# DaanVrancken/HubbardTN

Measured on AMD Instinct MI355X. Metric: DMRG sweep time (s) + GS energy/site, 1-band Hubbard L=64 chi=1024, lower is better.
Workload: dtype c128; 1 GPU; one-band Hubbard chain L=64 U/t=4, half filling, fZ2xSU(2)xU(1), two-site DMRG sweep (2L-3=125 bond updates) at chi=1024 (TensorKit dim units); model=one_band, L=64, chi=1024, krylovdim=30, parallelism=sector-parallel apply x1, backend=hip

## Files before the change

hubbardtn_amd/abi.py:

```python
from __future__ import annotations

import ctypes as C
import os

import numpy as np

HERE = os.path.dirname(os.path.abspath(__file__))
LIB_PATH = os.path.join(HERE, "csrc", "libhubbardtn_hip.so")

HTN_MAX_BUFS = 8
HTN_TILE = 32
OP_N, OP_T, OP_C = 0, 1, 2
SEG_GEMM, SEG_COPY = 0, 1

TILE_DT = np.dtype([("c_off", "<i8"), ("buf_c", "<i4"), ("ldc", "<i4"), ("m", "<i4"), ("n", "<i4"),
                    ("row0", "<i4"), ("col0", "<i4"), ("seg_begin", "<i4"), ("seg_count", "<i4"),
                    ("pad0", "<i4"), ("pad1", "<i4"), ("part", "<i4"), ("nparts", "<i4"), ("ws_slot", "<i4"),
                    ("ticket", "<i4")], align=False)
BUF_WS = 7
WS_TICKET_ELEMS = 4096
SEG_DT = np.dtype([("a_off", "<i8"), ("b_off", "<i8"), ("buf_a", "<i4"), ("buf_b", "<i4"),
                   ("lda", "<i4"), ("ldb", "<i4"), ("k", "<i4"), ("op_a", "<i4"), ("op_b", "<i4"),
                   ("type", "<i4"), ("alpha_re", "<f8"), ("alpha_im", "<f8")], align=False)
SVD_DT = np.dtype([("g_off", "<i8"), ("v_off", "<i8"), ("s_off", "<i8"), ("m", "<i4"), ("n", "<i4"),
                   ("flags", "<i4"), ("pad", "<i4")], align=False)
SVD_ACCUMULATE = 1
SVD_QRCP = 2
COPY_DT = np.dtype([("dst_off", "<i8"), ("src_off", "<i8"), ("idx_off", "<i8"), ("scl_off", "<i8"),
                    ("rows", "<i4"), ("cols", "<i4"), ("ldd", "<i4"), ("lds", "<i4"), ("op", "<i4"),
                    ("gather_dim", "<i4"), ("scale_dim", "<i4"), ("inv_norm", "<i4")], align=False)
assert TILE_DT.itemsize == 64 and SEG_DT.itemsize == 64 and SVD_DT.itemsize == 40 and COPY_DT.itemsize == 64

SYM_SU2_U1, SYM_U1_U1, SYM_SU2 = 0, 1, 2
MAX_SITE = 4
BACKEND_CPU, BACKEND_HIP = 0, 1
SITE_OP_DT = np.dtype([("k", "<i4"), ("dN", "<i4"), ("red", "<f8", (MAX_SITE * MAX_SITE,))], align=False)
MPO_ENTRY_DT = np.dtype([("wl", "<i4"), ("wr", "<i4"), ("op", "<i4"), ("pad", "<i4"), ("coef_re", "<f8"),
                         ("coef_im", "<f8")], align=False)
SUBBLOCK_DT = np.dtype([("lN", "<i4"), ("lj", "<i4"), ("s", "<i4"), ("rN", "<i4"), ("rj", "<i4"), ("ld", "<i4"),
                        ("off", "<i8")], align=False)
SECTOR_DT = np.dtype([("N", "<i4"), ("j", "<i4"), ("count", "<i4")], align=False)
ENV_BLOCK_DT = np.dtype([("aN", "<i4"), ("aj", "<i4"), ("w", "<i4"), ("bN", "<i4"), ("bj", "<i4"), ("rows", "<i4"),
                         ("cols", "<i4"), ("pad", "<i4"), ("off", "<i8")], align=False)
BOND_STATS_DT = np.dtype([("bond", "<i4"), ("direction", "<i4"), ("n_matvec", "<i4"), ("jacobi_sweeps", "<i4"),
                          ("chi_full", "<i4"), ("multiplets", "<i4"), ("n_tiles", "<i4"), ("n_segs", "<i4"),
                          ("theta_size", "<i8"), ("apply_flops", "<i8"), ("apply_bytes", "<i8"), ("svd_flops", "<i8"),
                          ("energy", "<f8"), ("residual", "<f8"), ("trunc_weight", "<f8"), ("t_plan", "<f8"),
                          ("t_lanczos", "<f8"), ("t_svd", "<f8"), ("t_env", "<f8"), ("t_total", "<f8"),
                          ("matvec_ms", "<f8")], align=False)
assert SITE_OP_DT.itemsize == 136 and MPO_ENTRY_DT.itemsize == 32 and SUBBLOCK_DT.itemsize == 32
assert SECTOR_DT.itemsize == 12 and ENV_BLOCK_DT.itemsize == 40 and BOND_STATS_DT.itemsize == 136


class Symmetry(C.Structure):
    _fields_ = [("kind", C.c_int32), ("n_site", C.c_int32), ("site_N", C.c_int32 * MAX_SITE),
                ("site_j", C.c_int32 * MAX_SITE)]


class SvdOpts(C.Structure):
    _fields_ = [("split_elems", C.c_int32), ("sweeps_hint", C.c_int32), ("rank_cut", C.c_double),
                ("sweeps_used", C.POINTER(C.c_int32))]


class SweepOpts(C.Structure):
    _fields_ = [("chi_full", C.c_int32), ("weighting", C.c_int32), ("cutoff", C.c_double), ("krylovdim", C.c_int32),
                ("maxrestart", C.c_int32), ("lanczos_tol", C.c_double), ("jacobi_tol", C.c_double),
                ("jacobi_max_sweeps", C.c_int32), ("svd_split_elems", C.c_int32), ("rank_cut", C.c_double),
                ("profile", C.c_int32), ("pad", C.c_int32)]


class IdmrgOpts(C.Structure):
    _fields_ = [("sweep", SweepOpts), ("cell_sites", C.c_int32), ("window_dN", C.c_int32), ("tol", C.c_double),
                ("min_steps", C.c_int32), ("maxiter", C.c_int32), ("sweeps_per_step", C.c_int32), ("warm_start", C.c_int32)]


class IdmrgStats(C.Structure):
    _fields_ = [("step", C.c_int32), ("sweeps", C.c_int32), ("converged", C.c_int32), ("finished", C.c_int32),
                ("needs_window", C.c_int32), ("chi_full", C.c_int32), ("energy", C.c_double),
                ("energy_per_site", C.c_double), ("delta", C.c_double)]


assert C.sizeof(SweepOpts) == 64 and C.sizeof(IdmrgOpts) == 96 and C.sizeof(IdmrgStats) == 48

EXPORTS = ["htn_last_error", "htn_abi_version", "htn_device_init", "htn_grouped_gemm_z",
           "htn_dots_scratch_elems", "htn_dots_z", "htn_axpys_z", "htn_scale_inv_sqrt_z",
           "htn_jacobi_svd_z", "htn_batched_copy_z", "htn_lanczos_scratch_elems", "htn_lanczos_z", "htn_lanczos_orth_z"]
ENGINE_EXPORTS = ["htn_ctx_create", "htn_ctx_destroy", "htn_ctx_backend", "htn_ctx_set_timing", "htn_comm_unique_id",
                  "htn_ctx_set_comm", "htn_ctx_set_exchange", "htn_mpo_create", "htn_mpo_destroy", "htn_mps_create",
                  "htn_mps_destroy", "htn_bond_update", "htn_dmrg2_sweep", "htn_mps_theta_size", "htn_heff2_apply",
                  "htn_mps_get_theta", "htn_mps_nsites", "htn_mps_bond", "htn_mps_spectrum", "htn_mps_site_size",
                  "htn_mps_get_site", "htn_mps_env_size", "htn_mps_get_env", "htn_mps_env_blocks", "htn_mps_env_bond",
                  "htn_plan_apply_dump", "htn_mps_cache_stats", "htn_balance_tiles",
                  "htn_idmrg_create", "htn_idmrg_destroy", "htn_idmrg_boundary", "htn_idmrg_step", "htn_idmrg_window",
                  "htn_mps_set_orthogonal", "htn_mps_orthogonal_count", "htn_mps_overlap"]


class GemmLaunch(C.Structure):
    _fields_ = [("bufs", C.c_void_p * HTN_MAX_BUFS), ("tiles", C.c_void_p), ("segs", C.c_void_p),
                ("n_tiles", C.c_int32), ("pad", C.c_int32)]


EXCHANGE_FN = C.CFUNCTYPE(C.c_int, C.c_void_p, C.c_int64, C.c_void_p)

_lib = None


class HtnError(RuntimeError):
    pass


def load_library(path: str | None = None):
    global _lib
    if _lib is not None and path is None:
        return _lib
    p = path or LIB_PATH
    import torch
    if not os.path.exists(p):
        raise HtnError(f"{p} not found: build it with `python -m hubbardtn_amd.build` "
                       "(hipcc --offload-arch=gfx950); there is no CPU fallback")
    lib = C.CDLL(p)
    vp, i32, i64, f64 = C.c_void_p, C.c_int32, C.c_int64, C.c_double
    lib.htn_last_error.restype = C.c_char_p
    lib.htn_abi_version.restype = C.c_int
    lib.htn_device_init.argtypes = [C.c_int, C.c_char_p, C.POINTER(C.c_int)]
    lib.htn_grouped_gemm_z.argtypes = [C.POINTER(vp), vp, i32, vp, vp]
    lib.htn_dots_scratch_elems.argtypes = [i32]
    lib.htn_dots_scratch_elems.restype = i64
    lib.htn_dots_z.argtypes = [vp, i64, i32, vp, i64, vp, vp, vp]
    lib.htn_axpys_z.argtypes = [vp, vp, i64, i32, vp, f64, i64, vp]
    lib.htn_scale_inv_sqrt_z.argtypes = [vp, vp, vp, i64, vp]
    lib.htn_jacobi_svd_z.argtypes = [vp, vp, vp, vp, vp, i32, i32, i32, f64, vp, C.POINTER(SvdOpts), vp]
    lib.htn_batched_copy_z.argtypes = [vp, vp, vp, vp, vp, i32, f64, vp]
    lib.htn_lanczos_scratch_elems.argtypes = [i32]
    lib.htn_lanczos_scratch_elems.restype = i64
    lib.htn_lanczos_z.argtypes = [C.POINTER(GemmLaunch), i32, i32, i32, vp, i64, i32, f64, i32, vp, i32,
                                  EXCHANGE_FN, vp, C.POINTER(f64), C.POINTER(i32), C.POINTER(f64), C.POINTER(f64), vp]
    lib.htn_lanczos_orth_z.argtypes = [C.POINTER(GemmLaunch), i32, i32, i32, vp, i64, i32, f64, i32, vp, i32,
                                       EXCHANGE_FN, vp, C.POINTER(f64), C.POINTER(i32), C.POINTER(f64), C.POINTER(f64),
                                       vp, i32, vp]
    declare_engine(lib)
    for name in EXPORTS + ENGINE_EXPORTS:
        getattr(lib, name)
    if lib.htn_abi_version() != ABI_VERSION:
        raise HtnError("ABI version mismatch")
    if path is None:
        _lib = lib
    return lib


ABI_VERSION = 2


def declare_engine(lib):
    vp, i32, i64, f64 = C.c_void_p, C.c_int32, C.c_int64, C.c_double
    lib.htn_last_error.restype = C.c_char_p
    lib.htn_abi_version.restype = C.c_int
    lib.htn_ctx_create.argtypes = [i32, i32, vp, C.POINTER(vp)]
    lib.htn_ctx_destroy.argtypes = [vp]
    lib.htn_ctx_destroy.restype = None
    lib.htn_ctx_backend.argtypes = [vp]
    lib.htn_ctx_set_timing.argtypes = [vp, i32]
    lib.htn_comm_unique_id.argtypes = [vp]
    lib.htn_ctx_set_comm.argtypes = [vp, i32, i32, vp]
    lib.htn_ctx_set_exchange.argtypes = [vp, i32, i32, EXCHANGE_FN, vp]
    lib.htn_mpo_create.argtypes = [vp, C.POINTER(Symmetry), i32, vp, i32, vp, vp, vp, vp, C.POINTER(vp)]
    lib.htn_mpo_destroy.argtypes = [vp]
    lib.htn_mpo_destroy.restype = None
    lib.htn_mps_create.argtypes = [vp, vp, i32, vp, vp, vp, vp, vp, vp, vp, vp, C.POINTER(vp)]
    lib.htn_mps_destroy.argtypes = [vp]
    lib.htn_mps_destroy.restype = None
    lib.htn_bond_update.argtypes = [vp, i32, i32, i32, i32, C.POINTER(SweepOpts), vp]
    lib.htn_dmrg2_sweep.argtypes = [vp, C.POINTER(SweepOpts), vp, C.POINTER(f64)]
    lib.htn_mps_theta_size.argtypes = [vp, i32]
    lib.htn_mps_theta_size.restype = i64
    lib.htn_heff2_apply.argtypes = [vp, i32, vp, vp]
    lib.htn_mps_get_theta.argtypes = [vp, i32, vp]
    lib.htn_mps_nsites.argtypes = [vp]
    lib.htn_mps_bond.argtypes = [vp, i32, vp]
    lib.htn_mps_spectrum.argtypes = [vp, i32, vp, vp]
    lib.htn_mps_spectrum.restype = i64
    lib.htn_mps_site_size.argtypes = [vp, i32, C.POINTER(i32)]
    lib.htn_mps_site_size.restype = i64
    lib.htn_mps_get_site.argtypes = [vp, i32, vp, vp]
    lib.htn_mps_env_size.argtypes = [vp, i32, i32]
    lib.htn_mps_env_size.restype = i64
    lib.htn_mps_get_env.argtypes = [vp, i32, i32, vp]
    lib.htn_mps_env_blocks.argtypes = [vp, i32, i32, vp]
    lib.htn_mps_env_bond.argtypes = [vp, i32, i32, vp]
    lib.htn_plan_apply_dump.argtypes = [vp, i32, i32, C.POINTER(i32), vp, C.POINTER(i32), vp, C.POINTER(i64),
                                        C.POINTER(i64)]
    lib.htn_mps_cache_stats.argtypes = [vp, C.POINTER(i64), C.POINTER(i64)]
    lib.htn_balance_tiles.argtypes = [vp, i32, i32, vp, i32, C.POINTER(i32)]
    lib.htn_idmrg_create.argtypes = [vp, vp, C.POINTER(IdmrgOpts), C.POINTER(vp)]
    lib.htn_idmrg_destroy.argtypes = [vp]
    lib.htn_idmrg_destroy.restype = None
    lib.htn_idmrg_boundary.argtypes = [vp, i32, vp]
    lib.htn_idmrg_step.argtypes = [vp, vp, vp, vp, vp, vp, vp, C.POINTER(IdmrgStats)]
    lib.htn_idmrg_window.argtypes = [vp, C.POINTER(vp)]
    lib.htn_mps_set_orthogonal.argtypes = [vp, C.POINTER(vp), i32]
    lib.htn_mps_orthogonal_count.argtypes = [vp, C.POINTER(i32)]
    lib.htn_mps_overlap.argtypes = [vp, vp, C.POINTER(f64)]
    for name in ENGINE_EXPORTS:
        getattr(lib, name)


def check(lib, rc: int, what: str):
    if rc != 0:
        raise HtnError(f"{what}: {lib.htn_last_error().decode()}")
```

hubbardtn_amd/csrc/htn_backend_hip.hip:

```cpp
#include <dlfcn.h>

#include <map>
#include <mutex>

#include "htn_common.h"
#include "htn_core.h"

namespace {

__global__ __launch_bounds__(256) void k_scale_z(double2* __restrict__ x, int64_t n, double f) {
    for (int64_t j = (int64_t)blockIdx.x * blockDim.x + threadIdx.x; j < n; j += (int64_t)gridDim.x * blockDim.x) {
        const double2 v = x[j];
        x[j] = make_double2(v.x * f, v.y * f);
    }
}

__global__ __launch_bounds__(256) void k_copy_words(uint32_t* __restrict__ dst, const uint32_t* __restrict__ src, size_t n) {
    for (size_t j = (size_t)blockIdx.x * blockDim.x + threadIdx.x; j < n; j += (size_t)gridDim.x * blockDim.x) dst[j] = src[j];
    __threadfence_system();
}

struct Rccl {
    void* lib = nullptr;
    int (*GetUniqueId)(void*) = nullptr;
// ... 161 lines not shown
        } else
            HIP_TRY(hipMemcpyAsync(land, src, bytes, hipMemcpyDeviceToHost, st));
        HIP_TRY(htn_stream_spin(st));
        memcpy(dst, land, bytes);
        stage_pos = 0;
        return 0;
    }
    int zero(void* p, size_t bytes) override {
        if (!bytes) return 0;
        HIP_TRY(hipMemsetAsync(p, 0, bytes, st));
        return 0;
    }
    int sync() override {
        HIP_TRY(htn_stream_spin(st));
        stage_pos = 0;
        return 0;
    }
    int grouped_gemm(const void* const* bufs, const htn_tile* tiles, int32_t n_tiles, const htn_seg* segs) override {
        return htn_grouped_gemm_z(bufs, tiles, n_tiles, segs, st);
    }
    int lanczos(const htn_gemm_launch* stages, int n_stages, int x_slot, int y_slot, void* V, int64_t n, int krylovdim,
                double tol, int max_restart, int zero_y, htn_exchange2_fn exchange, void* user, double* eig, int* n_matvec,
                double* residual, double* matvec_ms) override {
        if (ensure_lan_scratch(htn_lanczos_scratch_elems(krylovdim))) return 1;
        int32_t nmv = 0;
        const int rc = htn_lanczos_z(stages, n_stages, x_slot, y_slot, V, n, krylovdim, tol, max_restart, lan_scratch, zero_y,
                                     exchange, user, eig, &nmv, residual, matvec_ms, st);
        *n_matvec = nmv;
        return rc;
    }
    int ensure_lan_scratch(int64_t need) {
        if (need > lan_scratch_elems) {
            if (lan_scratch) HIP_TRY(hipFree(lan_scratch));
            HIP_TRY(hipMalloc(&lan_scratch, sizeof(double2) * need));
            if (htn_debug_poison()) HIP_TRY(hipMemsetAsync(lan_scratch, 0xFF, sizeof(double2) * need, st));
            lan_scratch_elems = need;
        }
        return 0;
    }
    int lanczos_orth(const htn_gemm_launch* stages, int n_stages, int x_slot, int y_slot, void* V, int64_t n, int krylovdim,
                     double tol, int max_restart, int zero_y, htn_exchange2_fn exchange, void* user, const void* Q, int n_frozen,
                     double* eig, int* n_matvec, double* residual, double* matvec_ms) override {
        if (ensure_lan_scratch(htn_lanczos_scratch_elems(krylovdim + n_frozen))) return 1;
        int32_t nmv = 0;
        const int rc = htn_lanczos_orth_z(stages, n_stages, x_slot, y_slot, V, n, krylovdim, tol, max_restart, lan_scratch, zero_y,
                                          exchange, user, eig, &nmv, residual, matvec_ms, Q, n_frozen, st);
        *n_matvec = nmv;
        return rc;
    }
    int orthonormalise_rows(void* Pv, int64_t n, int nvec, double drop_tol, int* kept) override {
        if (nvec > 32) return htn::set_error("orthonormalise_rows: more than 32 rows");
        if (ensure_lan_scratch(htn_dots_scratch_elems(32) + 64)) return 1;
        double2* P = (double2*)Pv;
        double2* part = (double2*)lan_scratch;
        double2* coef = part + htn_dots_scratch_elems(32);
        double2* nrm = coef + 32;
        int k = 0;
        for (int r = 0; r < nvec; ++r) {
            double2* dst = P + (int64_t)k * n;
            if (r != k) HIP_TRY(hipMemcpyAsync(dst, P + (int64_t)r * n, sizeof(double2) * n, hipMemcpyDeviceToDevice, st));
            if (htn_dots_z(dst, n, 1, dst, n, nrm, part, st)) return 1;
            for (int pass = 0; pass < 2 && k > 0; ++pass) {
                if (htn_dots_z(P, n, k, dst, n, coef, part, st)) return 1;
                if (htn_axpys_z(dst, P, n, k, coef, -1.0, n, st)) return 1;
            }
            if (htn_dots_z(dst, n, 1, dst, n, nrm + 1, part, st)) return 1;
            double h[4];
            if (download(h, nrm, sizeof(h))) return 1;
            const double n0 = h[0], n1 = h[2];
            if (!(n0 > 0.0) || !(n1 > drop_tol * drop_tol * n0)) continue;
            if (htn_scale_inv_sqrt_z(dst, dst, nrm + 1, n, st)) return 1;
            ++k;
        }
        *kept = k;
        return 0;
    }
    int jacobi_svd(void* G, void* Vj, double* S, const htn_svd_block* desc_dev, const htn_svd_block* desc_host, int n_blocks,
                   int max_m, int max_sweeps, double tol, int32_t* info_dev, const htn_svd_opts* opts) override {
        fork_open = true;
        const int rc = htn_jacobi_svd_z(G, Vj, S, desc_dev, desc_host, n_blocks, max_m, max_sweeps, tol, info_dev, opts, st);
        fork_open = false;
        return rc;
    }
    int batched_copy(void* dst, const void* src, const int32_t* idx, const double* scl, const htn_copy_item* items, int n_items,
                     double gscale) override {
        return htn_batched_copy_z(dst, src, idx, scl, items, n_items, gscale, st);
    }
    int scale(void* x, int64_t n, double f) override {
        if (n <= 0) return 0;
        const int grid = (int)std::min<int64_t>((n + 255) / 256, 2048);
        hipLaunchKernelGGL(k_scale_z, dim3(grid), dim3(256), 0, st, (double2*)x, n, f);
        HIP_TRY(hipGetLastError());
        return 0;
    }
    int set_comm(int rank, int world, const void* id) override {
        Rccl& r = rccl();
        if (!r.ok) return htn::set_error("htn_ctx_set_comm: librccl.so could not be loaded");
        if (comm) {
            r.CommDestroy(comm);
            comm = nullptr;
        }
        NcclId uid;
        memcpy(uid.internal, id, sizeof(uid.internal));
        const int rc = ((nccl_init_fn)r.CommInitRank)(&comm, world, uid, rank);
        if (rc != 0) return htn::set_error("ncclCommInitRank: %s", r.GetErrorString ? r.GetErrorString(rc) : "error");
        return 0;
    }
    bool has_comm() const override { return comm != nullptr; }
    int allreduce(void* y, int64_t n) override {
        if (!comm) return htn::set_error("allreduce: no communicator (htn_ctx_set_comm)");
        const int rc = rccl().AllReduce(y, y, (size_t)(2 * n), 8, 0, comm, st);
        if (rc != 0) return htn::set_error("ncclAllReduce: %s", rccl().GetErrorString ? rccl().GetErrorString(rc) : "error");
        return 0;
    }
};

}

char* htn_err_buf() { return htn::err_buf(); }

namespace htn {
Backend* make_backend(int backend, int device, void* stream) {
    if (backend != HTN_BACKEND_HIP) {
        set_error("libhubbardtn_hip.so has no CPU backend (backend %d requested): there is no CPU fallback", backend);
        return nullptr;
    }
    char name[256];
    int cus = 0;
    if (htn_device_init(device, name, &cus)) return nullptr;
    auto* b = new HipBackend();
    b->device = device;
    if (stream) b->st = (hipStream_t)stream;
    else {
        if (hipStreamCreateWithFlags(&b->st, hipStreamNonBlocking) != hipSuccess) {
            set_error("hipStreamCreate failed");
            delete b;
            return nullptr;
        }
        b->own_stream = true;
    }
    return b;
}
}

extern "C" int htn_comm_unique_id(void* id_host) {
    Rccl& r = rccl();
    if (!r.ok) return htn::set_error("htn_comm_unique_id: librccl.so could not be loaded");
    const int rc = r.GetUniqueId(id_host);
    if (rc != 0) return htn::set_error("ncclGetUniqueId: %s", r.GetErrorString ? r.GetErrorString(rc) : "error");
    return 0;
}
```

hubbardtn_amd/csrc/htn_common.h:

```cpp
#pragma once
#include <hip/hip_runtime.h>
#include <stdint.h>
#include <stdio.h>
#include <stdlib.h>
#include <string.h>

#include <map>
#include <memory>
#include <mutex>
#include <utility>

#include "hubbardtn_hip.h"

char* htn_err_buf();

static inline int htn_fail(const char* what, hipError_t e) {
    snprintf(htn_err_buf(), 512, "%s: %s", what, hipGetErrorString(e));
    return 1;
}
static inline int htn_fail_msg(const char* what) {
    snprintf(htn_err_buf(), 512, "%s", what);
    return 1;
}
#define fail htn_fail
// ... 43 lines not shown
__host__ __device__ __forceinline__ unsigned long long lan_check(unsigned long long w0, unsigned long long w1, unsigned long long w2,
                                                                 unsigned long long serial) {
    return serial ^ lan_rotl(w0, 13) ^ lan_rotl(w1, 29) ^ lan_rotl(w2, 47) ^ 0x9E3779B97F4A7C15ull;
}
#define HTN_DOT_BLOCKS 256
struct HtnGemmPublish {
    const double* norm_partial;
    const double2* c1;
    const double2* c2;
    LanRecord* rec_out;
    unsigned long long serial;
};
int htn_grouped_gemm_launch(const void* const* bufs_host, const htn_tile* tiles, int32_t n_tiles, const htn_seg* segs,
                            const HtnGemmPublish* pub, hipStream_t stream);

enum HtnBufKind {
    HTN_BUF_DEVICE,
    HTN_BUF_PINNED,
    HTN_BUF_MAPPED
};
struct HtnBuf {
    const HtnBufKind kind;
    const bool poison;
    void* p = nullptr;
    void* dev = nullptr;
    size_t cap = 0;
    explicit HtnBuf(HtnBufKind k, bool poison_new = true) : kind(k), poison(poison_new) {}
    HtnBuf(const HtnBuf&) = delete;
    ~HtnBuf() { (void)release(); }
    hipError_t release() {
        const hipError_t e = !p ? hipSuccess : (kind == HTN_BUF_DEVICE ? hipFree(p) : hipHostFree(p));
        p = dev = nullptr, cap = 0;
        return e;
    }
    int reserve(size_t bytes) {
        if (bytes <= cap) return 0;
        HIP_TRY(release());
        const size_t want = bytes * 2;
        if (kind == HTN_BUF_DEVICE) {
            HIP_TRY(hipMalloc(&p, want));
            dev = p;
            if (poison && htn_debug_poison()) HIP_TRY(hipMemset(p, 0xFF, want));
        } else if (kind == HTN_BUF_PINNED) {
            HIP_TRY(hipHostMalloc(&p, want, hipHostMallocDefault));
        } else {
            HIP_TRY(hipHostMalloc(&p, want, hipHostMallocMapped | hipHostMallocCoherent));
            HIP_TRY(hipHostGetDevicePointer(&dev, p, 0));
        }
        cap = want;
        return 0;
    }
};

template <class T>
class HtnStreamRegistry {
    std::mutex mu;
    std::map<std::pair<int, hipStream_t>, std::unique_ptr<T>> entries;

public:
    template <class Init>
    int get(hipStream_t st, T** out, Init init) {
        int dev = 0;
        HIP_TRY(hipGetDevice(&dev));
        std::lock_guard<std::mutex> lk(mu);
        auto it = entries.find({dev, st});
        if (it == entries.end()) {
            auto r = std::make_unique<T>();
            r->device = dev;
            if (init(*r)) return 1;
            it = entries.emplace(std::make_pair(dev, st), std::move(r)).first;
        }
        *out = it->second.get();
        return 0;
    }
    void release(hipStream_t st) {
        int dev = 0;
        if (hipGetDevice(&dev) != hipSuccess) return;
        std::lock_guard<std::mutex> lk(mu);
        entries.erase({dev, st});
    }
};
void htn_krylov_release_stream(hipStream_t st);
void htn_svd_release_stream(hipStream_t st);

template <int CTRL>
__device__ __forceinline__ double dpp_f64(double v) {
    const int lo = __builtin_amdgcn_update_dpp(0, __double2loint(v), CTRL, 0xF, 0xF, true);
    const int hi = __builtin_amdgcn_update_dpp(0, __double2hiint(v), CTRL, 0xF, 0xF, true);
    return __hiloint2double(hi, lo);
}

__device__ __forceinline__ double row_sum16(double v) {
    v += dpp_f64<0xB1>(v);
    v += dpp_f64<0x4E>(v);
    v += dpp_f64<0x141>(v);
    v += dpp_f64<0x140>(v);
    return v;
}

template <int L>
__device__ __forceinline__ double lane_bcast(double v) {
    const int lo = __builtin_amdgcn_readlane(__double2loint(v), L);
    const int hi = __builtin_amdgcn_readlane(__double2hiint(v), L);
    return __hiloint2double(hi, lo);
}

__device__ __forceinline__ double wave_sum(double v) {
    v = row_sum16(v);
    const double a = lane_bcast<0>(v) + lane_bcast<16>(v);
    const double b = lane_bcast<32>(v) + lane_bcast<48>(v);
    return a + b;
}

template <int CTRL>
__device__ __forceinline__ unsigned long long dpp_u64(unsigned long long v) {
    const unsigned lo = (unsigned)__builtin_amdgcn_update_dpp(0, (int)(unsigned)v, CTRL, 0xF, 0xF, true);
    const unsigned hi = (unsigned)__builtin_amdgcn_update_dpp(0, (int)(unsigned)(v >> 32), CTRL, 0xF, 0xF, true);
    return ((unsigned long long)hi << 32) | lo;
}
__device__ __forceinline__ unsigned long long umax64(unsigned long long a, unsigned long long b) { return a > b ? a : b; }
__device__ __forceinline__ unsigned long long row_max16_u64(unsigned long long v) {
    v = umax64(v, dpp_u64<0xB1>(v));
    v = umax64(v, dpp_u64<0x4E>(v));
    v = umax64(v, dpp_u64<0x141>(v));
    v = umax64(v, dpp_u64<0x140>(v));
    return v;
}
template <int L>
__device__ __forceinline__ unsigned long long lane_bcast_u64(unsigned long long v) {
    const unsigned lo = (unsigned)__builtin_amdgcn_readlane((int)(unsigned)v, L);
    const unsigned hi = (unsigned)__builtin_amdgcn_readlane((int)(unsigned)(v >> 32), L);
    return ((unsigned long long)hi << 32) | lo;
}
__device__ __forceinline__ unsigned long long wave_max_u64(unsigned long long v) {
    v = row_max16_u64(v);
    return umax64(umax64(lane_bcast_u64<0>(v), lane_bcast_u64<16>(v)),
                  umax64(lane_bcast_u64<32>(v), lane_bcast_u64<48>(v)));
}

__device__ __forceinline__ double fast_rcp(double a) {
    double x = __builtin_amdgcn_rcp(a);
    x = fma(fma(-a, x, 1.0), x, x);
    x = fma(fma(-a, x, 1.0), x, x);
    return x;
}
__device__ __forceinline__ double fast_rsq(double a) {
    double y = __builtin_amdgcn_rsq(a);
    const double h = 0.5 * a;
    y = y * fma(-h * y, y, 1.5);
    y = y * fma(-h * y, y, 1.5);
    return y;
}
```

hubbardtn_amd/csrc/htn_core.h:

```cpp
#pragma once
#include <stdint.h>
#include <string.h>

#include <array>
#include <complex>
#include <memory>
#include <string>
#include <unordered_map>
#include <utility>
#include <vector>

#include "hubbardtn_hip.h"

namespace htn {

typedef std::complex<double> cplx;

enum { BUF_X = 0, BUF_Y, BUF_L, BUF_R, BUF_Z, BUF_S1, BUF_S2, BUF_AUX };

struct Sec {
    int32_t N, j;
};
inline bool operator<(const Sec& a, const Sec& b) { return a.N < b.N || (a.N == b.N && a.j < b.j); }
inline bool operator==(const Sec& a, const Sec& b) { return a.N == b.N && a.j == b.j; }
// ... 184 lines not shown
    int64_t zsize = 0;
    int64_t nterms = 0;
};
void plan_apply(const Mpo& mpo, const ThetaLayout& tl, const EnvLayout& Ll, const EnvLayout& Rl, const MpoSite& W1,
                const MpoSite& W2, ApplyPlan& out);
void plan_theta(const char* mode, const SiteLayout& lay1, const SiteLayout& lay2, const ThetaLayout& tl, Tasks& out);
struct EnvPlan {
    Tasks t1, t2;
    int64_t zsize = 0;
};
void plan_left_env(const Mpo& mpo, const EnvLayout& Ll, const SiteLayout& lay, const MpoSite& W, const EnvLayout& Lnew,
                   EnvPlan& out);
void plan_right_env(const Mpo& mpo, const EnvLayout& Rl, const SiteLayout& lay, const MpoSite& W, const EnvLayout& Rnew,
                    EnvPlan& out);

struct OvlLayout {
    BondP rows, cols;
    std::vector<Sec> secs;
    std::vector<int64_t> off;
    std::vector<int32_t> m, n;
    std::unordered_map<uint64_t, int> index;
    int64_t size = 0;
    int find(Sec s) const {
        auto it = index.find(skey(s));
        return it == index.end() ? -1 : it->second;
    }
};
typedef std::shared_ptr<const OvlLayout> OvlLayoutP;
OvlLayoutP build_ovl_layout(BondP rows, BondP cols);
struct OvlPlan {
    Tasks t1, t2;
    int64_t zsize = 0;
};
void plan_ovl_left(const OvlLayout& Ol, const SiteLayout& bra, const SiteLayout& ket, const OvlLayout& Onew, OvlPlan& out);
void plan_ovl_right(const OvlLayout& Or, const SiteLayout& bra, const SiteLayout& ket, const OvlLayout& Onew, OvlPlan& out);
void plan_ovl_project(const OvlLayout& Ol, const OvlLayout& Or, const SiteLayout& k1, const SiteLayout& k2, const ThetaLayout& tl,
                      OvlPlan& out);

struct SvdPlan {
    std::vector<htn_svd_block> desc;
    std::vector<htn_copy_item> stage;
    std::vector<Sec> mids;
    std::vector<char> transposed, accumulate;
    int64_t g_size = 0, v_size = 0, s_size = 0;
    int32_t max_m = 0;
    int64_t flops = 0;
    bool any_accumulate = false;
};
int plan_svd(const ThetaLayout& tl, bool right, SvdPlan& out);

void truncate(const std::vector<double>& vals, const std::vector<int>& lens, const std::vector<int>& qdims, int chi_full,
              double cutoff, int weighting, std::vector<int>& counts, double& trunc_weight, double& kept_norm);

struct FinalizePlan {
    std::vector<htn_copy_item> iso_g, cen_g, iso_v;
    Tasks cen;
    bool has_cen = false;
    int64_t n_idx = 0;
};
void plan_finalize(const ThetaLayout& tl, const SvdPlan& sp, const std::vector<int>& keep, const SiteLayout& layA,
                   const SiteLayout& layB, bool right, int64_t offA, int64_t offB, FinalizePlan& out);

struct Backend {
    virtual ~Backend() {}
    virtual int kind() const = 0;
    virtual int activate() { return 0; }
    virtual void* alloc(size_t bytes) = 0;
    virtual void release(void* p) = 0;
    virtual int upload(void* dst, const void* src_host, size_t bytes) = 0;
    virtual int download(void* dst_host, const void* src, size_t bytes) = 0;
    virtual int zero(void* p, size_t bytes) = 0;
    virtual int sync() = 0;
    virtual int grouped_gemm(const void* const* bufs, const htn_tile* tiles, int32_t n_tiles, const htn_seg* segs) = 0;
    virtual int lanczos(const htn_gemm_launch* stages, int n_stages, int x_slot, int y_slot, void* V, int64_t n,
                        int krylovdim, double tol, int max_restart, int zero_y, htn_exchange2_fn exchange, void* user,
                        double* eig, int* n_matvec, double* residual, double* matvec_ms) = 0;
    virtual int lanczos_orth(const htn_gemm_launch* stages, int n_stages, int x_slot, int y_slot, void* V, int64_t n,
                             int krylovdim, double tol, int max_restart, int zero_y, htn_exchange2_fn exchange, void* user,
                             const void* Q, int n_frozen, double* eig, int* n_matvec, double* residual, double* matvec_ms);
    virtual int orthonormalise_rows(void* P, int64_t n, int nvec, double drop_tol, int* kept);
    virtual int jacobi_svd(void* G, void* Vj, double* S, const htn_svd_block* desc_dev, const htn_svd_block* desc_host,
                           int n_blocks, int max_m, int max_sweeps, double tol, int32_t* info_dev,
                           const htn_svd_opts* opts) = 0;
    virtual int batched_copy(void* dst, const void* src, const int32_t* idx, const double* scl,
                             const htn_copy_item* items_dev, int n_items, double gscale) = 0;
    virtual int scale(void* x, int64_t n, double f) = 0;
    virtual int set_comm(int rank, int world, const void* id) { return 1; }
    virtual bool has_comm() const { return false; }
    virtual int allreduce(void* y, int64_t n) { return 1; }
    bool timing = false;
};

int set_error(const char* fmt, ...);
char* err_buf();

}
```

hubbardtn_amd/csrc/htn_engine.cpp:

```cpp
#include <math.h>
#include <stdio.h>
#include <stdlib.h>

#include <algorithm>
#include <atomic>
#include <chrono>
#include <map>

#include "htn_core.h"

namespace htn {
Backend* make_backend(int backend, int device, void* stream);
}
using namespace htn;

namespace {
void tridiag_lowest_host(const std::vector<double>& alpha, const std::vector<double>& beta, double* eig, std::vector<double>& vec) {
    const int k = (int)alpha.size();
    auto count = [&](double x) {
        int cnt = 0;
        double d = 1.0;
        for (int i = 0; i < k; ++i) {
            d = (alpha[i] - x) - (i ? beta[i - 1] * beta[i - 1] / d : 0.0);
            if (d == 0.0) d = 1e-300;
// ... 191 lines not shown
    }
    DBuf(const DBuf&) = delete;
    DBuf& operator=(const DBuf&) = delete;
};
typedef std::shared_ptr<DBuf> DBufP;
struct DView {
    DBufP base;
    int64_t off = 0;
    cplx* ptr() const { return base ? (cplx*)base->p + off : nullptr; }
};

struct DevTasks {
    DBufP mem;
    const htn_tile* tiles = nullptr;
    const htn_seg* segs = nullptr;
    int32_t ntiles = 0, nsegs = 0;
    int32_t ws_slots = 0;
    int64_t flops = 0;
};

struct ApplyC {
    DevTasks dz, dy;
    bool has_z = false;
    int64_t zsize = 0, flops = 0;
    int32_t ntiles = 0, nsegs = 0;
};
struct EnvC {
    EnvLayoutP lay;
    DevTasks d1, d2;
    int64_t zsize = 0, flops = 0;
};
struct SvdC {
    SvdPlan sp;
    DBufP stage, desc;
    std::vector<htn_svd_block> own_desc;
    DBufP own_stage, own_desc_dev;
    int n_own = 0;
};
struct FinC {
    SiteLayoutP layA, layB;
    DBufP items;
    const htn_copy_item *ig = nullptr, *cg = nullptr, *iv = nullptr;
    int n_ig = 0, n_cg = 0, n_iv = 0;
    DevTasks cen;
    bool has_cen = false;
};

struct Spectrum {
    std::vector<Sec> secs;
    std::vector<std::vector<double>> vals;
};
struct OvlC {
    OvlLayoutP lay;
    DevTasks d1, d2;
    int64_t zsize = 0;
};
struct OrthState {
    htn_mps* phi = nullptr;
    std::vector<OvlLayoutP> Llay, Rlay;
    std::vector<DView> Lbuf, Rbuf;
};

}

struct htn_mps {
    std::atomic<int> refs{1};
    htn_ctx* ctx;
    htn_mpo* mpo_handle = nullptr;
    Backend* be;
    const Mpo* mpo;
    int L;
    std::vector<BondP> bonds;
    std::vector<SiteLayoutP> site_lay;
    std::vector<DView> site_buf;
    std::vector<EnvLayoutP> Llay, Rlay;
    std::vector<DView> Lbuf, Rbuf;
    std::unordered_map<std::string, std::shared_ptr<const void>> cache;
    int64_t hits = 0, misses = 0;
    double energy = 0.0;
    std::map<int, Spectrum> spectra;
    std::map<int, std::pair<std::pair<int, double>, double>> cut_hint;
    std::map<int, int> sweeps_hint;
    std::vector<int32_t> idx_host;
    std::vector<OrthState> orth;
    int orth_dropped = 0;

    template <class T, class F>
    std::shared_ptr<T> cached(const std::string& key, F build) {
        auto it = cache.find(key);
        if (it != cache.end()) {
            ++hits;
            return std::const_pointer_cast<T>(std::static_pointer_cast<const T>(it->second));
        }
        if (cache.size() > 20000) cache.clear();
        ++misses;
        std::shared_ptr<T> v = build();
        if (v) cache[key] = v;
        return v;
    }
    static std::string ikey(const char* tag, int i) {
        std::string k(tag);
        k.append((const char*)&i, sizeof(i));
        return k;
    }
    DBufP dalloc(size_t bytes) {
        auto b = std::make_shared<DBuf>(be, bytes);
        return b->p ? b : nullptr;
    }
    DView zalloc(int64_t n, bool zero) {
        DView v;
        v.base = dalloc(sizeof(cplx) * (size_t)std::max<int64_t>(n, 1));
        if (v.base && zero) be->zero(v.base->p, sizeof(cplx) * (size_t)std::max<int64_t>(n, 1));
        return v;
    }
    DView ws;
    int64_t ws_slots = -1;
    int ensure_ws(int slots) {
        if (slots <= ws_slots) return 0;
        const int64_t want = std::max<int64_t>(2 * (int64_t)slots, 256);
        ws = zalloc(HTN_WS_ELEMS(want), false);
        if (!ws.base) return set_error("device allocation of the split-K workspace failed");
        if (be->zero(ws.ptr(), sizeof(cplx) * HTN_WS_TICKET_ELEMS)) return 1;
        ws_slots = want;
        return 0;
    }
    int upload_tasks(const Tasks& t_in, DevTasks& d) {
        Tasks balanced;
        const Tasks* tp = &t_in;
        d.ws_slots = 0;
        if (be->kind() == HTN_BACKEND_HIP && t_in.ntiles > 0) {
            balanced = t_in;
            balanced.tiles.resize((size_t)t_in.ntiles);
            d.ws_slots = balance_tiles(balanced, 256);
            tp = &balanced;
        }
        const Tasks& t = *tp;
        const size_t tb = (sizeof(htn_tile) * t.tiles.size() + 63) / 64 * 64, sb = sizeof(htn_seg) * t.segs.size();
        d.mem = dalloc(tb + sb);
        if (!d.mem) return set_error("device allocation of a task list failed");
        if (be->upload(d.mem->p, t.tiles.data(), sizeof(htn_tile) * t.tiles.size())) return 1;
        if (be->upload((char*)d.mem->p + tb, t.segs.data(), sb)) return 1;
        d.tiles = (const htn_tile*)d.mem->p;
        d.segs = (const htn_seg*)((char*)d.mem->p + tb);
        d.ntiles = t.ntiles;
        d.nsegs = t.nsegs;
        d.flops = t.flops;
        return 0;
    }
    SiteLayoutP site_layout(char kind, BondP bl, BondP br) {
        return cached<const SiteLayout>(std::string("slay") + kind + bl->key + "|" + br->key,
                                        [&] { return build_site_layout(mpo->sym, kind, bl, br); });
    }
    ThetaLayoutP theta_layout(BondP bl, BondP br) {
        return cached<const ThetaLayout>(std::string("tl") + bl->key + "|" + br->key,
                                         [&] { return build_theta_layout(mpo->sym, bl, br); });
    }
    int gemm(const DevTasks& d, std::initializer_list<std::pair<int, const void*>> bufs) {
        if (d.ntiles == 0) return 0;
        if (ensure_ws(d.ws_slots)) return 1;
        const void* table[HTN_MAX_BUFS] = {nullptr};
        for (auto& kv : bufs) table[kv.first] = kv.second;
        table[HTN_BUF_WS] = ws.ptr();
        return be->grouped_gemm(table, d.tiles, d.ntiles, d.segs);
    }

    int left_env(int i);
// ... 275 lines not shown
        if (plan_svd(tl, right, s->sp)) return nullptr;
        s->stage = dalloc(sizeof(htn_copy_item) * s->sp.stage.size());
        s->desc = dalloc(sizeof(htn_svd_block) * s->sp.desc.size());
        if (!s->stage || !s->desc) return nullptr;
        if (be->upload(s->stage->p, s->sp.stage.data(), sizeof(htn_copy_item) * s->sp.stage.size())) return nullptr;
        if (be->upload(s->desc->p, s->sp.desc.data(), sizeof(htn_svd_block) * s->sp.desc.size())) return nullptr;
        if (ctx->world > 1) {
            const int nbk = (int)s->sp.mids.size();
            std::vector<int> ord(nbk);
            for (int b = 0; b < nbk; ++b) ord[b] = b;
            auto cost = [&](int b) { return (double)s->sp.desc[b].m * s->sp.desc[b].n * s->sp.desc[b].n; };
            std::stable_sort(ord.begin(), ord.end(), [&](int a, int b) { return cost(a) > cost(b); });
            std::vector<double> load(ctx->world, 0.0);
            std::vector<htn_copy_item> st_own;
            for (int b : ord) {
                int r = 0;
                for (int q = 1; q < ctx->world; ++q)
                    if (load[q] < load[r]) r = q;
                load[r] += cost(b);
                if (r == ctx->rank) {
                    s->own_desc.push_back(s->sp.desc[b]);
                    st_own.push_back(s->sp.stage[b]);
                }
            }
            s->n_own = (int)s->own_desc.size();
            if (s->n_own) {
                s->own_stage = dalloc(sizeof(htn_copy_item) * st_own.size());
                s->own_desc_dev = dalloc(sizeof(htn_svd_block) * s->own_desc.size());
                if (!s->own_stage || !s->own_desc_dev) return nullptr;
                if (be->upload(s->own_stage->p, st_own.data(), sizeof(htn_copy_item) * st_own.size())) return nullptr;
                if (be->upload(s->own_desc_dev->p, s->own_desc.data(), sizeof(htn_svd_block) * s->own_desc.size())) return nullptr;
            }
        }
        return s;
    });
    if (!sc) return 1;
    const SvdPlan& sp = sc->sp;
    const int nb = (int)sp.mids.size();
    DView G = zalloc(sp.g_size, false), Vj = zalloc(sp.v_size, false);
    const size_t s_elems = ((size_t)std::max<int64_t>(sp.s_size, 1) + 1) & ~(size_t)1, i_elems = (size_t)std::max(nb, 1);
    DBufP S = dalloc(sizeof(double) * s_elems + sizeof(int32_t) * i_elems);
    if (!G.base || !Vj.base || !S) return set_error("device allocation failed (SVD workspace)");
    int32_t* info_dev = (int32_t*)((double*)S->p + s_elems);
    const bool svd_shard = ctx->world > 1 && ctx->shard;
    if (svd_shard) {
        if (be->zero(G.ptr(), sizeof(cplx) * (size_t)std::max<int64_t>(sp.g_size, 1))) return 1;
        if (be->zero(S->p, sizeof(double) * s_elems + sizeof(int32_t) * i_elems)) return 1;
        if (sp.any_accumulate && be->zero(Vj.ptr(), sizeof(cplx) * (size_t)std::max<int64_t>(sp.v_size, 1))) return 1;
        if (sc->n_own && be->batched_copy(G.ptr(), x, nullptr, nullptr, (const htn_copy_item*)sc->own_stage->p, sc->n_own, 1.0)) return 1;
    } else if (be->batched_copy(G.ptr(), x, nullptr, nullptr, (const htn_copy_item*)sc->stage->p, nb, 1.0))
        return 1;
    htn_svd_opts so;
    int32_t jac_used = 0;
    so.split_elems = o.svd_split_elems;
    so.sweeps_hint = 0;
    so.rank_cut = 0.0;
    so.sweeps_used = &jac_used;
    {
        auto h = sweeps_hint.find(i + 1);
        if (h != sweeps_hint.end()) so.sweeps_hint = h->second;
    }
    if (o.rank_cut > 0.0) {
        double cut = 0.0;
        auto h = cut_hint.find(i + 1);
        if (h != cut_hint.end() && h->second.first.first == o.chi_full && h->second.first.second == o.cutoff)
            cut = o.rank_cut * h->second.second;
        so.rank_cut = std::max(cut, o.rank_cut * o.cutoff);
    }
    if (svd_shard) {
        if (sc->n_own && be->jacobi_svd(G.ptr(), Vj.ptr(), (double*)S->p, (const htn_svd_block*)sc->own_desc_dev->p,
                                        sc->own_desc.data(), sc->n_own, sp.max_m, o.jacobi_max_sweeps > 0 ? o.jacobi_max_sweeps : 40,
                                        o.jacobi_tol > 0.0 ? o.jacobi_tol : 1e-14, info_dev, &so))
            return 1;
        if (exchange_tramp(G.ptr(), std::max<int64_t>(sp.g_size, 1), ctx)) return set_error("sharded SVD: exchange of the blocks failed");
        if (exchange_tramp(S->p, (int64_t)(s_elems / 2), ctx)) return set_error("sharded SVD: exchange of the singular values failed");
        if (sp.any_accumulate && exchange_tramp(Vj.ptr(), std::max<int64_t>(sp.v_size, 1), ctx)) return 1;
    } else if (be->jacobi_svd(G.ptr(), Vj.ptr(), (double*)S->p, (const htn_svd_block*)sc->desc->p, sp.desc.data(), nb, sp.max_m,
                              o.jacobi_max_sweeps > 0 ? o.jacobi_max_sweeps : 40, o.jacobi_tol > 0.0 ? o.jacobi_tol : 1e-14,
                              info_dev, &so))
        return 1;
    if (jac_used > 0) sweeps_hint[i + 1] = jac_used;
    static const bool dbg_timers = getenv("HTN_DEBUG_HOST_TIMERS") != nullptr;
    const double tA = now();
    std::vector<double> s_host(s_elems + (i_elems + 1) / 2);
    if (be->download(s_host.data(), S->p, sizeof(double) * s_elems + sizeof(int32_t) * i_elems)) return 1;
    const double tB = now();
    const int32_t* info_h = (const int32_t*)(s_host.data() + s_elems);
    int jac_sweeps = 0;
    for (int b = 0; b < (svd_shard ? sc->n_own : nb); ++b) {
        if (info_h[b] < 0) return set_error("Jacobi SVD did not converge (bond %d, block %d, %d sweeps)", i + 1, b, -info_h[b]);
        jac_sweeps = std::max(jac_sweeps, (int)info_h[b]);
    }
    std::vector<int> lens(nb), qd(nb);
    std::vector<std::vector<int>> order(nb);
    std::vector<double> vals;
    vals.reserve((size_t)sp.s_size);
    std::vector<std::pair<double, int>> tmp;
    for (int b = 0; b < nb; ++b) {
        const int len = sp.desc[b].n;
        const double* sv = s_host.data() + sp.desc[b].s_off;
        lens[b] = len;
        qd[b] = sym.qdim(sp.mids[b]);
        tmp.resize(len);
        for (int k = 0; k < len; ++k) tmp[k] = {sv[k], k};
        std::sort(tmp.begin(), tmp.end(), [](const std::pair<double, int>& a, const std::pair<double, int>& c) {
            return a.first != c.first ? a.first > c.first : a.second < c.second;
        });
        order[b].resize(len);
        for (int k = 0; k < len; ++k) {
            order[b][k] = tmp[k].second;
            vals.push_back(tmp[k].first);
        }
    }
    std::vector<int> counts;
    double tw = 0.0, nrm = 0.0;
    truncate(vals, lens, qd, o.chi_full, o.cutoff, o.weighting, counts, tw, nrm);
    std::vector<std::pair<Sec, int>> mid_items;
    int64_t kept_tot = 0, positive = 0;
    for (int b = 0; b < nb; ++b) {
        if (counts[b] > 0) mid_items.push_back({sp.mids[b], counts[b]});
        kept_tot += counts[b];
    }
    for (double v : vals) positive += v > 0.0;
    if (kept_tot == 0 || !(nrm > 0.0)) return set_error("htn_bond_update: nothing kept by the truncation on bond %d", i + 1);
    BondP mid = std::make_shared<Bond>(mid_items);
    const double tC = now();
    if (o.chi_full > 0 && tw > 0.0 && kept_tot < positive) {
        double smin = 1e300;
        size_t p = 0;
        for (int b = 0; b < nb; ++b) {
            if (counts[b] > 0) smin = std::min(smin, vals[p + counts[b] - 1]);
            p += lens[b];
        }
        cut_hint[i + 1] = {{o.chi_full, o.cutoff}, smin};
    } else
        cut_hint.erase(i + 1);
    std::string ckey((const char*)counts.data(), sizeof(int) * counts.size());
    auto fc = cached<FinC>(std::string(right ? "finR" : "finL") + bl->key + "|" + br->key + "|" + ckey, [&]() -> std::shared_ptr<FinC> {
        auto f = std::make_shared<FinC>();
        f->layA = site_layout('L', bl, mid);
        f->layB = site_layout('R', mid, br);
        FinalizePlan fp;
        plan_finalize(tl, sp, counts, *f->layA, *f->layB, right, 0, f->layA->size, fp);
        f->n_ig = (int)fp.iso_g.size(), f->n_cg = (int)fp.cen_g.size(), f->n_iv = (int)fp.iso_v.size();
        const size_t tot = (size_t)(f->n_ig + f->n_cg + f->n_iv);
        if (tot) {
            std::vector<htn_copy_item> all;
            all.insert(all.end(), fp.iso_g.begin(), fp.iso_g.end());
            all.insert(all.end(), fp.cen_g.begin(), fp.cen_g.end());
            all.insert(all.end(), fp.iso_v.begin(), fp.iso_v.end());
            f->items = dalloc(sizeof(htn_copy_item) * tot);
            if (!f->items || be->upload(f->items->p, all.data(), sizeof(htn_copy_item) * tot)) return nullptr;
            f->ig = (const htn_copy_item*)f->items->p;
            f->cg = f->ig + f->n_ig;
            f->iv = f->cg + f->n_cg;
        }
        f->has_cen = fp.has_cen;
        if (fp.has_cen && upload_tasks(fp.cen, f->cen)) return nullptr;
        return f;
    });
    if (!fc) return 1;
    const double tD = now();
    idx_host.clear();
    for (int b = 0; b < nb; ++b)
        for (int k = 0; k < counts[b]; ++k) idx_host.push_back(order[b][k]);
    DBufP idx_d = dalloc(sizeof(int32_t) * std::max<size_t>(idx_host.size(), 1));
    const int64_t sizeA = fc->layA->size, sizeB = fc->layB->size;
    DView out = zalloc(sizeA + sizeB, true);
    if (!idx_d || !out.base) return set_error("device allocation failed (site tensors)");
    if (be->upload(idx_d->p, idx_host.data(), sizeof(int32_t) * idx_host.size())) return 1;
    const int32_t* idxp = (const int32_t*)idx_d->p;
    const double* Sp = (const double*)S->p;
    if (fc->n_ig && be->batched_copy(out.ptr(), G.ptr(), idxp, Sp, fc->ig, fc->n_ig, 1.0)) return 1;
    if (fc->n_cg && be->batched_copy(out.ptr(), G.ptr(), idxp, Sp, fc->cg, fc->n_cg, 1.0 / nrm)) return 1;
    if (fc->n_iv && be->batched_copy(out.ptr(), Vj.ptr(), idxp, Sp, fc->iv, fc->n_iv, 1.0)) return 1;
    if (fc->has_cen) {
        if (be->scale(x, n, 1.0 / nrm)) return 1;
        if (gemm(fc->cen, {{BUF_X, x}, {BUF_S1, out.ptr()}, {BUF_Y, out.ptr()}})) return 1;
    }
    bonds[i + 1] = mid;
    site_lay[i] = fc->layA;
    site_buf[i] = DView{out.base, out.off};
    site_lay[i + 1] = fc->layB;
    site_buf[i + 1] = DView{out.base, out.off + sizeA};
    if (dbg_timers)
        fprintf(stderr, "bond %d: svd call %.1f us, download %.1f, sort+truncate %.1f, finalize plan %.1f, enqueue %.1f  misses %lld hits %lld nvals %zu\n", i + 1,
                (tA - t0 - t_plan - t_lan) * 1e6, (tB - tA) * 1e6, (tC - tB) * 1e6, (tD - tC) * 1e6, (now() - tD) * 1e6, (long long)misses, (long long)hits, vals.size());
    if (o.profile) be->sync();
    const double t_svd = now() - t0 - t_plan - t_lan;
    if (right ? left_env(i) : right_env(i + 1)) return 1;
    for (auto& os : orth)
        if (right ? ovl_left(os.phi, i, os.Llay[i], os.Lbuf[i], &os.Llay[i + 1], &os.Lbuf[i + 1])
                  : ovl_right(os.phi, i + 1, os.Rlay[i + 2], os.Rbuf[i + 2], &os.Rlay[i + 1], &os.Rbuf[i + 1]))
            return 1;
    if (o.profile) be->sync();
    const double t_env = now() - t0 - t_plan - t_lan - t_svd;
    energy = E;
    Spectrum spec;
    {
        size_t p = 0;
        for (int b = 0; b < nb; ++b) {
            if (counts[b] > 0) {
                spec.secs.push_back(sp.mids[b]);
                std::vector<double> v(counts[b]);
                const double f = 1.0 / nrm / sqrt((double)qd[b]);
                for (int k = 0; k < counts[b]; ++k) v[k] = vals[p + k] * f;
                spec.vals.push_back(std::move(v));
            }
            p += lens[b];
        }
    }
    spectra[i + 1] = std::move(spec);
    if (st) {
        memset(st, 0, sizeof(*st));
        st->bond = i + 1;
        st->direction = direction;
        st->n_matvec = nmv;
        st->jacobi_sweeps = jac_sweeps;
        st->chi_full = (int32_t)mid->dim_full(sym);
        st->multiplets = mid->multiplets();
        st->n_tiles = ap->ntiles;
        st->n_segs = ap->nsegs;
        st->theta_size = n;
        st->apply_flops = ap->flops;
        st->apply_bytes = 16 * (2 * n + Llay[i]->size + Rlay[i + 2]->size);
        st->svd_flops = sp.flops;
        st->energy = E;
        st->residual = res;
        st->trunc_weight = tw;
        st->t_plan = t_plan;
        st->t_lanczos = t_lan;
        st->t_svd = t_svd;
        st->t_env = t_env;
        st->t_total = now() - t0;
        st->matvec_ms = mv_ms > 0.0 ? mv_ms : 0.0;
    }
    return 0;
}

int htn_mps::sweep(const htn_sweep_opts& o, htn_bond_stats* st, double* E) {
    int k = 0;
    for (int i = 0; i < L - 1; ++i, ++k)
        if (update_bond(i, +1, i < L - 2, true, o, st ? st + k : nullptr)) return 1;
    for (int i = L - 3; i >= 0; --i, ++k)
        if (update_bond(i, -1, false, true, o, st ? st + k : nullptr)) return 1;
    if (E) *E = energy;
    return 0;
}
// ... 1025 lines not shown
```

hubbardtn_amd/csrc/htn_krylov.hip:

```cpp
#include <math.h>

#include <chrono>
#include <vector>

#include "htn_common.h"

#define DOT_BLOCKS HTN_DOT_BLOCKS
#define DOT_THREADS 256
#define DOT_CHUNK 32

#define HTN_CH_DISPATCH(nvec, per, LAUNCH)          \
    do {                                            \
        if ((nvec) <= 4) LAUNCH(4, 256);            \
        else if ((nvec) <= 8) LAUNCH(8, 256);       \
        else if ((nvec) <= 12) LAUNCH(12, 256);     \
        else if ((nvec) <= 16) LAUNCH(16, 256);     \
        else if ((nvec) <= 20) LAUNCH(20, 256);     \
        else if ((nvec) <= 24) LAUNCH(24, 256);     \
        else if ((nvec) <= 28) LAUNCH(28, 256);     \
        else LAUNCH(32, 256);                       \
    } while (0)
static inline int64_t dot_slice(int64_t n) { return (n + DOT_BLOCKS - 1) / DOT_BLOCKS; }

template <bool FZ>
// ... 293 lines not shown
#pragma unroll
        for (int b = 0; b < DOT_BLOCKS / 64; ++b) t += norm_partial[tid + 64 * b];
        t = wave_sum(t);
        if (tid == 0) {
            s_inv = t > 0.0 ? 1.0 / sqrt(t) : 0.0;
            if (blockIdx.x == 0 && rec_out) {
                const unsigned long long w0 = (unsigned long long)__double_as_longlong(c1[0].x);
                const unsigned long long w1 = (unsigned long long)__double_as_longlong(c2[0].x);
                const unsigned long long w2 = (unsigned long long)__double_as_longlong(t);
                ulonglong2* out = (ulonglong2*)rec_out;
                out[0] = make_ulonglong2(w0, w1);
                out[1] = make_ulonglong2(w2, lan_check(w0, w1, w2, serial));
                __threadfence_system();
            }
        }
    }
    __syncthreads();
    const double s = s_inv;
    for (int64_t j = (int64_t)blockIdx.x * DOT_THREADS + tid; j < n; j += (int64_t)gridDim.x * DOT_THREADS) {
        const double2 v = src[j];
        dst[j] = make_double2(v.x * s, v.y * s);
    }
}

__global__ __launch_bounds__(64) void k_publish_record(const double* __restrict__ norm_partial, const double2* __restrict__ c1,
                                                       const double2* __restrict__ c2, LanRecord* __restrict__ rec_out,
                                                       unsigned long long serial) {
    const int tid = threadIdx.x;
    double t = 0.0;
#pragma unroll
    for (int b = 0; b < DOT_BLOCKS / 64; ++b) t += norm_partial[tid + 64 * b];
    t = wave_sum(t);
    if (tid == 0) {
        const unsigned long long w0 = (unsigned long long)__double_as_longlong(c1[0].x);
        const unsigned long long w1 = (unsigned long long)__double_as_longlong(c2[0].x);
        const unsigned long long w2 = (unsigned long long)__double_as_longlong(t);
        ulonglong2* out = (ulonglong2*)rec_out;
        out[0] = make_ulonglong2(w0, w1);
        out[1] = make_ulonglong2(w2, lan_check(w0, w1, w2, serial));
        __threadfence_system();
    }
}

__global__ __launch_bounds__(DOT_THREADS) void k_norm_partial(const double2* __restrict__ w, int64_t n,
                                                              double* __restrict__ norm_partial) {
    __shared__ double red[DOT_THREADS / 64];
    const int tid = threadIdx.x;
    const int64_t per = (n + DOT_BLOCKS - 1) / DOT_BLOCKS;
    const int64_t lo = (int64_t)blockIdx.x * per;
    const int64_t hi = lo + per < n ? lo + per : n;
    double nn = 0.0;
    for (int64_t j = lo + tid; j < hi; j += DOT_THREADS) {
        const double2 x = w[j];
        nn += x.x * x.x + x.y * x.y;
    }
    nn = wave_sum(nn);
    if ((tid & 63) == 0) red[tid >> 6] = nn;
    __syncthreads();
    if (tid == 0) {
        double t = 0.0;
        for (int q = 0; q < DOT_THREADS / 64; ++q) t += red[q];
        norm_partial[blockIdx.x] = t;
    }
}

__global__ __launch_bounds__(256) void k_axpys(double2* __restrict__ w, const double2* __restrict__ V,
                                               int64_t ldv, int nvec, const double2* __restrict__ coef,
                                               double sign, int64_t n) {
    for (int64_t j = (int64_t)blockIdx.x * blockDim.x + threadIdx.x; j < n; j += (int64_t)gridDim.x * blockDim.x) {
        double sr = 0.0, si = 0.0;
        for (int i = 0; i < nvec; ++i) {
            const double2 c = coef[i];
            const double2 v = V[(int64_t)i * ldv + j];
            sr += c.x * v.x - c.y * v.y;
            si += c.x * v.y + c.y * v.x;
        }
        double2 x = w[j];
        x.x += sign * sr;
        x.y += sign * si;
        w[j] = x;
    }
}

__global__ __launch_bounds__(256) void k_scale_inv_sqrt(double2* __restrict__ dst, const double2* __restrict__ src,
                                                        const double2* __restrict__ nrm2, int64_t n) {
    const double s = 1.0 / sqrt(nrm2[0].x);
    for (int64_t j = (int64_t)blockIdx.x * blockDim.x + threadIdx.x; j < n; j += (int64_t)gridDim.x * blockDim.x) {
        const double2 v = src[j];
        dst[j] = make_double2(v.x * s, v.y * s);
    }
}

static inline int grid_for(int64_t n) {
    int64_t b = (n + 255) / 256;
    return (int)(b > 1024 ? 1024 : (b < 1 ? 1 : b));
}

extern "C" int64_t htn_dots_scratch_elems(int32_t nvec) { return (int64_t)nvec * DOT_BLOCKS; }

extern "C" int htn_dots_z(const void* V, int64_t ldv, int32_t nvec, const void* w, int64_t n, void* out,
                          void* scratch, void* stream) {
    if (nvec <= 0) return 0;
    if (nvec > 64) return fail_msg("htn_dots_z: nvec > 64");
    launch_dots_partial((const double2*)V, ldv, nvec, (const double2*)w, n, (double2*)scratch, (hipStream_t)stream);
    hipLaunchKernelGGL(k_dots_reduce, dim3(nvec), dim3(64), 0, (hipStream_t)stream, (const double2*)scratch,
                       nvec, (double2*)out);
    HIP_TRY(hipGetLastError());
    return 0;
}

extern "C" int htn_axpys_z(void* w, const void* V, int64_t ldv, int32_t nvec, const void* coef, double sign,
                           int64_t n, void* stream) {
    if (nvec <= 0 || n <= 0) return 0;
    hipLaunchKernelGGL(k_axpys, dim3(grid_for(n)), dim3(256), 0, (hipStream_t)stream, (double2*)w, (const double2*)V,
                       ldv, nvec, (const double2*)coef, sign, n);
    HIP_TRY(hipGetLastError());
    return 0;
}

extern "C" int htn_scale_inv_sqrt_z(void* dst, const void* src, const void* nrm2, int64_t n, void* stream) {
    if (n <= 0) return 0;
    hipLaunchKernelGGL(k_scale_inv_sqrt, dim3(grid_for(n)), dim3(256), 0, (hipStream_t)stream, (double2*)dst,
                       (const double2*)src, (const double2*)nrm2, n);
    HIP_TRY(hipGetLastError());
    return 0;
}

static int sturm_count(const std::vector<double>& a, const std::vector<double>& b, double x) {
    int cnt = 0;
    double d = 1.0;
    const int k = (int)a.size();
    for (int i = 0; i < k; ++i) {
        const double off = i ? b[i - 1] * b[i - 1] : 0.0;
        d = (a[i] - x) - (i ? off / d : 0.0);
        if (d == 0.0) d = 1e-300;
        if (d < 0.0) ++cnt;
    }
    return cnt;
}

static void tridiag_lowest(const std::vector<double>& alpha, const std::vector<double>& beta, double* eig,
                           std::vector<double>& vec) {
    const int k = (int)alpha.size();
    double lo = alpha[0], hi = alpha[0];
    for (int i = 0; i < k; ++i) {
        const double r = (i ? fabs(beta[i - 1]) : 0.0) + (i + 1 < k ? fabs(beta[i]) : 0.0);
        lo = fmin(lo, alpha[i] - r);
        hi = fmax(hi, alpha[i] + r);
    }
    const double scale = fmax(fabs(lo), fabs(hi)) + 1e-300;
    hi = hi + 1e-12 * scale;
    for (int it = 0; it < 200 && hi - lo > 4e-16 * scale; ++it) {
        const double mid = 0.5 * (lo + hi);
        if (sturm_count(alpha, beta, mid) >= 1) hi = mid;
        else lo = mid;
    }
    const double lam = 0.5 * (lo + hi);
    *eig = lam;
    vec.assign(k, 1.0 / sqrt((double)k));
    if (k == 1) {
        vec[0] = 1.0;
        return;
    }
    const double mu = lam - 1e-10 * scale;
    std::vector<double> d(k), l(k), z(k);
    d[0] = alpha[0] - mu;
    for (int i = 1; i < k; ++i) {
        l[i] = beta[i - 1] / d[i - 1];
        d[i] = (alpha[i] - mu) - l[i] * beta[i - 1];
        if (d[i] == 0.0) d[i] = 1e-300;
    }
    for (int i = 0; i < k; ++i) vec[i] = (i & 1) ? -0.7 : 1.0;
    for (int iter = 0; iter < 4; ++iter) {
        z[0] = vec[0];
        for (int i = 1; i < k; ++i) z[i] = vec[i] - l[i] * z[i - 1];
        z[k - 1] /= d[k - 1];
        for (int i = k - 2; i >= 0; --i) z[i] = z[i] / d[i] - l[i + 1] * z[i + 1];
        double nn = 0.0;
        for (int i = 0; i < k; ++i) nn += z[i] * z[i];
        nn = 1.0 / sqrt(nn);
        for (int i = 0; i < k; ++i) vec[i] = z[i] * nn;
    }
    if (vec[0] < 0.0)
        for (int i = 0; i < k; ++i) vec[i] = -vec[i];
}

extern "C" int64_t htn_lanczos_scratch_elems(int32_t krylovdim) {
    return 2 * (int64_t)(krylovdim + 1) * DOT_BLOCKS + 3 * (krylovdim + 1) + DOT_BLOCKS + 8;
}

#define LAN_SLOTS 64
namespace {
struct LanRes {
    int device = -1;
    LanRecord* h_rec = nullptr;
    LanRecord* d_rec = nullptr;
    double2* h_y = nullptr;
    hipEvent_t ev_done[LAN_SLOTS], ev_mv0[LAN_SLOTS], ev_mv1[LAN_SLOTS];
    bool have_events = false;
    unsigned long long serial = 0;
    unsigned sample = 0;
    ~LanRes() {
        if (device >= 0) (void)hipSetDevice(device);
        if (h_rec) (void)hipHostFree(h_rec);
        if (h_y) (void)hipHostFree(h_y);
        if (have_events)
            for (int i = 0; i < LAN_SLOTS; ++i) {
                (void)hipEventDestroy(ev_done[i]);
                (void)hipEventDestroy(ev_mv0[i]);
                (void)hipEventDestroy(ev_mv1[i]);
            }
    }
};
HtnStreamRegistry<LanRes> g_lan_res;

int lan_res_get(hipStream_t st, LanRes** out) {
    return g_lan_res.get(st, out, [](LanRes& r) -> int {
        HIP_TRY(hipHostMalloc((void**)&r.h_rec, sizeof(LanRecord) * LAN_SLOTS, hipHostMallocMapped | hipHostMallocCoherent));
        memset(r.h_rec, 0, sizeof(LanRecord) * LAN_SLOTS);
        HIP_TRY(hipHostGetDevicePointer((void**)&r.d_rec, r.h_rec, 0));
        HIP_TRY(hipHostMalloc((void**)&r.h_y, sizeof(double2) * LAN_SLOTS, hipHostMallocDefault));
        for (int i = 0; i < LAN_SLOTS; ++i) {
            HIP_TRY(hipEventCreateWithFlags(&r.ev_done[i], hipEventDisableTiming));
            HIP_TRY(hipEventCreate(&r.ev_mv0[i]));
            HIP_TRY(hipEventCreate(&r.ev_mv1[i]));
        }
        r.have_events = true;
        return 0;
    });
}
}

void htn_krylov_release_stream(hipStream_t st) { g_lan_res.release(st); }

static int lanczos_run(const htn_gemm_launch* stages, int32_t n_stages, int32_t x_slot, int32_t y_slot,
                       void* Vv, int64_t n, int32_t krylovdim, double tol, int32_t max_restart,
                       void* scratch, int32_t zero_y, htn_exchange2_fn exchange, void* user,
                       double* eig_host, int32_t* n_matvec_host, double* residual_host,
                       double* matvec_ms_host, void* stream_v, const double2* Q, int nf) {
    hipStream_t st = (hipStream_t)stream_v;
    const int kd = krylovdim;
    const int kt = kd + nf;
    double2* V = (double2*)Vv;
    double2* partial = (double2*)scratch;
    double2* partial2 = partial + (int64_t)(kt + 1) * DOT_BLOCKS;
    double2* c1 = partial2 + (int64_t)(kt + 1) * DOT_BLOCKS;
    double2* c2 = c1 + (kt + 1);
    double2* ycoef = c2 + (kt + 1);
    double* norm_partial = (double*)(ycoef + (kt + 1));

    LanRes* R = nullptr;
    if (lan_res_get(st, &R)) return 1;
    const bool event_waits = htn_debug_event_waits();
    static const bool full_first_pass = htn_env_flag("HTN_LANCZOS_FULL_FIRST_PASS");

    bool timed_step[LAN_SLOTS] = {false};
    unsigned long long step_serial[LAN_SLOTS] = {0};
    auto matvec = [&](double2* x, double2* y, const HtnGemmPublish* pub) -> int {
        if (zero_y) HIP_TRY(hipMemsetAsync(y, 0, sizeof(double2) * n, st));
        bool published = pub == nullptr;
        for (int s = 0; s < n_stages; ++s) {
            const void* bufs[HTN_MAX_BUFS];
            for (int b = 0; b < HTN_MAX_BUFS; ++b) bufs[b] = stages[s].bufs[b];
            bufs[x_slot] = x;
            bufs[y_slot] = y;
            const bool here = !published && stages[s].n_tiles > 0;
            if (htn_grouped_gemm_launch(bufs, stages[s].tiles, stages[s].n_tiles, stages[s].segs, here ? pub : nullptr, st)) return 1;
            published |= here;
        }
        if (!published)
            hipLaunchKernelGGL(k_publish_record, dim3(1), dim3(64), 0, st, pub->norm_partial, pub->c1, pub->c2, pub->rec_out, pub->serial);
        if (exchange && exchange(y, n, user)) return fail_msg("htn_lanczos_z: the exchange hook reported a failure");
        return 0;
    };
    auto enqueue_step = [&](int j, bool first) -> int {
        double2* vj = V + (int64_t)j * n;
        double2* w = V + (int64_t)(j + 1) * n;
        const bool timed = matvec_ms_host && (R->sample % 8) == 0;
        timed_step[j] = timed;
        ++R->sample;
        step_serial[j] = ++R->serial;
        HtnGemmPublish pub = {nullptr, nullptr, nullptr, nullptr, 0ull};
        if (!first) pub = {norm_partial, (const double2*)(c1 + (j - 1)), (const double2*)(c2 + (j - 1)), R->d_rec + (j - 1), step_serial[j - 1]};
        if (timed) HIP_TRY(hipEventRecord(R->ev_mv0[j], st));
        if (matvec(vj, w, first ? nullptr : &pub)) return 1;
        if (timed) HIP_TRY(hipEventRecord(R->ev_mv1[j], st));
        if (!first && event_waits) HIP_TRY(hipEventRecord(R->ev_done[j - 1], st));
        const int upd0 = full_first_pass || j < 2 ? 0 : j - 1;
        if (nf == 0) {
            launch_dots_partial(V + (int64_t)upd0 * n, n, j + 1 - upd0, w, n, partial, st);
            launch_axpy_dots(w, V, n, j + 1, partial, c1 + j, j, -1.0, n, partial2, first ? (const double*)nullptr : norm_partial, upd0, st);
            launch_axpy_norm(w, V, n, j + 1, partial2, c2 + j, j, -1.0, n, norm_partial, st);
        } else {
            launch_dots_partial_fz(V, n, nf + j + 1 - upd0, w, n, partial, Q, nf, upd0, st);
            launch_axpy_dots_fz(w, V, n, nf + j + 1, partial, c1 + j, nf + j, -1.0, n, partial2,
                                first ? (const double*)nullptr : norm_partial, nf + upd0, Q, nf, st);
            launch_axpy_norm_fz(w, V, n, nf + j + 1, partial2, c2 + j, nf + j, -1.0, n, norm_partial, Q, nf, st);
        }
        if (j == kd - 1) {
            hipLaunchKernelGGL(k_publish_record, dim3(1), dim3(64), 0, st, (const double*)norm_partial, (const double2*)(c1 + j),
                               (const double2*)(c2 + j), R->d_rec + j, step_serial[j]);
            if (event_waits) HIP_TRY(hipEventRecord(R->ev_done[j], st));
        }
        return 0;
    };
    auto read_record = [&](int j, double* a1, double* a2, double* nn) -> bool {
        const volatile unsigned long long* p = R->h_rec[j].w;
        const unsigned long long w0 = p[0], w1 = p[1], w2 = p[2], w3 = p[3];
        if (w3 != lan_check(w0, w1, w2, step_serial[j])) return false;
        memcpy(a1, &w0, 8);
        memcpy(a2, &w1, 8);
        memcpy(nn, &w2, 8);
        return true;
    };
    auto wait_step = [&](int j, double* a1, double* a2, double* nn) -> int {
        if (event_waits) {
            HIP_TRY(hipEventSynchronize(R->ev_done[j]));
            if (!read_record(j, a1, a2, nn)) return fail_msg("htn_lanczos_z: the step's event completed but its record does not validate");
            return 0;
        }
        for (unsigned spins = 1;; ++spins) {
            if (read_record(j, a1, a2, nn)) return 0;
            __builtin_ia32_pause();
            if ((spins & 0xffff) == 0) {
                const hipError_t q = hipStreamQuery(st);
                if (q == hipSuccess)
                    return read_record(j, a1, a2, nn) ? 0 : fail_msg("htn_lanczos_z: the stream drained without producing the step's record");
                if (q != hipErrorNotReady) return fail("hipStreamQuery", q);
            }
        }
    };

    auto project_out = [&](double2* w) {
        for (int pass = 0; pass < 2; ++pass) {
            launch_dots_partial(Q, n, nf, w, n, partial, st);
            launch_axpy_norm(w, Q, n, nf, partial, c1, -1, -1.0, n, norm_partial, st);
        }
    };
    if (nf > 0) project_out(V);
    else
    hipLaunchKernelGGL(k_norm_partial, dim3(DOT_BLOCKS), dim3(DOT_THREADS), 0, st, V, n, norm_partial);
    hipLaunchKernelGGL(k_scale_by_norm, dim3(grid_for(n)), dim3(DOT_THREADS), 0, st, V, V, norm_partial, n,
                       (LanRecord*)nullptr, (const double2*)nullptr, (const double2*)nullptr, 0ull);
    double mv_ms = 0.0;
    int nmv = 0, n_timed = 0;
    static const bool dbg_timers = getenv("HTN_DEBUG_HOST_TIMERS") != nullptr;
    auto now_us = [] { return std::chrono::duration<double, std::micro>(std::chrono::steady_clock::now().time_since_epoch()).count(); };
    double t_enq = 0.0, t_wait = 0.0, t_host = 0.0;
    const double t_begin = now_us();
    double theta = 0.0, res = 0.0, beta = 0.0, amax = 0.0;
    std::vector<double> y;
    for (int restart = 0; restart <= max_restart; ++restart) {
        std::vector<double> alphas, betas;
        double tq = now_us();
        if (enqueue_step(0, true)) return 1;
        t_enq += now_us() - tq;
        ++nmv;
        for (int j = 0; j < kd; ++j) {
            if (j + 1 < kd) {
                tq = now_us();
                if (enqueue_step(j + 1, false)) return 1;
                t_enq += now_us() - tq;
                ++nmv;
            }
            double a1 = 0.0, a2 = 0.0, nn = 0.0;
            tq = now_us();
            if (wait_step(j, &a1, &a2, &nn)) return 1;
            t_wait += now_us() - tq;
            tq = now_us();
            if (timed_step[j]) {
                float ms = 0.f;
                HIP_TRY(htn_event_spin(R->ev_mv1[j]));
                HIP_TRY(hipEventElapsedTime(&ms, R->ev_mv0[j], R->ev_mv1[j]));
                mv_ms += ms;
                ++n_timed;
            }
            const double alpha = a1 + a2;
            if (!(alpha == alpha) || !(nn == nn)) return fail_msg("htn_lanczos_z: NaN in the tridiagonal coefficients (operator or start vector not finite)");
            beta = sqrt(nn > 0.0 ? nn : 0.0);
            alphas.push_back(alpha);
            tridiag_lowest(alphas, betas, &theta, y);
            res = fabs(beta * y.back());
            amax = std::max(amax, std::max(fabs(alpha), beta));
            t_host += now_us() - tq;
            if (res < tol || beta < 1e-14 * std::max(amax, 1e-300) || j == kd - 1) break;
            betas.push_back(beta);
        }
        HIP_TRY(htn_stream_spin(st));
        const int k = (int)y.size();
        for (int i = 0; i < k; ++i) R->h_y[i] = make_double2(y[i], 0.0);
        HIP_TRY(hipMemcpyAsync(ycoef, R->h_y, sizeof(double2) * k, hipMemcpyHostToDevice, st));
        double2* xrow = V + (int64_t)(kd + 1) * n;
        HIP_TRY(hipMemsetAsync(xrow, 0, sizeof(double2) * n, st));
        hipLaunchKernelGGL(k_axpys, dim3(grid_for(n)), dim3(256), 0, st, xrow, V, n, k, ycoef, 1.0, n);
        if (nf > 0) project_out(xrow);
        else
        hipLaunchKernelGGL(k_norm_partial, dim3(DOT_BLOCKS), dim3(DOT_THREADS), 0, st, xrow, n, norm_partial);
        hipLaunchKernelGGL(k_scale_by_norm, dim3(grid_for(n)), dim3(DOT_THREADS), 0, st, V, xrow, norm_partial, n,
                           (LanRecord*)nullptr, (const double2*)nullptr, (const double2*)nullptr, 0ull);
        HIP_TRY(htn_stream_spin(st));
        if (res < tol || beta < 1e-14 * std::max(amax, 1e-300)) break;
    }
    HIP_TRY(hipGetLastError());
    if (dbg_timers)
        fprintf(stderr, "lanczos n=%lld: %d matvecs in %.1f us: enqueue %.1f, waiting for records %.1f, tridiagonal %.1f\n", (long long)n, nmv,
                now_us() - t_begin, t_enq, t_wait, t_host);
    *eig_host = theta;
    *n_matvec_host = nmv;
    *residual_host = res;
    if (matvec_ms_host) *matvec_ms_host = n_timed ? mv_ms * nmv / n_timed : -1.0;
    return 0;
}

extern "C" int htn_lanczos_z(const htn_gemm_launch* stages, int32_t n_stages, int32_t x_slot, int32_t y_slot,
                             void* Vv, int64_t n, int32_t krylovdim, double tol, int32_t max_restart,
                             void* scratch, int32_t zero_y, htn_exchange2_fn exchange, void* user,
                             double* eig_host, int32_t* n_matvec_host, double* residual_host,
                             double* matvec_ms_host, void* stream_v) {
    if (krylovdim < 2 || krylovdim + 1 > DOT_CHUNK) return fail_msg("htn_lanczos_z: krylovdim must be in 2..31");
    return lanczos_run(stages, n_stages, x_slot, y_slot, Vv, n, krylovdim, tol, max_restart, scratch, zero_y, exchange, user,
                       eig_host, n_matvec_host, residual_host, matvec_ms_host, stream_v, nullptr, 0);
}

extern "C" int htn_lanczos_orth_z(const htn_gemm_launch* stages, int32_t n_stages, int32_t x_slot, int32_t y_slot,
                                  void* Vv, int64_t n, int32_t krylovdim, double tol, int32_t max_restart,
                                  void* scratch, int32_t zero_y, htn_exchange2_fn exchange, void* user,
                                  double* eig_host, int32_t* n_matvec_host, double* residual_host,
                                  double* matvec_ms_host, const void* Q, int32_t n_frozen, void* stream_v) {
    if (n_frozen < 0 || (n_frozen > 0 && !Q)) return fail_msg("htn_lanczos_orth_z: n_frozen rows need a device pointer Q");
    if (krylovdim < 2 || krylovdim + n_frozen + 1 > DOT_CHUNK)
        return fail_msg("htn_lanczos_orth_z: krylovdim >= 2 and krylovdim + n_frozen <= 31 required");
    return lanczos_run(stages, n_stages, x_slot, y_slot, Vv, n, krylovdim, tol, max_restart, scratch, zero_y, exchange, user,
                       eig_host, n_matvec_host, residual_host, matvec_ms_host, stream_v, (const double2*)Q, n_frozen);
}
```

hubbardtn_amd/csrc/htn_svd.hip:

```cpp
#include <algorithm>
#include <utility>
#include <vector>

#include "htn_common.h"

#define JAC_THREADS 1024
#define JAC_MAXEL 8

template <int GS>
__device__ __forceinline__ double group_sum(double v) {
    v = row_sum16(v);
    if (GS == 16) return v;
    const double a = lane_bcast<0>(v) + lane_bcast<16>(v);
    const double b = lane_bcast<32>(v) + lane_bcast<48>(v);
    if (GS == 32) return (threadIdx.x & 32) ? b : a;
    return a + b;
}

template <int GS>
__device__ __forceinline__ double jacobi_pair(double2* ga, double2* gb, double2* __restrict__ va,
                                              double2* __restrict__ vb, int m, int n, int sub, double tol,
                                              bool accumulate, double zero2) {
    double2 a[JAC_MAXEL], b[JAC_MAXEL];
    double aa = 0.0, bb = 0.0, gr = 0.0, gi = 0.0;
// ... 891 lines not shown
        __syncthreads();
        if (!s_share_ok) rank = -1;
    }
    for (int i = tid; i < n0; i += JAC_THREADS) s_col[i] = i;
    __syncthreads();
    return rank;
}

#define QR_SYNC_WORDS 16
#define QR_BOX_BYTES 137728
__global__ __launch_bounds__(JAC_THREADS) void k_qr_large(double2* __restrict__ G, double2* __restrict__ Vj,
                                                          const htn_svd_block* __restrict__ desc,
                                                          const int* __restrict__ large_ids, int* __restrict__ perm,
                                                          double* __restrict__ zero2_out, double cut2,
                                                          int* __restrict__ rank_host, int NW, char* __restrict__ qr_box,
                                                          unsigned* __restrict__ qr_sync, int nl, int nx, int part_off) {
    extern __shared__ double2 g_lds[];
    __shared__ double s_piv[2];
    __shared__ int s_col[64 * JAC_MAXEL];
    __shared__ double s_cn2[64 * JAC_MAXEL];
    __shared__ int s_qlocal;
    const int px = (int)(blockIdx.x % (unsigned)nx), ps = (int)(blockIdx.x / (unsigned)nx);
    const int li = (ps / NW) * nx + px, role = ps % NW;
    if (li >= nl) return;
    const htn_svd_block D = desc[large_ids[li]];
    const int m = D.m, n = D.n, m0 = D.pad, tid = threadIdx.x;
    const int gsx = m <= 16 * JAC_MAXEL ? 16 : (m <= 32 * JAC_MAXEL ? 32 : 64);
    const int mp = gsx * ((m + gsx - 1) / gsx);
    double2* __restrict__ X = Vj + D.v_off;
    QrShare sh;
    sh.NW = NW, sh.role = role;
    char* box = qr_box + (size_t)li * QR_BOX_BYTES;
    sh.qn = (double2*)box;
    sh.scol = (int*)(box + 16 * 513 * 16);
    sh.cn2 = (double*)(box + 16 * 513 * 16 + 512 * 4);
    sh.meta = (int*)(box + 16 * 513 * 16 + 512 * 4 + 512 * 8);
    sh.qflag = qr_sync + li * QR_SYNC_WORDS;
    sh.hflag = qr_sync + li * QR_SYNC_WORDS + 1;
    sh.fail = qr_sync + nl * QR_SYNC_WORDS;
    sh.local = false;
    if (NW > 1) {
        if (tid == 0) {
            unsigned xcc;
            asm volatile("s_getreg_b32 %0, hwreg(HW_REG_XCC_ID)" : "=s"(xcc));
            xcc = (xcc & 0xfu) + 1u;
            unsigned* xw = qr_sync + li * QR_SYNC_WORDS + 8;
            __hip_atomic_store(xw + role, xcc, __ATOMIC_RELAXED, __HIP_MEMORY_SCOPE_AGENT);
            int local = 1;
            for (int q = 0; q < NW && local >= 0; ++q) {
                if (!qr_wait_ge(xw + q, 1u, sh.fail)) local = -1;
                else if (__hip_atomic_load(xw + q, __ATOMIC_RELAXED, __HIP_MEMORY_SCOPE_AGENT) != xcc) local = 0;
            }
            s_qlocal = local;
        }
        __syncthreads();
        sh.local = s_qlocal > 0;
    }
    double* part = (part_off > 0 && ((m0 + 15) & ~15) <= 256) ? (double*)(g_lds + part_off) : nullptr;
    if (role > 0) {
        qr_helper(G + D.g_off, m0, m, n, X, mp, s_col, (double2*)g_lds, tid, sh, part);
        return;
    }
    int rank;
    if (NW > 1) {
        if (m0 <= 256) rank = qrcp_blocked<4, true>(G + D.g_off, m0, m, n, X, mp, s_col, s_cn2, s_piv, (double2*)g_lds, tid, cut2, sh, part);
        else rank = qrcp_blocked<8, true>(G + D.g_off, m0, m, n, X, mp, s_col, s_cn2, s_piv, (double2*)g_lds, tid, cut2, sh, part);
    } else {
        if (m0 <= 256) rank = qrcp_blocked<4, false>(G + D.g_off, m0, m, n, X, mp, s_col, s_cn2, s_piv, (double2*)g_lds, tid, cut2, sh, part);
        else rank = qrcp_blocked<8, false>(G + D.g_off, m0, m, n, X, mp, s_col, s_cn2, s_piv, (double2*)g_lds, tid, cut2, sh, part);
    }
    if (tid == 0) {
        rank_host[li] = rank;
        zero2_out[li] = s_piv[1];
        __threadfence_system();
    }
    for (int i = tid; i < m; i += JAC_THREADS) perm[li * 64 * JAC_MAXEL + i] = s_col[i];
}

__global__ __launch_bounds__(JAC_THREADS) void k_jacobi_svd(double2* __restrict__ G, double2* __restrict__ Vj,
                                                            double* __restrict__ S,
                                                            const htn_svd_block* __restrict__ desc,
                                                            int max_sweeps, double tol, int* __restrict__ info,
                                                            int lds_elems, const int* __restrict__ large_slot,
                                                            double cut2) {
    extern __shared__ double2 g_lds[];
    __shared__ double s_ratio;
    __shared__ double s_piv[2];
    __shared__ int s_col[64 * JAC_MAXEL];
    __shared__ double s_cn2[64 * JAC_MAXEL];
    if (large_slot && large_slot[blockIdx.x] >= 0) return;
    const htn_svd_block D = desc[blockIdx.x];
    const int m = D.m, n = D.n;
    double2* __restrict__ gglob = G + D.g_off;
    double2* __restrict__ v = Vj + D.v_off;
    const int tid = threadIdx.x, lane = tid & 63, wave = tid >> 6;
    const int nwaves = JAC_THREADS / 64;
    const bool in_lds = (int64_t)m * n <= lds_elems;
    const bool accumulate = (D.flags & HTN_SVD_ACCUMULATE) != 0;
    const bool qrcp = (D.flags & HTN_SVD_QRCP) != 0;
    double2* g;
    if (qrcp) {
        const int m0 = D.pad;
        const int gsx = m <= 16 * JAC_MAXEL ? 16 : (m <= 32 * JAC_MAXEL ? 32 : 64);
        const int E = (m + gsx - 1) / gsx;
        const int mp = gsx * E;
        const bool x_lds = (int64_t)mp * n <= lds_elems;
        const int nl = x_lds ? n : 0;
        const SplitCols X = {(double2*)g_lds, v, nl, mp};
        int rank;
        if (m0 <= 16 * JAC_MAXEL) rank = qrcp_mgs<16>(gglob, m0, m, n, X, s_col, s_cn2, s_piv, tid, cut2);
        else if (m0 <= 32 * JAC_MAXEL) rank = qrcp_mgs<32>(gglob, m0, m, n, X, s_col, s_cn2, s_piv, tid, cut2);
        else rank = qrcp_mgs<64>(gglob, m0, m, n, X, s_col, s_cn2, s_piv, tid, cut2);
        {
            double f = 0.0;
            for (int idx = tid; idx < mp * n; idx += JAC_THREADS) {
                const double2 x = X.col(idx / mp)[idx % mp];
                f += x.x * x.x + x.y * x.y;
            }
            f = wave_sum(f);
            if (lane == 0) s_cn2[wave] = f;
            __syncthreads();
            if (tid == 0) {
                double t = 0.0;
                for (int q = 0; q < JAC_THREADS / 64; ++q) t += s_cn2[q];
                s_ratio = t;
            }
            __syncthreads();
        }
        const double zero2q = 1e-30 * s_ratio;
        __syncthreads();
        int swq;
        if (x_lds) {
            const DenseCols<double2*> dc = {(double2*)g_lds, mp};
            if (gsx == 16) swq = jacobi_dispatch_e<16>(dc, E, rank, max_sweeps, tol, &s_ratio, tid, zero2q);
            else if (gsx == 32) swq = jacobi_dispatch_e<32>(dc, E, rank, max_sweeps, tol, &s_ratio, tid, zero2q);
            else swq = jacobi_dispatch_e<64>(dc, E, rank, max_sweeps, tol, &s_ratio, tid, zero2q);
        } else {
            const DenseCols<double2*> dc = {v, mp};
            if (gsx == 16) swq = jacobi_dispatch_e<16>(dc, E, rank, max_sweeps, tol, &s_ratio, tid, zero2q);
            else if (gsx == 32) swq = jacobi_dispatch_e<32>(dc, E, rank, max_sweeps, tol, &s_ratio, tid, zero2q);
            else swq = jacobi_dispatch_e<64>(dc, E, rank, max_sweeps, tol, &s_ratio, tid, zero2q);
        }
        __syncthreads();
        for (int j = wave; j < n; j += nwaves) {
            double sn = 0.0;
            for (int i = lane; i < m; i += 64) {
                const double2 x = X.col(j)[i];
                sn += x.x * x.x + x.y * x.y;
                gglob[(int64_t)j * m + s_col[i]] = x;
            }
            sn = wave_sum(sn);
            if (lane == 0) S[D.s_off + j] = sqrt(sn);
        }
        if (tid == 0) info[blockIdx.x] = swq;
        return;
    } else {
        if (accumulate)
            for (int idx = tid; idx < n * n; idx += JAC_THREADS) {
                const int i = idx % n, j = idx / n;
                v[idx] = make_double2(i == j ? 1.0 : 0.0, 0.0);
            }
        if (in_lds)
            for (int idx = tid; idx < m * n; idx += JAC_THREADS) g_lds[idx] = gglob[idx];
        __syncthreads();
        g = in_lds ? (double2*)g_lds : gglob;
    }
    {
        double f = 0.0;
        for (int idx = tid; idx < m * n; idx += JAC_THREADS) {
            const double2 x = g[idx];
            f += x.x * x.x + x.y * x.y;
        }
        f = wave_sum(f);
        if (lane == 0) s_cn2[wave] = f;
        __syncthreads();
        if (tid == 0) {
            double t = 0.0;
            for (int q = 0; q < JAC_THREADS / 64; ++q) t += s_cn2[q];
            s_ratio = t;
        }
        __syncthreads();
    }
    const double zero2 = 1e-30 * s_ratio;
    __syncthreads();
    int sw;
    if (m <= 16 * JAC_MAXEL) sw = jacobi_sweeps<16>(g, v, m, n, max_sweeps, tol, &s_ratio, tid, accumulate, zero2);
    else if (m <= 32 * JAC_MAXEL) sw = jacobi_sweeps<32>(g, v, m, n, max_sweeps, tol, &s_ratio, tid, accumulate, zero2);
    else sw = jacobi_sweeps<64>(g, v, m, n, max_sweeps, tol, &s_ratio, tid, accumulate, zero2);
    __syncthreads();
    for (int j = wave; j < n; j += nwaves) {
        double s = 0.0;
        for (int i = lane; i < m; i += 64) {
            const double2 x = g[(int64_t)j * m + i];
            s += x.x * x.x + x.y * x.y;
            if (in_lds) gglob[(int64_t)j * m + i] = x;
        }
        s = wave_sum(s);
        if (lane == 0) S[D.s_off + j] = sqrt(s);
    }
    if (tid == 0) info[blockIdx.x] = sw;
}

#define JAC_PANEL 8
struct JacPairItem {
    int32_t blk, ci, ni, cj, nj, pad[3];
};

__device__ __forceinline__ int jg_partner(int x, int r, int mode) {
    if (mode == 0) return x < 8 ? 8 + ((x + r) & 7) : ((x - r) & 7);
    const int g = x & 8, k = x & 7;
    if (k == 7) return g + r;
    if (k == r) return g + 7;
    int y = 2 * r - k + 7;
    y = y >= 14 ? y - 14 : (y >= 7 ? y - 7 : y);
    return g + y;
}

__device__ __forceinline__ double2 cmul(double2 a, double2 b) {
    return make_double2(fma(a.x, b.x, -a.y * b.y), fma(a.x, b.y, a.y * b.x));
}
__device__ __forceinline__ double2 cmulc(double2 ac, double2 b) {
    return make_double2(fma(ac.x, b.x, ac.y * b.y), fma(ac.x, b.y, -ac.y * b.x));
}


__device__ __forceinline__ bool jg_rotation(double aa, double bb, double2 g, bool live, double z2, double tol2,
                                            double& c, double& cq, double& dq) {
    const double g2 = fma(g.x, g.x, g.y * g.y);
    const bool on = live && aa > z2 && bb > z2 && g2 > 0.0 && g2 > tol2 * aa * bb;
    const double h = on ? bb - aa : 0.0, g2s = on ? g2 : 1.0, ah = fabs(h);
    const double w2 = fma(h, h, 4.0 * g2s);
    const double iw = fast_rsq(w2);
    double q = 2.0 * fast_rcp(fma(w2, iw, ah));
    q = h >= 0.0 ? q : -q;
    const double c2 = fma(0.5 * ah, iw, 0.5);
    const double cc = c2 * fast_rsq(c2);
    c = on ? cc : 1.0;
    cq = on ? cc * q : 0.0;
    dq = on ? q * g2s : 0.0;
    return on;
}

#define JG_LD 17
#define JG_PS 9
#define JG_GU_ELEMS (4 * 64 * JG_PS / 2)
__global__ __launch_bounds__(256) void k_jacobi_pairs_gram(double2* __restrict__ Vj,
                                                           const htn_svd_block* __restrict__ desc,
                                                           const int* __restrict__ large_ids,
                                                           const JacPairItem* __restrict__ items,
                                                           const double* __restrict__ zero2,
                                                           unsigned long long* __restrict__ ratio_bits,
                                                           const int* __restrict__ done, double tol, int inner) {
    extern __shared__ double2 g_lds[];
    __shared__ unsigned long long s_rbits;
    const JacPairItem it = items[blockIdx.x];
    if (done[it.blk]) return;
    const htn_svd_block D = desc[large_ids[it.blk]];
    const int m = D.m, tid = threadIdx.x, lane = tid & 63, wave = tid >> 6, l15 = lane & 15, l4 = lane >> 4;
    const int gsx = m <= 16 * JAC_MAXEL ? 16 : (m <= 32 * JAC_MAXEL ? 32 : 64);
    const int mp = gsx * ((m + gsx - 1) / gsx);
    const int ldp = mp + 1;
    double2* __restrict__ X = Vj + D.v_off;
    const int mode = it.pad[0], nrounds = mode ? 7 : 8;
    double2* P = g_lds;
    double2* GU = g_lds + 16 * ldp;
    const double z2 = zero2[it.blk];
    const double tol2 = tol * tol;
    if (tid == 0) s_rbits = 0ull;
    {
        const int c = tid >> 4, r = tid & 15;
        const bool live = c < 8 ? c < it.ni : c - 8 < it.nj;
        const int col = c < 8 ? it.ci + c : it.cj + (c - 8);
        const double2* __restrict__ src = X + (int64_t)(live ? col : 0) * mp;
        double2* dst = P + c * ldp;
        const int ne = mp >> 4;
        for (int e0 = 0; e0 < ne; e0 += 16) {
            double2 v[16];
#pragma unroll
            for (int e = 0; e < 16; ++e) {
                const int row = r + 16 * (e0 + e);
                v[e] = (live && e0 + e < ne) ? src[row] : make_double2(0.0, 0.0);
            }
#pragma unroll
// ... 103 lines not shown
                gn.x = pd ? dg : (po ? 0.0 : gn.x);
                gn.y = (pd || po) ? 0.0 : gn.y;
            }
            t2 = cmul(uijb, jpj);
            Gn[ei * JG_LD + ej] = gn;
            Un[ei * JG_LD + ej] = make_double2(fma(cj, uij.x, t2.x), fma(cj, uij.y, t2.y));
            __syncthreads();
            cur ^= 1;
        }
    }
    {
        const double2* Uc = GU + (2 + cur) * 16 * JG_LD;
        double ur[4], ui[4], nui[4];
#pragma unroll
        for (int kk = 0; kk < 4; ++kk) {
            const double2 u = Uc[(4 * kk + l4) * JG_LD + l15];
            ur[kk] = u.x;
            ui[kk] = u.y;
            nui[kk] = -u.y;
        }
        int colg[4];
#pragma unroll
        for (int r = 0; r < 4; ++r) {
            const int b = l4 + 4 * r;
            colg[r] = b < 8 ? (b < it.ni ? it.ci + b : -1) : (b - 8 < it.nj ? it.cj + (b - 8) : -1);
        }
        const int nrt = mp >> 4;
        const double2* pb = P + l4 * ldp + l15;
        double2 pn[4];
#pragma unroll
        for (int kk = 0; kk < 4; ++kk) pn[kk] = wave < nrt ? pb[4 * kk * ldp + wave * 16] : make_double2(0.0, 0.0);
        for (int rt = wave; rt < nrt; rt += 4) {
            const int i0 = rt * 16;
            double2 p[4];
#pragma unroll
            for (int kk = 0; kk < 4; ++kk) p[kk] = pn[kk];
            if (rt + 4 < nrt) {
#pragma unroll
                for (int kk = 0; kk < 4; ++kk) pn[kk] = pb[4 * kk * ldp + i0 + 64];
            }
            d4 ar = {0.0, 0.0, 0.0, 0.0}, ai = {0.0, 0.0, 0.0, 0.0};
#pragma unroll
            for (int kk = 0; kk < 4; ++kk) {
                ar = __builtin_amdgcn_mfma_f64_16x16x4f64(ur[kk], p[kk].x, ar, 0, 0, 0);
                ai = __builtin_amdgcn_mfma_f64_16x16x4f64(ur[kk], p[kk].y, ai, 0, 0, 0);
                ar = __builtin_amdgcn_mfma_f64_16x16x4f64(nui[kk], p[kk].y, ar, 0, 0, 0);
                ai = __builtin_amdgcn_mfma_f64_16x16x4f64(ui[kk], p[kk].x, ai, 0, 0, 0);
            }
#pragma unroll
            for (int r = 0; r < 4; ++r)
                if (colg[r] >= 0) X[(int64_t)colg[r] * mp + i0 + l15] = make_double2(ar[r], ai[r]);
        }
    }
    if (tid == 0) atomicMax(&ratio_bits[it.blk], first_bits);
}

__global__ void k_jacobi_check(unsigned long long* __restrict__ ratio_bits, int* __restrict__ done,
                               int* __restrict__ sweeps, int nl, double thr, int* __restrict__ active_out) {
    __shared__ int s_active;
    if (threadIdx.x == 0) s_active = 0;
    __syncthreads();
    for (int li = threadIdx.x; li < nl; li += blockDim.x) {
        if (!done[li]) {
            const double mx = __longlong_as_double((long long)ratio_bits[li]);
            sweeps[li] += 1;
            if (mx <= thr) done[li] = 1;
            else atomicAdd(&s_active, 1);
        }
        ratio_bits[li] = 0ull;
    }
    __syncthreads();
    if (threadIdx.x == 0) {
        *active_out = s_active;
        __threadfence_system();
    }
}

__global__ __launch_bounds__(JAC_THREADS) void k_jacobi_finish(double2* __restrict__ G, const double2* __restrict__ Vj,
                                                               double* __restrict__ S,
                                                               const htn_svd_block* __restrict__ desc,
                                                               const int* __restrict__ large_ids,
                                                               const int* __restrict__ perm,
                                                               const int* __restrict__ sweeps,
                                                               const int* __restrict__ done, int* __restrict__ info) {
    const int b = large_ids[blockIdx.x];
    const htn_svd_block D = desc[b];
    const int m = D.m, n = D.n, tid = threadIdx.x, lane = tid & 63, wave = tid >> 6;
    const int gsx = m <= 16 * JAC_MAXEL ? 16 : (m <= 32 * JAC_MAXEL ? 32 : 64);
    const int mp = gsx * ((m + gsx - 1) / gsx);
    const double2* __restrict__ X = Vj + D.v_off;
    double2* __restrict__ g = G + D.g_off;
    const int* __restrict__ pc = perm + blockIdx.x * 64 * JAC_MAXEL;
    for (int j = wave; j < n; j += JAC_THREADS / 64) {
        double sn = 0.0;
        for (int i = lane; i < m; i += 64) {
            const double2 x = X[(int64_t)j * mp + i];
            sn += x.x * x.x + x.y * x.y;
            g[(int64_t)j * m + pc[i]] = x;
        }
        sn = wave_sum(sn);
        if (lane == 0) S[D.s_off + j] = sqrt(sn);
    }
    if (tid == 0) info[b] = done[blockIdx.x] ? sweeps[blockIdx.x] : -sweeps[blockIdx.x];
}

#define TALL_THREADS 512
#define TALL_WAVES (TALL_THREADS / 64)
#define TALL_DEPTH 8
#define TALL_PARTS 32

__device__ __forceinline__ int tall_col(const JacPairItem& it, int q) {
    return q < 8 ? (q < it.ni ? it.ci + q : -1) : (q - 8 < it.nj ? it.cj + (q - 8) : -1);
}

__device__ __forceinline__ void tall_apply(double2* A, int64_t ld, int rows, const double2* Uc, const JacPairItem& it,
                                           int wave, int l15, int l4) {
    double ur[4], ui[4], nui[4];
    int colk[4], colg[4];
#pragma unroll
    for (int kk = 0; kk < 4; ++kk) {
        const double2 u = Uc[(4 * kk + l4) * JG_LD + l15];
        ur[kk] = u.x;
        ui[kk] = u.y;
        nui[kk] = -u.y;
        colk[kk] = tall_col(it, 4 * kk + l4);
        colg[kk] = tall_col(it, l4 + 4 * kk);
    }
    const int nrt = (rows + 15) >> 4;
    for (int rt0 = wave; rt0 < nrt; rt0 += TALL_WAVES * (TALL_DEPTH / 4)) {
        double2 p[TALL_DEPTH / 4][4];
#pragma unroll
        for (int t = 0; t < TALL_DEPTH / 4; ++t) {
            const int row = (rt0 + t * TALL_WAVES) * 16 + l15;
#pragma unroll
            for (int kk = 0; kk < 4; ++kk)
                p[t][kk] = (colk[kk] >= 0 && row < rows) ? A[(int64_t)colk[kk] * ld + row] : make_double2(0.0, 0.0);
        }
#pragma unroll
        for (int t = 0; t < TALL_DEPTH / 4; ++t) {
            const int row = (rt0 + t * TALL_WAVES) * 16 + l15;
            d4 ar = {0.0, 0.0, 0.0, 0.0}, ai = {0.0, 0.0, 0.0, 0.0};
#pragma unroll
            for (int kk = 0; kk < 4; ++kk) {
                ar = __builtin_amdgcn_mfma_f64_16x16x4f64(ur[kk], p[t][kk].x, ar, 0, 0, 0);
                ai = __builtin_amdgcn_mfma_f64_16x16x4f64(ur[kk], p[t][kk].y, ai, 0, 0, 0);
                ar = __builtin_amdgcn_mfma_f64_16x16x4f64(nui[kk], p[t][kk].y, ar, 0, 0, 0);
                ai = __builtin_amdgcn_mfma_f64_16x16x4f64(ui[kk], p[t][kk].x, ai, 0, 0, 0);
            }
            if (row < rows) {
#pragma unroll
                for (int r = 0; r < 4; ++r)
                    if (colg[r] >= 0) A[(int64_t)colg[r] * ld + row] = make_double2(ar[r], ai[r]);
            }
        }
    }
}

__global__ __launch_bounds__(TALL_THREADS) void k_jacobi_tall_visit(double2* __restrict__ G, double2* __restrict__ Vj,
                                                                    const htn_svd_block* __restrict__ desc,
                                                                    const int* __restrict__ tall_ids,
                                                                    const JacPairItem* __restrict__ items,
                                                                    const double* __restrict__ zero2,
                                                                    unsigned long long* __restrict__ ratio_bits,
                                                                    const int* __restrict__ done, double tol) {
    __shared__ double s_part[TALL_WAVES * 64 * JG_PS];
    __shared__ double2 GU[4 * 16 * JG_LD];
    __shared__ unsigned long long s_rbits;
    const JacPairItem it = items[blockIdx.x];
    if (done[it.blk]) return;
    const htn_svd_block D = desc[tall_ids[it.blk]];
    const int m = D.m, n = D.n, tid = threadIdx.x, lane = tid & 63, wave = tid >> 6, l15 = lane & 15, l4 = lane >> 4;
    double2* X = G + D.g_off;
    const int mode = it.pad[0], nrounds = mode ? 7 : 8;
    const double z2 = zero2[it.blk];
    const double tol2 = tol * tol;
    if (tid == 0) s_rbits = 0ull;
    {
        d4 g1 = {0.0, 0.0, 0.0, 0.0}, g2 = {0.0, 0.0, 0.0, 0.0}, mm = {0.0, 0.0, 0.0, 0.0};
        const int col = tall_col(it, l15);
        const double2* src = X + (int64_t)(col >= 0 ? col : 0) * m;
        const int nks = (m + 3) >> 2, per = (nks + TALL_WAVES - 1) / TALL_WAVES;
        const int ks0 = wave * per, ks1 = min(nks, ks0 + per);
        for (int ks = ks0; ks < ks1; ks += TALL_DEPTH) {
            double2 v[TALL_DEPTH];
#pragma unroll
            for (int u = 0; u < TALL_DEPTH; ++u) {
// ... 58 lines not shown
    int cur = 0;
    for (int r = 0; r < nrounds; ++r) {
        const double2* Gc = GU + cur * 16 * JG_LD;
        const double2* Uc = GU + (2 + cur) * 16 * JG_LD;
        double2* Gn = GU + (cur ^ 1) * 16 * JG_LD;
        double2* Un = GU + (2 + (cur ^ 1)) * 16 * JG_LD;
        const int ib = jg_partner(ei, r, mode), jb = jg_partner(ej, r, mode);
        const int ilo = ei < ib ? ei : ib, ihi = ei < ib ? ib : ei;
        const int jlo = ej < jb ? ej : jb, jhi = ej < jb ? jb : ej;
        const double iaa = Gc[ilo * JG_LD + ilo].x, ibb = Gc[ihi * JG_LD + ihi].x;
        const double2 ig = Gc[ilo * JG_LD + ihi];
        const double jaa = Gc[jlo * JG_LD + jlo].x, jbb = Gc[jhi * JG_LD + jhi].x;
        const double2 jg = Gc[jlo * JG_LD + jhi];
        const double2 gij = Gc[ei * JG_LD + ej], gijb = Gc[ei * JG_LD + jb];
        const double2 gibj = Gc[ib * JG_LD + ej], gibjb = Gc[ib * JG_LD + jb];
        const double2 uij = Uc[ei * JG_LD + ej], uijb = Uc[ei * JG_LD + jb];
        double ci, cqi, dqi, cj, cqj, dqj;
        const bool oni = jg_rotation(iaa, ibb, ig, ((livemask >> ilo) & (livemask >> ihi) & 1u) != 0, z2, tol2, ci, cqi, dqi);
        jg_rotation(jaa, jbb, jg, ((livemask >> jlo) & (livemask >> jhi) & 1u) != 0, z2, tol2, cj, cqj, dqj);
        const double2 jpj = ej == jlo ? make_double2(-cqj * jg.x, cqj * jg.y) : make_double2(cqj * jg.x, cqj * jg.y);
        const double2 ipi = ei == ilo ? make_double2(-cqi * ig.x, cqi * ig.y) : make_double2(cqi * ig.x, cqi * ig.y);
        double2 t2 = cmul(gijb, jpj);
        const double2 Tij = make_double2(fma(cj, gij.x, t2.x), fma(cj, gij.y, t2.y));
        t2 = cmul(gibjb, jpj);
        const double2 Tibj = make_double2(fma(cj, gibj.x, t2.x), fma(cj, gibj.y, t2.y));
        t2 = cmulc(ipi, Tibj);
        double2 gn = make_double2(fma(ci, Tij.x, t2.x), fma(ci, Tij.y, t2.y));
        {
            const double dg = ei == ilo ? iaa - dqi : ibb + dqi;
            const bool pd = oni && ej == ei, po = oni && ej == ib;
            gn.x = pd ? dg : (po ? 0.0 : gn.x);
            gn.y = (pd || po) ? 0.0 : gn.y;
        }
        t2 = cmul(uijb, jpj);
        if (el) {
            Gn[ei * JG_LD + ej] = gn;
            Un[ei * JG_LD + ej] = make_double2(fma(cj, uij.x, t2.x), fma(cj, uij.y, t2.y));
        }
        __syncthreads();
        cur ^= 1;
    }
    const double2* Uf = GU + (2 + cur) * 16 * JG_LD;
    tall_apply(X, m, m, Uf, it, wave, l15, l4);
    if (D.flags & HTN_SVD_ACCUMULATE) tall_apply(Vj + D.v_off, n, n, Uf, it, wave, l15, l4);
    if (tid == 0) atomicMax(&ratio_bits[it.blk], first_bits);
}

__global__ __launch_bounds__(256) void k_jacobi_tall_init(double2* __restrict__ G, double2* __restrict__ Vj,
                                                          const htn_svd_block* __restrict__ desc,
                                                          const int* __restrict__ tall_ids, double* __restrict__ part) {
    __shared__ double s_w[4];
    const htn_svd_block D = desc[tall_ids[blockIdx.x]];
    const int m = D.m, n = D.n, tid = threadIdx.x, lane = tid & 63, wave = tid >> 6;
    const double2* __restrict__ X = G + D.g_off;
    double f = 0.0;
    for (int j = blockIdx.y; j < n; j += TALL_PARTS)
        for (int i = tid; i < m; i += 256) {
            const double2 x = X[(int64_t)j * m + i];
            f += x.x * x.x + x.y * x.y;
        }
    if (D.flags & HTN_SVD_ACCUMULATE) {
        double2* __restrict__ J = Vj + D.v_off;
        for (int j = blockIdx.y; j < n; j += TALL_PARTS)
            for (int i = tid; i < n; i += 256) J[(int64_t)j * n + i] = make_double2(i == j ? 1.0 : 0.0, 0.0);
    }
    f = wave_sum(f);
    if (lane == 0) s_w[wave] = f;
    __syncthreads();
    if (tid == 0) part[blockIdx.x * TALL_PARTS + blockIdx.y] = (s_w[0] + s_w[1]) + (s_w[2] + s_w[3]);
}

__global__ void k_jacobi_tall_zero(const double* __restrict__ part, double* __restrict__ zero2, int nt) {
    for (int li = threadIdx.x; li < nt; li += blockDim.x) {
        double t = 0.0;
        for (int q = 0; q < TALL_PARTS; ++q) t += part[li * TALL_PARTS + q];
        zero2[li] = 1e-30 * t;
    }
}

__global__ __launch_bounds__(256) void k_jacobi_tall_finish(const double2* __restrict__ G, double* __restrict__ S,
                                                            const htn_svd_block* __restrict__ desc,
                                                            const int* __restrict__ tall_ids,
                                                            const int* __restrict__ sweeps, const int* __restrict__ done,
                                                            int* __restrict__ info) {
    const int b = tall_ids[blockIdx.y];
    const htn_svd_block D = desc[b];
    const int m = D.m, tid = threadIdx.x, lane = tid & 63, wave = tid >> 6;
    const int j = blockIdx.x * 4 + wave;
    if (j < D.n) {
        const double2* __restrict__ x = G + D.g_off + (int64_t)j * m;
        double sn = 0.0;
        for (int i = lane; i < m; i += 64) sn += x[i].x * x[i].x + x[i].y * x[i].y;
        sn = wave_sum(sn);
        if (lane == 0) S[D.s_off + j] = sqrt(sn);
    }
    if (blockIdx.x == 0 && tid == 0) info[b] = done[blockIdx.y] ? sweeps[blockIdx.y] : -sweeps[blockIdx.y];
}

#define RING_THREADS 512
#define RING_PANEL_ELEMS 4608
#define RING_MAX_P 64
struct RingItem {
    int32_t li;
    int32_t k, P;
    int32_t w;
    int32_t n;
    int32_t g0;
    int64_t mbox;
};
typedef unsigned int ring_u4 __attribute__((ext_vector_type(4)));
__host__ __device__ __forceinline__ int ring_gs(int m) { return m <= 256 ? 16 : 64; }
__host__ __device__ __forceinline__ int ring_e(int m) {
    const int g = ring_gs(m);
    return (m + g - 1) / g;
}
__device__ __forceinline__ bool ring_wait_ge(unsigned* flag, unsigned want, unsigned* fail) {
    const long long t0 = wall_clock64();
    for (unsigned spins = 1;; ++spins) {
        if (__hip_atomic_load(flag, __ATOMIC_RELAXED, __HIP_MEMORY_SCOPE_AGENT) >= want) return true;
        __builtin_amdgcn_s_sleep(1);
        if ((spins & 255u) == 0u) {
            if (__hip_atomic_load(fail, __ATOMIC_RELAXED, __HIP_MEMORY_SCOPE_AGENT) != 0u) return false;
            if (wall_clock64() - t0 > 300000000ll) {
                __hip_atomic_store(fail, 1u, __ATOMIC_RELAXED, __HIP_MEMORY_SCOPE_AGENT);
                return false;
            }
        }
    }
}

__device__ __forceinline__ void ring_send(const double2* __restrict__ src, double2* slot, int cnt, int tid, bool local) {
    const __amdgpu_buffer_rsrc_t rs = __builtin_amdgcn_make_buffer_rsrc((void*)slot, 0, cnt * 16, 0x00020000);
    if (local) {
        for (int idx = tid; idx < cnt; idx += RING_THREADS) {
            const double2 v = src[idx];
            ring_u4 u;
            __builtin_memcpy(&u, &v, 16);
            __builtin_amdgcn_raw_buffer_store_b128(u, rs, idx * 16, 0, 0);
        }
    } else {
        for (int idx = tid; idx < cnt; idx += RING_THREADS) {
            const double2 v = src[idx];
            ring_u4 u;
            __builtin_memcpy(&u, &v, 16);
            __builtin_amdgcn_raw_buffer_store_b128(u, rs, idx * 16, 0, 16);
        }
    }
}
__device__ __forceinline__ void ring_flag(unsigned* flag, unsigned epoch, bool local) {
    if (local) __hip_atomic_store(flag, epoch, __ATOMIC_RELAXED, __HIP_MEMORY_SCOPE_WORKGROUP);
    else __hip_atomic_store(flag, epoch, __ATOMIC_RELAXED, __HIP_MEMORY_SCOPE_AGENT);
}
__device__ __forceinline__ void ring_recv(double2* dst, const double2* slot, int cnt, int tid) {
    const __amdgpu_buffer_rsrc_t rs = __builtin_amdgcn_make_buffer_rsrc((void*)slot, 0, cnt * 16, 0x00020000);
#define RING_LD(q) const ring_u4 u##q = __builtin_amdgcn_raw_buffer_load_b128(rs, (tid + q * RING_THREADS) * 16, 0, 16)
    RING_LD(0);
    RING_LD(1);
    RING_LD(2);
    RING_LD(3);
    RING_LD(4);
    RING_LD(5);
    RING_LD(6);
    RING_LD(7);
    RING_LD(8);
#undef RING_LD
    auto put = [&](int idx, ring_u4 u) {
        if (idx < cnt) {
            double2 v;
            __builtin_memcpy(&v, &u, 16);
            dst[idx] = v;
        }
    };
    put(tid + 0 * RING_THREADS, u0);
    put(tid + 1 * RING_THREADS, u1);
    put(tid + 2 * RING_THREADS, u2);
    put(tid + 3 * RING_THREADS, u3);
    put(tid + 4 * RING_THREADS, u4);
    put(tid + 5 * RING_THREADS, u5);
    put(tid + 6 * RING_THREADS, u6);
// ... 222 lines not shown
    if (own) {
#pragma unroll
        for (int e = 0; e < E; ++e) T[grp * mp + sub + GS * e] = make_double2(a[e].x * sa, a[e].y * sa);
    }
    if (grp < nb) {
        const double sb = bscale[grp];
        if (sb != 1.0) {
            double2* bc = B + grp * mp + sub;
#pragma unroll
            for (int e = 0; e < E; ++e) {
                const double2 v = bc[GS * e];
                bc[GS * e] = make_double2(v.x * sb, v.y * sb);
            }
        }
    }
    __syncthreads();
    return ratio;
}

template <int GS, int E>
__device__ __forceinline__ double ring_intra(double2* T, int nt, double2* B, int nb, int tid, double tol2, double zero2) {
    constexpr int mp = GS * E;
    const int grp = tid / GS, sub = tid % GS;
    const int npT = nt + (nt & 1), npB = nb + (nb & 1), hT = npT >> 1, hB = npB >> 1;
    const int steps = (npT > npB ? npT : npB) - 1;
    double ratio = 0.0;
    for (int r = 0; r < steps; ++r) {
        double2* base = nullptr;
        int np = 0, pn = 0, p = 0;
        if (grp < hT) base = T, np = npT, pn = nt, p = grp;
        else if (grp < hT + hB) base = B, np = npB, pn = nb, p = grp - hT;
        if (base && r < np - 1) {
            const int md = np - 1;
            int i, j;
            if (p == 0) i = np - 1, j = r;
            else {
                i = r + p;
                i = i >= md ? i - md : i;
                j = r + md - p;
                j = j >= md ? j - md : j;
            }
            if (i < pn && j < pn) {
                const int lo = i < j ? i : j, hi = i < j ? j : i;
                const double rr = jacobi_pair_pad<GS, E>(base + lo * mp, base + hi * mp, sub, tol2, zero2);
                ratio = rr > ratio ? rr : ratio;
            }
        }
        __syncthreads();
    }
    return ratio;
}

#ifdef HTN_RING_PROF
__device__ long long g_ring_prof[256 * 16];
extern "C" int htn_ring_prof_dump(long long* out) {
    HIP_TRY(hipDeviceSynchronize());
    HIP_TRY(hipMemcpyFromSymbol(out, HIP_SYMBOL(g_ring_prof), sizeof(long long) * 256 * 16));
    return 0;
}
#define RING_T(var) const long long var = wall_clock64()
#define RING_ACC(slot, a, b) prof[slot] += (b) - (a)
#else
#define RING_T(var)
#define RING_ACC(slot, a, b)
#endif
struct RingArgs {
    double2* Vj;
    double2* G;
    double* S;
    const htn_svd_block* desc;
    const int* large_ids;
    const RingItem* items;
    const int* perm;
    const double* zero2;
    double2* mbox;
    unsigned* sync;
    int arrive_off, fail_off, conv_off;
    int xcc_off;
    int max_sweeps;
    int two_partner;
    double tol;
    int* info;
    int* sweeps_out;
};

template <int GS, int E>
__device__ __forceinline__ void ring_run(const RingArgs A, const RingItem it, const htn_svd_block D, double2* lds, int* s_top, int* s_bot,
                         unsigned long long* s_rbits, int* s_ok, double* s_bnorm, int* s_local) {
    constexpr int mp = GS * E;
    const int tid = threadIdx.x, lane = tid & 63, wave = tid >> 6;
    const int P = it.P, k = it.k, w = it.w, n = it.n, m = D.m;
    double2* __restrict__ X = A.Vj + D.v_off;
    const int slot_elems = w * mp;
    double2* bufT = lds;
    double2* bufB = lds + slot_elems;
    unsigned* flags = A.sync;
    unsigned* fail = A.sync + A.fail_off;
    const double zero2 = A.zero2[it.li];
    const double tol2 = A.tol * A.tol, thr = fmax(tol2, 0.1 * A.tol);
    auto ncols = [&](int q) {
        const int c = n - q * w;
        return c < 0 ? 0 : (c > w ? w : c);
    };
    if (tid < P) {
        s_top[tid] = 2 * tid;
        s_bot[tid] = 2 * tid + 1;
    }
    if (tid == 0) {
        *s_ok = 1;
        int local = 0;
        if (P > 1 && A.xcc_off >= 0) {
            unsigned xcc;
            asm volatile("s_getreg_b32 %0, hwreg(HW_REG_XCC_ID)" : "=s"(xcc));
            xcc = (xcc & 0xfu) + 1u;
            unsigned* xw = A.sync + A.xcc_off + it.g0;
            __hip_atomic_store(xw + k, xcc, __ATOMIC_RELAXED, __HIP_MEMORY_SCOPE_AGENT);
            local = 1;
            for (int q = 0; q < P && local >= 0; ++q) {
                if (!ring_wait_ge(xw + q, 1u, fail)) local = -1;
                else if (__hip_atomic_load(xw + q, __ATOMIC_RELAXED, __HIP_MEMORY_SCOPE_AGENT) != xcc) local = local > 0 ? 0 : local;
            }
            if (local < 0) *s_ok = 0;
        }
        *s_local = local > 0 ? 1 : 0;
    }
    __syncthreads();
    const bool local = *s_local != 0;
    {
        const int gsx = m <= 16 * JAC_MAXEL ? 16 : (m <= 32 * JAC_MAXEL ? 32 : 64);
        const int ldx = gsx * ((m + gsx - 1) / gsx);
        for (int side = 0; side < 2; ++side) {
            const int q = side ? s_bot[k] : s_top[k];
            double2* buf = side ? bufB : bufT;
            const int cnt = ncols(q) * mp;
            for (int idx = tid; idx < cnt; idx += RING_THREADS) {
                const int c = idx / mp, i = idx - c * mp;
                buf[idx] = i < m ? X[(int64_t)(q * w + c) * ldx + i] : make_double2(0.0, 0.0);
            }
        }
    }
    __syncthreads();
#ifdef HTN_RING_PROF
    long long prof[16] = {0, 0, 0, 0, 0, 0, 0, 0, 0, 0, 0, 0, 0, 0, 0, 0};
    const long long prof_t0 = wall_clock64();
    long long prof_c0;
    asm volatile("s_memtime %0\n\ts_waitcnt lgkmcnt(0)" : "=s"(prof_c0)::"memory");
#endif
    long long* split = nullptr;
#ifdef HTN_RING_STEP_PROF
    split = prof + 8;
#endif
    int sweeps = 0;
    bool done = n < 2, ok = *s_ok != 0;
    const int rounds = 2 * P - 1;
    while (!done && ok && sweeps < A.max_sweeps) {
        double ratio = 0.0;
        for (int r = 0; r < rounds && ok; ++r) {
            const unsigned epoch = (unsigned)(sweeps * rounds + r + 1);
            const int par = (int)(epoch & 1u);
            const int nt = ncols(s_top[k]), nb = ncols(s_bot[k]);
            RING_T(p0);
            double rr;
            if constexpr (GS == 16) {
                if (A.two_partner) rr = ring_cross<GS, E, true>(bufT, bufB, nt, nb, tid, tol2, zero2, s_bnorm, s_bnorm + RING_THREADS / 16, split);
                else rr = ring_cross<GS, E, false>(bufT, bufB, nt, nb, tid, tol2, zero2, s_bnorm, s_bnorm + RING_THREADS / 16, split);
            } else {
// ... 29 lines not shown
                if (good && k < P - 1) good = ring_wait_ge(flags + (it.g0 + k) * 2 + 1, epoch, fail);
                if (!good) *s_ok = 0;
            }
            if (k == P - 1) {
                double2* t = bufT;
                bufT = bufB;
                bufB = t;
            }
            __syncthreads();
            RING_T(p3);
            RING_ACC(2, p2, p3);
            ok = *s_ok != 0;
            if (ok) {
                const double2* mine = box + (int64_t)(k * 4) * slot_elems;
                if (k > 0) ring_recv(bufT, mine + (int64_t)(0 * 2 + par) * slot_elems, ncols(s_top[k]) * mp, tid);
                if (k < P - 1) ring_recv(bufB, mine + (int64_t)(1 * 2 + par) * slot_elems, ncols(s_bot[k]) * mp, tid);
            }
            __syncthreads();
            RING_T(p4);
            RING_ACC(3, p3, p4);
        }
        if (!ok) break;
        RING_T(p5);
        {
            const double rr = ring_intra<GS, E>(bufT, ncols(s_top[k]), bufB, ncols(s_bot[k]), tid, tol2, zero2);
            ratio = rr > ratio ? rr : ratio;
        }
        RING_T(p6);
        RING_ACC(4, p5, p6);
        if (tid == 0) *s_rbits = 0ull;
        __syncthreads();
        {
            const unsigned long long key = wave_max_u64((unsigned long long)__double_as_longlong(ratio));
            if (lane == 0 && key) atomicMax(s_rbits, key);
        }
        __syncthreads();
        if (tid == 0) {
            unsigned long long* conv = (unsigned long long*)(A.sync + A.conv_off) + (int64_t)it.li * A.max_sweeps + sweeps;
            unsigned* arrive = A.sync + A.arrive_off + it.li * A.max_sweeps + sweeps;
            unsigned long long mx = *s_rbits;
            if (P > 1) {
                const unsigned long long old = __hip_atomic_fetch_max(conv, mx, __ATOMIC_RELAXED, __HIP_MEMORY_SCOPE_AGENT);
                asm volatile("s_waitcnt vmcnt(0)" ::: "memory");
                (void)old;
                __hip_atomic_fetch_add(arrive, 1u, __ATOMIC_RELAXED, __HIP_MEMORY_SCOPE_AGENT);
                if (ring_wait_ge(arrive, (unsigned)P, fail)) mx = __hip_atomic_load(conv, __ATOMIC_RELAXED, __HIP_MEMORY_SCOPE_AGENT);
                else *s_ok = 0;
            }
            *s_rbits = mx;
        }
        __syncthreads();
        ok = *s_ok != 0;
        ++sweeps;
        done = __longlong_as_double((long long)*s_rbits) <= thr;
        __syncthreads();
        RING_T(p7);
        RING_ACC(5, p6, p7);
    }
#ifdef HTN_RING_PROF
    if (tid == 0 && blockIdx.x < 256) {
        prof[6] = wall_clock64() - prof_t0;
        prof[7] = (local ? 1000000 : 0) + sweeps * 1000 + P;
        long long prof_c1;
        asm volatile("s_memtime %0\n\ts_waitcnt lgkmcnt(0)" : "=s"(prof_c1)::"memory");
        prof[15] = prof_c1 - prof_c0;
        for (int q = 0; q < 16; ++q) g_ring_prof[blockIdx.x * 16 + q] = prof[q];
    }
#endif
    double2* __restrict__ g = A.G + D.g_off;
    const int* __restrict__ pc = A.perm + it.li * 64 * JAC_MAXEL;
    for (int side = 0; side < 2; ++side) {
        const double2* buf = side ? bufB : bufT;
        const int q = side ? s_bot[k] : s_top[k];
        const int nc = ncols(q);
        for (int c = wave; c < nc; c += RING_THREADS / 64) {
            const int col = q * w + c;
            double sn = 0.0;
            for (int i = lane; i < m; i += 64) {
                const double2 x = buf[c * mp + i];
                sn += x.x * x.x + x.y * x.y;
                g[(int64_t)col * m + pc[i]] = x;
            }
            sn = wave_sum(sn);
            if (lane == 0) A.S[D.s_off + col] = sqrt(sn);
        }
    }
    for (int col = n + k * (RING_THREADS / 64) + wave; col < D.n; col += P * (RING_THREADS / 64)) {
        for (int i = lane; i < m; i += 64) g[(int64_t)col * m + i] = make_double2(0.0, 0.0);
        if (lane == 0) A.S[D.s_off + col] = 0.0;
    }
    if (k == 0 && tid == 0) {
        A.info[A.large_ids[it.li]] = (done && ok) ? sweeps : -(sweeps > 0 ? sweeps : 1);
        A.sweeps_out[it.li] = ok ? sweeps + ((local || P == 1) ? 1000 : 0) : 0;
        __threadfence_system();
    }
}

__global__ __launch_bounds__(RING_THREADS) void k_jacobi_ring(RingArgs A) {
    extern __shared__ double2 g_lds[];
    __shared__ int s_top[RING_MAX_P], s_bot[RING_MAX_P];
    __shared__ unsigned long long s_rbits;
    __shared__ int s_ok, s_local;
    __shared__ double s_bnorm[2 * (RING_THREADS / 16)];
    const RingItem it = A.items[blockIdx.x];
    if (it.P <= 0) return;
    const htn_svd_block D = A.desc[A.large_ids[it.li]];
    const int m = D.m;
    const int gs = ring_gs(m), E = ring_e(m);
#define RING_CASE(GSV, EV) \
    case EV: ring_run<GSV, EV>(A, it, D, g_lds, s_top, s_bot, &s_rbits, &s_ok, s_bnorm, &s_local); break;
    if (gs == 16) {
        switch (E) {
            RING_CASE(16, 1) RING_CASE(16, 2) RING_CASE(16, 3) RING_CASE(16, 4) RING_CASE(16, 5) RING_CASE(16, 6) RING_CASE(16, 7)
            RING_CASE(16, 8) RING_CASE(16, 9) RING_CASE(16, 10) RING_CASE(16, 11) RING_CASE(16, 12) RING_CASE(16, 13)
            RING_CASE(16, 14) RING_CASE(16, 15)
            default: ring_run<16, 16>(A, it, D, g_lds, s_top, s_bot, &s_rbits, &s_ok, s_bnorm, &s_local);
        }
    } else {
        switch (E) {
            RING_CASE(64, 5) RING_CASE(64, 6) RING_CASE(64, 7)
            default: ring_run<64, 8>(A, it, D, g_lds, s_top, s_bot, &s_rbits, &s_ok, s_bnorm, &s_local);
        }
    }
#undef RING_CASE
}

struct JacScratch {
    int device = -1;
    int cu_count = 0;
    int xcd_local = 0;
    HtnBuf dev{HTN_BUF_DEVICE};
    HtnBuf pinned{HTN_BUF_PINNED};
    HtnBuf flags{HTN_BUF_MAPPED};
    HtnBuf ring_sync{HTN_BUF_DEVICE, false};
    HtnBuf ring_items{HTN_BUF_DEVICE, false};
    HtnBuf ring_items_h{HTN_BUF_PINNED};
    HtnBuf ring_mbox{HTN_BUF_DEVICE};
    HtnBuf qr_box{HTN_BUF_DEVICE};
    HtnBuf tall_dev{HTN_BUF_DEVICE};
    HtnBuf tall_pin{HTN_BUF_PINNED};
    HtnBuf tall_flags{HTN_BUF_MAPPED};
    hipStream_t aux = nullptr;
    hipEvent_t ev_fork = nullptr, ev_join = nullptr, ev_sweep[2] = {nullptr, nullptr};
    ~JacScratch() {
        if (device >= 0) (void)hipSetDevice(device);
        if (aux) {
            (void)hipStreamSynchronize(aux);
            (void)hipStreamDestroy(aux);
        }
        for (hipEvent_t ev : {ev_fork, ev_join, ev_sweep[0], ev_sweep[1]})
            if (ev) (void)hipEventDestroy(ev);
    }
};
static HtnStreamRegistry<JacScratch> g_js_res;

void htn_svd_release_stream(hipStream_t st) { g_js_res.release(st); }

static int js_get(hipStream_t st, JacScratch** out) {
    return g_js_res.get(st, out, [](JacScratch& js) -> int {
        HIP_TRY(hipDeviceGetAttribute(&js.cu_count, hipDeviceAttributeMultiprocessorCount, js.device));
        HIP_TRY(hipStreamCreateWithFlags(&js.aux, hipStreamNonBlocking));
        HIP_TRY(hipEventCreateWithFlags(&js.ev_fork, hipEventDisableTiming));
        HIP_TRY(hipEventCreateWithFlags(&js.ev_join, hipEventDisableTiming));
        HIP_TRY(hipEventCreateWithFlags(&js.ev_sweep[0], hipEventDisableTiming));
        HIP_TRY(hipEventCreateWithFlags(&js.ev_sweep[1], hipEventDisableTiming));
        return 0;
    });
}

struct JacTournament {
    std::vector<JacPairItem> items;
    std::vector<size_t> off;
    int n_rounds() const { return (int)off.size() - 1; }
    unsigned round_size(int r) const { return (unsigned)(off[r + 1] - off[r]); }
};
static JacTournament jacobi_tournament(const int* n_cols, int n_blk) {
    const int w = JAC_PANEL;
    std::vector<std::vector<JacPairItem>> rounds;
    std::vector<JacPairItem> intra;
    for (int li = 0; li < n_blk; ++li) {
        const int n = n_cols[li];
        if (n < 1) continue;
        const int nb = (n + w - 1) / w;
        const int nbp = nb + (nb & 1);
        if ((int)rounds.size() < nbp - 1) rounds.resize(nbp - 1);
        for (int r = 0; r < nbp - 1; ++r)
            for (int p = 0; p < nbp / 2; ++p) {
                int a = p == 0 ? nbp - 1 : (r + p) % (nbp - 1);
                int c = p == 0 ? r : (r + nbp - 1 - p) % (nbp - 1);
                if (a >= nb || c >= nb) continue;
                if (a > c) std::swap(a, c);
                JacPairItem it = {li, a * w, std::min(w, n - a * w), c * w, std::min(w, n - c * w), {0, 0, 0}};
                rounds[r].push_back(it);
            }
        for (int a = 0; a < nb; a += 2) {
            const int c = a + 1;
            JacPairItem it = {li, a * w, std::min(w, n - a * w), c < nb ? c * w : 0,
                              c < nb ? std::min(w, n - c * w) : 0, {1, 0, 0}};
            intra.push_back(it);
        }
    }
    rounds.push_back(intra);
    JacTournament T;
    for (auto& rl : rounds) {
        T.off.push_back(T.items.size());
        T.items.insert(T.items.end(), rl.begin(), rl.end());
    }
    T.off.push_back(T.items.size());
    return T;
}
static int upload_tournament(const JacTournament& T, JacPairItem* h_items, JacPairItem* d_items, hipStream_t st) {
    if (T.items.empty()) return 0;
    memcpy(h_items, T.items.data(), sizeof(JacPairItem) * T.items.size());
    HIP_TRY(hipMemcpyAsync(d_items, h_items, sizeof(JacPairItem) * T.items.size(), hipMemcpyHostToDevice, st));
    return 0;
}

template <class Enqueue>
static int jacobi_sweep_pipeline(int max_sweeps, int hint, hipEvent_t* ev_sweep, const volatile int* h_active,
                                 hipStream_t st, Enqueue enqueue) {
    hipError_t err = hipSuccess;
    int enq = 0, used = 0;
    auto enqueue_next = [&]() {
        enqueue(enq);
        err = hipEventRecord(ev_sweep[enq & 1], st);
        ++enq;
    };
    if (max_sweeps > 0) enqueue_next();
    for (int sweep = 0; sweep < max_sweeps && err == hipSuccess; ++sweep) {
        const bool expect_last = hint > 0 && sweep + 1 >= hint;
        if (sweep + 1 < max_sweeps && !expect_last && enq == sweep + 1) enqueue_next();
        if (err == hipSuccess) err = htn_event_spin(ev_sweep[sweep & 1]);
        if (err != hipSuccess) break;
        used = sweep + 1;
        if (h_active[sweep] == 0) break;
        if (sweep + 1 < max_sweeps && enq == sweep + 1) enqueue_next();
    }
    return err == hipSuccess ? used : -htn_fail("jacobi_sweep_pipeline", err);
}

struct JacCall {
    double2 *G, *Vj;
    double* S;
    const htn_svd_block *desc, *desc_host;
    int n_blocks, max_sweeps;
    double tol, cut2;
    int split;
    int32_t* info_dev;
    hipStream_t st;
    std::vector<int> large;
    std::vector<int> n_eff;
    int nl() const { return (int)large.size(); }
};
static int jac_padded_rows(int m) {
    const int gsx = m <= 16 * JAC_MAXEL ? 16 : (m <= 32 * JAC_MAXEL ? 32 : 64);
    return gsx * ((m + gsx - 1) / gsx);
}
static const int JAC_LDS_ELEMS = 9216;

static int jac_set_kernel_attributes() {
    static std::mutex attr_mu;
    static bool attr_set[64] = {};
    int dev = 0;
    HIP_TRY(hipGetDevice(&dev));
    std::lock_guard<std::mutex> lk(attr_mu);
    if (dev >= 0 && dev < 64 && !attr_set[dev]) {
        HIP_TRY(hipFuncSetAttribute((const void*)k_jacobi_svd, hipFuncAttributeMaxDynamicSharedMemorySize,
                                    JAC_LDS_ELEMS * (int)sizeof(double2)));
        HIP_TRY(hipFuncSetAttribute((const void*)k_qr_large, hipFuncAttributeMaxDynamicSharedMemorySize,
                                    16 * (64 * JAC_MAXEL + 1) * (int)sizeof(double2)));
        HIP_TRY(hipFuncSetAttribute((const void*)k_jacobi_pairs_gram, hipFuncAttributeMaxDynamicSharedMemorySize,
                                    (16 * (64 * JAC_MAXEL + 1) + JG_GU_ELEMS) * (int)sizeof(double2)));
        HIP_TRY(hipFuncSetAttribute((const void*)k_jacobi_ring, hipFuncAttributeMaxDynamicSharedMemorySize,
                                    2 * RING_PANEL_ELEMS * (int)sizeof(double2)));
        attr_set[dev] = true;
    }
    return 0;
}

static std::vector<int> classify_large(const htn_svd_block* desc_host, int n_blocks, int split) {
    const int large_min = split > 0 ? std::min(split, JAC_LDS_ELEMS) : JAC_LDS_ELEMS;
    std::vector<int> large;
    if (desc_host)
        for (int b = 0; b < n_blocks; ++b) {
            const htn_svd_block& D = desc_host[b];
            if (!(D.flags & HTN_SVD_QRCP) || D.n < 2) continue;
            if ((int64_t)jac_padded_rows(D.m) * D.n > large_min) large.push_back(b);
        }
    return large;
}

struct JacCoreBufs {
    int *d_ids, *d_slot, *d_perm;
    double* d_zero;
    unsigned long long* d_ratio;
    int *d_done, *d_sw;
    unsigned* d_qsync;
    JacPairItem* d_items;
    JacPairItem* h_items;
    int *h_ids, *h_slot;
    volatile int *h_active, *h_rank, *h_ring_sw;
    int *d_active, *d_rank, *d_ring_sw;
};
static int carve_core_scratch(JacScratch& js, int nl, int n_blocks, int max_sweeps, size_t n_items_max, JacCoreBufs* B) {
    const size_t off_ids = 0, off_slot = off_ids + sizeof(int) * nl, off_perm = off_slot + sizeof(int) * n_blocks;
    const size_t off_zero = off_perm + sizeof(int) * nl * 64 * JAC_MAXEL;
    const size_t off_ratio = (off_zero + sizeof(double) * nl + 7) / 8 * 8, off_done = off_ratio + 8 * nl;
    const size_t off_sw = off_done + sizeof(int) * nl, off_qsync = off_sw + sizeof(int) * nl;
    const size_t off_items = (off_qsync + sizeof(unsigned) * (QR_SYNC_WORDS * (size_t)nl + 8) + 31) / 32 * 32;
    if (js.dev.reserve(off_items + sizeof(JacPairItem) * n_items_max)) return 1;
    if (js.pinned.reserve(sizeof(JacPairItem) * n_items_max + 4 * (size_t)(nl + n_blocks) + 128)) return 1;
    if (js.flags.reserve(sizeof(int) * ((size_t)(max_sweeps + 1) + 2 * (size_t)nl + 16))) return 1;
    char* d = (char*)js.dev.p;
    B->d_ids = (int*)(d + off_ids);
    B->d_slot = (int*)(d + off_slot);
    B->d_perm = (int*)(d + off_perm);
    B->d_zero = (double*)(d + off_zero);
    B->d_ratio = (unsigned long long*)(d + off_ratio);
    B->d_done = (int*)(d + off_done);
    B->d_sw = (int*)(d + off_sw);
    B->d_qsync = (unsigned*)(d + off_qsync);
    B->d_items = (JacPairItem*)(d + off_items);
    char* h = (char*)js.pinned.p;
    B->h_items = (JacPairItem*)h;
    B->h_ids = (int*)(h + sizeof(JacPairItem) * n_items_max);
    B->h_slot = B->h_ids + nl;
    B->h_active = (volatile int*)js.flags.p;
    B->h_rank = B->h_active + (max_sweeps + 1);
    B->h_ring_sw = B->h_rank + nl;
    B->d_active = (int*)js.flags.dev;
    B->d_rank = B->d_active + (max_sweeps + 1);
    B->d_ring_sw = B->d_rank + nl;
// ... 33 lines not shown
    const int lane_cap = ring_cap / nx;
    while (left) {
        const int first = (int)plan->items.size();
        std::vector<int> lane_used((size_t)nx, 0);
        struct Put {
            int q, x, s0;
        };
        std::vector<Put> puts;
        for (size_t q = 0; q < blks.size(); ++q) {
            if (placed[q]) continue;
            int x = 0;
            for (int y = 1; y < nx; ++y)
                if (lane_used[y] < lane_used[x]) x = y;
            if (lane_used[x] + blks[q].P > lane_cap) continue;
            puts.push_back({(int)q, x, lane_used[x]});
            lane_used[x] += blks[q].P;
            placed[q] = 1;
            --left;
        }
        int depth = 0;
        for (int y = 0; y < nx; ++y) depth = std::max(depth, lane_used[y]);
        const int grid = depth * nx;
        plan->items.resize((size_t)first + grid, RingItem{0, 0, 0, 0, 0, 0, 0});
        for (const Put& pt : puts) {
            const Blk& B = blks[pt.q];
            for (int k = 0; k < B.P; ++k)
                plan->items[(size_t)first + (size_t)(pt.s0 + k) * nx + pt.x] = {B.li, k, B.P, B.w, c.n_eff[B.li], plan->wgs,
                                                                                 plan->mbox_elems};
            plan->mbox_elems += (int64_t)B.P * 4 * B.w * B.mp;
            plan->wgs += B.P;
        }
        plan->batches.push_back({first, grid});
    }
    return true;
}

static int launch_qr_large(const JacCall& c, JacScratch& js, const JacCoreBufs& B, int n_xcd) {
    const int nl = c.nl();
    int max_m0 = 0, min_m0 = 1 << 30, max_n0 = 0;
    for (int b : c.large) {
        max_m0 = std::max(max_m0, (int)c.desc_host[b].pad);
        min_m0 = std::min(min_m0, (int)c.desc_host[b].pad);
        max_n0 = std::max(max_n0, (int)c.desc_host[b].m);
    }
    const size_t qr_panel_elems = (size_t)16 * (((max_m0 + 15) & ~15) + 1);
    const bool coop = ((min_m0 + 15) & ~15) <= 256 && qr_panel_elems * sizeof(double2) + 65536 + 30720 <= 163840;
    const size_t qr_lds = qr_panel_elems * sizeof(double2) + (coop ? 65536 : 0);
    static const bool qr_single = htn_env_flag("HTN_QR_SINGLE");
    static const int env_nw = getenv("HTN_QR_NW") ? atoi(getenv("HTN_QR_NW")) : 0;
    int NW = qr_single ? 1 : ((max_n0 >= 160 || js.xcd_local) ? 4 : 1);
    if (env_nw > 0 && !qr_single) NW = std::min(env_nw, 4);
    const int cus = std::max(1, std::min(js.cu_count > 0 ? js.cu_count : 256, 256));
    const int qnx = (NW > 1 && n_xcd > 1) ? n_xcd : 1;
    const int nl_pad = (nl + qnx - 1) / qnx * qnx;
    NW = std::max(1, std::min(NW, cus / std::max(nl_pad, 1)));
    if (NW > 1 && js.qr_box.reserve((size_t)nl * QR_BOX_BYTES)) return 1;
    const int qgrid_nx = NW > 1 ? qnx : 1;
    hipLaunchKernelGGL(k_qr_large, dim3((NW > 1 ? nl_pad : nl) * NW), dim3(JAC_THREADS), qr_lds, c.st, c.G, c.Vj, c.desc, B.d_ids,
                       B.d_perm, B.d_zero, c.cut2, B.d_rank, NW, (char*)js.qr_box.p, B.d_qsync, nl, qgrid_nx,
                       coop ? (int)qr_panel_elems : 0);
    return 0;
}

static int run_ring(const JacCall& c, JacScratch& js, const JacCoreBufs& B, const RingPlan& plan, int n_xcd, bool two_partner,
                    int32_t* sweeps_used) {
    const int nl = c.nl(), n_wg = plan.wgs, n_items = (int)plan.items.size();
    const int arrive_off = 2 * n_wg, fail_off = arrive_off + nl * c.max_sweeps, xcc_off = fail_off + 1;
    const int conv_off = (xcc_off + n_wg + 3) & ~3;
    const size_t sync_bytes = ((size_t)conv_off * 4 + (size_t)nl * c.max_sweeps * 8 + 15) & ~(size_t)15;
    if (js.ring_sync.reserve(sync_bytes)) return 1;
    if (js.ring_mbox.reserve(sizeof(double2) * (size_t)std::max<int64_t>(plan.mbox_elems, 1))) return 1;
    if (js.ring_items.reserve(sizeof(RingItem) * n_items) || js.ring_items_h.reserve(sizeof(RingItem) * n_items)) return 1;
    memcpy(js.ring_items_h.p, plan.items.data(), sizeof(RingItem) * n_items);
    for (int li = 0; li < nl; ++li) B.h_ring_sw[li] = 0;
    HIP_TRY(hipMemcpyAsync(js.ring_items.p, js.ring_items_h.p, sizeof(RingItem) * n_items, hipMemcpyHostToDevice, c.st));
    HIP_TRY(hipMemsetAsync(js.ring_sync.p, 0, sync_bytes, c.st));
    RingArgs ra;
    ra.Vj = c.Vj, ra.G = c.G, ra.S = c.S, ra.desc = c.desc, ra.large_ids = B.d_ids;
    ra.perm = B.d_perm, ra.zero2 = B.d_zero, ra.mbox = (double2*)js.ring_mbox.p, ra.sync = (unsigned*)js.ring_sync.p;
    ra.arrive_off = arrive_off, ra.fail_off = fail_off, ra.conv_off = conv_off, ra.max_sweeps = c.max_sweeps, ra.tol = c.tol;
    ra.xcc_off = xcc_off;
    ra.two_partner = two_partner ? 1 : 0;
    ra.info = c.info_dev, ra.sweeps_out = B.d_ring_sw;
    for (auto& bt : plan.batches) {
        ra.items = (const RingItem*)js.ring_items.p + bt.first;
        hipLaunchKernelGGL(k_jacobi_ring, dim3((unsigned)bt.second), dim3(RING_THREADS), 2 * RING_PANEL_ELEMS * sizeof(double2),
                           c.st, ra);
    }
    HIP_TRY(hipGetLastError());
    HIP_TRY(hipStreamWaitEvent(c.st, js.ev_join, 0));
    HIP_TRY(htn_stream_spin(c.st));
    int used = 0;
    for (int li = 0; li < nl; ++li) {
        if (B.h_rank[li] < 0) return fail_msg("htn_jacobi_svd_z: a hand-off of the multi-workgroup QR timed out");
        if (B.h_ring_sw[li] <= 0 && c.n_eff[li] >= 2)
            return fail_msg("htn_jacobi_svd_z: a hand-off of the ring Jacobi kernel timed out");
        used = std::max(used, (int)B.h_ring_sw[li] % 1000);
    }
    int all_local = n_xcd > 1 ? 1 : 0;
    for (int li = 0; li < nl; ++li)
        if (c.n_eff[li] >= 2 && B.h_ring_sw[li] < 1000) all_local = 0;
    js.xcd_local = all_local;
    if (sweeps_used) *sweeps_used = used;
    return 0;
}

static int run_pair_visits(const JacCall& c, JacScratch& js, const JacCoreBufs& B, const JacTournament& T, int hint,
                           int32_t* sweeps_used) {
    const int nl = c.nl();
    int max_mp = 0;
    for (int b : c.large) max_mp = std::max(max_mp, jac_padded_rows(c.desc_host[b].m));
    const size_t gram_lds_bytes = (size_t)(16 * (max_mp + 1) + JG_GU_ELEMS) * sizeof(double2);
    const double thr = std::max(c.tol * c.tol, 0.1 * c.tol);
    const int used = jacobi_sweep_pipeline(c.max_sweeps, hint, js.ev_sweep, B.h_active, c.st, [&](int sweep) {
        for (int r = 0; r < T.n_rounds(); ++r)
            if (T.round_size(r))
                hipLaunchKernelGGL(k_jacobi_pairs_gram, dim3(T.round_size(r)), dim3(256), gram_lds_bytes, c.st, c.Vj, c.desc,
                                   B.d_ids, B.d_items + T.off[r], B.d_zero, B.d_ratio, B.d_done, c.tol, 1);
        hipLaunchKernelGGL(k_jacobi_check, dim3(1), dim3(64), 0, c.st, B.d_ratio, B.d_done, B.d_sw, nl, thr, B.d_active + sweep);
    });
    if (used < 0) return 1;
    if (sweeps_used) *sweeps_used = used;
    HIP_TRY(hipStreamWaitEvent(c.st, js.ev_join, 0));
    hipLaunchKernelGGL(k_jacobi_finish, dim3(nl), dim3(JAC_THREADS), 0, c.st, c.G, (const double2*)c.Vj, c.S, c.desc, B.d_ids,
                       B.d_perm, B.d_sw, B.d_done, c.info_dev);
    HIP_TRY(hipGetLastError());
    HIP_TRY(htn_stream_spin(c.st));
    return 0;
}

static int jacobi_svd_core(void* G, void* Vj, double* S, const htn_svd_block* desc, const htn_svd_block* desc_host,
                           int32_t n_blocks, int32_t max_m_host, int32_t max_sweeps, double tol, int32_t* info_dev,
                           const htn_svd_opts* opts, void* stream, const int* skip_dev, const unsigned char* skip_host) {
    if (n_blocks <= 0) return 0;
    if (max_m_host > 64 * JAC_MAXEL) return fail_msg("htn_jacobi_svd_z: block taller than 512 rows");
    const double rank_cut = opts && opts->rank_cut > 0.0 ? opts->rank_cut : 0.0;
    JacCall c = {(double2*)G, (double2*)Vj, S, desc, desc_host, n_blocks, max_sweeps, tol, rank_cut * rank_cut,
                 opts && opts->split_elems > 0 ? opts->split_elems : 0, info_dev, (hipStream_t)stream, {}, {}};
    int32_t* sweeps_used = opts ? opts->sweeps_used : nullptr;
    if (jac_set_kernel_attributes()) return 1;
    c.large = classify_large(desc_host, n_blocks, c.split);
    if (sweeps_used) *sweeps_used = 0;
    if (c.large.empty()) {
        hipLaunchKernelGGL(k_jacobi_svd, dim3(n_blocks), dim3(JAC_THREADS), JAC_LDS_ELEMS * sizeof(double2), c.st, c.G, c.Vj, S,
                           desc, max_sweeps, tol, info_dev, JAC_LDS_ELEMS, skip_dev, c.cut2);
        HIP_TRY(hipGetLastError());
        return 0;
    }
    const int nl = c.nl();
    size_t n_items_max = 0;
    for (int b : c.large) {
        const int nb = (desc_host[b].n + JAC_PANEL - 1) / JAC_PANEL, nbp = nb + (nb & 1);
        n_items_max += (size_t)(nbp - 1) * (nbp / 2) + (nb + 1) / 2;
        c.n_eff.push_back(desc_host[b].n);
    }
    JacScratch* jsp = nullptr;
    JacCoreBufs B;
    if (js_get(c.st, &jsp) || carve_core_scratch(*jsp, nl, n_blocks, max_sweeps, n_items_max, &B)) return 1;
    JacScratch& js = *jsp;
    for (int b = 0; b < n_blocks; ++b) B.h_slot[b] = skip_host && skip_host[b] ? nl : -1;
    for (int li = 0; li < nl; ++li) B.h_slot[c.large[li]] = li;
    for (int li = 0; li < nl; ++li) B.h_ids[li] = c.large[li];
    for (int k = 0; k <= max_sweeps; ++k) B.h_active[k] = 1;
    HIP_TRY(hipMemcpyAsync(B.d_ids, B.h_ids, sizeof(int) * (nl + n_blocks), hipMemcpyHostToDevice, c.st));
    HIP_TRY(hipMemsetAsync(B.d_ratio, 0, 16 * (size_t)nl + sizeof(unsigned) * (QR_SYNC_WORDS * (size_t)nl + 8), c.st));
    static const bool force_pairs = htn_env_flag("HTN_SVD_PAIRS");
    static const bool no_xcd = htn_env_flag("HTN_RING_NO_XCD");
    const bool ring_two_partner = htn_env_flag("HTN_RING_TWO_PARTNER");
    const int n_xcd = (!no_xcd && js.cu_count > 0 && js.cu_count % 8 == 0) ? 8 : 1;
    const int ring_cap = std::max(1, std::min(js.cu_count > 0 ? js.cu_count : 256, 256));
    RingPlan plan;
    JacTournament T;
    bool use_ring = !force_pairs && plan_ring(c, n_xcd, ring_cap, &plan);
    if (c.cut2 <= 0.0 && !use_ring) {
        T = jacobi_tournament(c.n_eff.data(), nl);
        if (upload_tournament(T, B.h_items, B.d_items, c.st)) return 1;
    }
    HIP_TRY(hipEventRecord(js.ev_fork, c.st));
    HIP_TRY(hipStreamWaitEvent(js.aux, js.ev_fork, 0));
    hipLaunchKernelGGL(k_jacobi_svd, dim3(n_blocks), dim3(JAC_THREADS), JAC_LDS_ELEMS * sizeof(double2), js.aux, c.G, c.Vj, S,
                       desc, max_sweeps, tol, info_dev, JAC_LDS_ELEMS, (const int*)B.d_slot, c.cut2);
    HIP_TRY(hipEventRecord(js.ev_join, js.aux));
    if (launch_qr_large(c, js, B, n_xcd)) return 1;
    if (c.cut2 > 0.0) {
        HIP_TRY(hipEventRecord(js.ev_sweep[0], c.st));
        HIP_TRY(htn_event_spin(js.ev_sweep[0]));
        for (int li = 0; li < nl; ++li) c.n_eff[li] = std::min(c.n_eff[li], (int)B.h_rank[li]);
        if (use_ring) use_ring = plan_ring(c, n_xcd, ring_cap, &plan);
        if (!use_ring) {
            T = jacobi_tournament(c.n_eff.data(), nl);
            if (upload_tournament(T, B.h_items, B.d_items, c.st)) return 1;
        }
    }
    if (use_ring) return run_ring(c, js, B, plan, n_xcd, ring_two_partner, sweeps_used);
    return run_pair_visits(c, js, B, T, opts && opts->sweeps_hint > 0 ? opts->sweeps_hint : 0, sweeps_used);
}

static int jacobi_svd_tall(void* G, void* Vj, double* S, const htn_svd_block* desc, const htn_svd_block* desc_host,
                           int32_t n_blocks, int32_t max_m_rest, int32_t max_sweeps, double tol, int32_t* info_dev,
                           const htn_svd_opts* opts, void* stream, const std::vector<int>& tall) {
    const int nt = (int)tall.size();
    hipStream_t st = (hipStream_t)stream;
    JacScratch* jsp = nullptr;
    if (js_get(st, &jsp)) return 1;
    JacScratch& js = *jsp;
    std::vector<int> n_cols(nt);
    for (int li = 0; li < nt; ++li) n_cols[li] = desc_host[tall[li]].n;
    const JacTournament T = jacobi_tournament(n_cols.data(), nt);
    const size_t n_items = T.items.size();
    const size_t off_skip = 0, off_ids = off_skip + sizeof(int) * n_blocks;
    const size_t off_zero = (off_ids + sizeof(int) * nt + 7) / 8 * 8, off_part = off_zero + sizeof(double) * nt;
    const size_t off_ratio = off_part + sizeof(double) * nt * TALL_PARTS, off_done = off_ratio + 8 * (size_t)nt;
    const size_t off_sw = off_done + sizeof(int) * nt, off_items = (off_sw + sizeof(int) * nt + 31) / 32 * 32;
    const size_t flag_elems = (size_t)std::max(max_sweeps, 0) + 1;
    if (js.tall_dev.reserve(off_items + sizeof(JacPairItem) * std::max<size_t>(n_items, 1))) return 1;
    if (js.tall_pin.reserve(sizeof(JacPairItem) * std::max<size_t>(n_items, 1) + sizeof(int) * (n_blocks + nt))) return 1;
    if (js.tall_flags.reserve(sizeof(int) * flag_elems)) return 1;
    char* d = (char*)js.tall_dev.p;
    int* d_skip = (int*)(d + off_skip);
    int* d_ids = (int*)(d + off_ids);
    double* d_zero = (double*)(d + off_zero);
    double* d_part = (double*)(d + off_part);
    unsigned long long* d_ratio = (unsigned long long*)(d + off_ratio);
    int* d_done = (int*)(d + off_done);
    int* d_sw = (int*)(d + off_sw);
    JacPairItem* d_items = (JacPairItem*)(d + off_items);
    JacPairItem* h_items = (JacPairItem*)js.tall_pin.p;
    int* h_skip = (int*)((char*)js.tall_pin.p + sizeof(JacPairItem) * std::max<size_t>(n_items, 1));
    int* h_ids = h_skip + n_blocks;
    volatile int* h_active = (volatile int*)js.tall_flags.p;
    int* d_active = (int*)js.tall_flags.dev;
    std::vector<unsigned char> skip(n_blocks, 0);
    for (int li = 0; li < nt; ++li) skip[tall[li]] = 1;
    for (int b = 0; b < n_blocks; ++b) h_skip[b] = skip[b] ? 0 : -1;
    for (int li = 0; li < nt; ++li) h_ids[li] = tall[li];
    for (size_t k = 0; k < flag_elems; ++k) h_active[k] = 1;
    HIP_TRY(hipMemcpyAsync(d_skip, h_skip, sizeof(int) * (n_blocks + nt), hipMemcpyHostToDevice, st));
    if (upload_tournament(T, h_items, d_items, st)) return 1;
    HIP_TRY(hipMemsetAsync(d_ratio, 0, 16 * (size_t)nt, st));
    int core_used = 0;
    if (nt < n_blocks) {
        if (jacobi_svd_core(G, Vj, S, desc, desc_host, n_blocks, max_m_rest, max_sweeps, tol, info_dev, opts, stream, d_skip,
                            skip.data()))
            return 1;
        if (opts && opts->sweeps_used) core_used = *opts->sweeps_used;
    }
    int max_n = 1;
    for (int li = 0; li < nt; ++li) max_n = std::max(max_n, (int)desc_host[tall[li]].n);
    hipLaunchKernelGGL(k_jacobi_tall_init, dim3(nt, TALL_PARTS), dim3(256), 0, st, (double2*)G, (double2*)Vj, desc, d_ids, d_part);
    hipLaunchKernelGGL(k_jacobi_tall_zero, dim3(1), dim3(64), 0, st, (const double*)d_part, d_zero, nt);
    HIP_TRY(hipGetLastError());
    const double thr = std::max(tol * tol, 0.1 * tol);
    const int hint = opts && opts->sweeps_hint > 0 ? opts->sweeps_hint : 0;
    const int used = jacobi_sweep_pipeline(max_sweeps, hint, js.ev_sweep, h_active, st, [&](int sweep) {
        for (int r = 0; r < T.n_rounds(); ++r)
            if (T.round_size(r))
                hipLaunchKernelGGL(k_jacobi_tall_visit, dim3(T.round_size(r)), dim3(TALL_THREADS), 0, st, (double2*)G,
                                   (double2*)Vj, desc, d_ids, d_items + T.off[r], d_zero, d_ratio, d_done, tol);
        hipLaunchKernelGGL(k_jacobi_check, dim3(1), dim3(64), 0, st, d_ratio, d_done, d_sw, nt, thr, d_active + sweep);
    });
    if (used < 0) return 1;
    hipLaunchKernelGGL(k_jacobi_tall_finish, dim3((unsigned)((max_n + 3) / 4), (unsigned)nt), dim3(256), 0, st,
                       (const double2*)G, S, desc, d_ids, d_sw, d_done, info_dev);
    HIP_TRY(hipGetLastError());
    HIP_TRY(htn_stream_spin(st));
    if (opts && opts->sweeps_used) *opts->sweeps_used = std::max(core_used, used);
    return 0;
}

extern "C" int htn_jacobi_svd_z(void* G, void* Vj, double* S, const htn_svd_block* desc,
                                const htn_svd_block* desc_host, int32_t n_blocks, int32_t max_m_host,
                                int32_t max_sweeps, double tol, int32_t* info_dev, const htn_svd_opts* opts,
                                void* stream) {
    if (n_blocks <= 0) return 0;
    std::vector<int> tall;
    int max_m_rest = 0;
    if (desc_host) {
        for (int b = 0; b < n_blocks; ++b) {
            const htn_svd_block& D = desc_host[b];
            if (!(D.flags & HTN_SVD_QRCP) && D.m > 64 * JAC_MAXEL) tall.push_back(b);
            else max_m_rest = std::max(max_m_rest, std::max(D.m, D.pad));
        }
    } else if (max_m_host > 64 * JAC_MAXEL) {
        return fail_msg("htn_jacobi_svd_z: blocks taller than 512 rows need the host copy of the descriptors (desc_host)");
    }
    if (tall.empty())
        return jacobi_svd_core(G, Vj, S, desc, desc_host, n_blocks, max_m_host, max_sweeps, tol, info_dev, opts, stream,
                               nullptr, nullptr);
    if (max_m_rest > 64 * JAC_MAXEL) return fail_msg("htn_jacobi_svd_z: block taller than 512 rows");
    return jacobi_svd_tall(G, Vj, S, desc, desc_host, n_blocks, max_m_rest, max_sweeps, tol, info_dev, opts, stream, tall);
}

__global__ __launch_bounds__(256) void k_batched_copy(double2* __restrict__ dst, const double2* __restrict__ src,
                                                      const int32_t* __restrict__ idx,
                                                      const double* __restrict__ scl,
                                                      const htn_copy_item* __restrict__ items, double gscale) {
    const htn_copy_item I = items[blockIdx.x];
    const int total = I.rows * I.cols;
    for (int e = blockIdx.y * blockDim.x + threadIdx.x; e < total; e += blockDim.x * gridDim.y) {
        const int i = e % I.rows, j = e / I.rows;
        int gi = i, gj = j;
        if (I.idx_off >= 0) {
            if (I.gather_dim == 0) gi = idx[I.idx_off + i];
            else gj = idx[I.idx_off + j];
        }
        double2 v;
        if (I.op == HTN_OP_N) v = src[I.src_off + (int64_t)gi + (int64_t)gj * I.lds];
        else {
            v = src[I.src_off + (int64_t)gj + (int64_t)gi * I.lds];
            v.y = -v.y;
        }
        double f = gscale;
        if (I.scale_dim >= 0 && I.scl_off >= 0) {
            const double sv = scl[I.scl_off + (I.scale_dim == 0 ? gi : gj)];
            f = I.inv_norm ? (sv > 0.0 ? f / sv : 0.0) : f * sv;
        }
        dst[I.dst_off + (int64_t)i + (int64_t)j * I.ldd] = make_double2(v.x * f, v.y * f);
    }
}

extern "C" int htn_batched_copy_z(void* dst, const void* src, const int32_t* idx, const double* scl,
                                  const htn_copy_item* items, int32_t n_items, double global_scale,
                                  void* stream) {
    if (n_items <= 0) return 0;
    hipLaunchKernelGGL(k_batched_copy, dim3(n_items, 16), dim3(256), 0, (hipStream_t)stream, (double2*)dst,
                       (const double2*)src, idx, scl, items, global_scale);
    HIP_TRY(hipGetLastError());
    return 0;
}
```

include/hubbardtn_hip.h:

```cpp
#ifndef HUBBARDTN_HIP_H
#define HUBBARDTN_HIP_H

#include <stdint.h>

#ifdef __cplusplus
extern "C" {
#endif

#define HTN_ABI_VERSION 2
#define HTN_MAX_BUFS 8
#define HTN_TILE 32

#define HTN_OP_N 0
#define HTN_OP_T 1
#define HTN_OP_C 2
#define HTN_SEG_GEMM 0
#define HTN_SEG_COPY 1

typedef struct {
    int64_t c_off;
    int32_t buf_c;
    int32_t ldc;
    int32_t m, n;
    int32_t row0, col0;
    int32_t seg_begin, seg_count;
    int32_t pad[2];
    int32_t part, nparts;
    int32_t ws_slot;
    int32_t ticket;
} htn_tile;
#define HTN_BUF_WS 7
#define HTN_WS_TICKET_ELEMS 4096
#define HTN_WS_ELEMS(n_slots) (HTN_WS_TICKET_ELEMS + (int64_t)(n_slots) * HTN_TILE * HTN_TILE)

typedef struct {
    int64_t a_off, b_off;
    int32_t buf_a, buf_b;
    int32_t lda, ldb;
    int32_t k;
    int32_t op_a, op_b;
    int32_t type;
    double alpha_re, alpha_im;
} htn_seg;

const char* htn_last_error(void);
int htn_abi_version(void);

int htn_device_init(int device, char* name_host, int* cu_count_host);

int htn_grouped_gemm_z(const void* const* bufs_host, const htn_tile* tiles, int32_t n_tiles,
                       const htn_seg* segs, void* stream);

int64_t htn_dots_scratch_elems(int32_t nvec);
int htn_dots_z(const void* V, int64_t ldv, int32_t nvec, const void* w, int64_t n,
               void* out, void* scratch, void* stream);
int htn_axpys_z(void* w, const void* V, int64_t ldv, int32_t nvec, const void* coef,
                double sign, int64_t n, void* stream);
int htn_scale_inv_sqrt_z(void* dst, const void* src, const void* nrm2, int64_t n, void* stream);

typedef struct {
    const void* bufs[HTN_MAX_BUFS];
    const htn_tile* tiles;
    const htn_seg* segs;
    int32_t n_tiles;
    int32_t pad;
} htn_gemm_launch;
typedef int (*htn_exchange2_fn)(void* y_dev, int64_t n, void* user);
int64_t htn_lanczos_scratch_elems(int32_t krylovdim);
int htn_lanczos_z(const htn_gemm_launch* stages_host, int32_t n_stages, int32_t x_slot, int32_t y_slot,
                  void* V, int64_t n, int32_t krylovdim, double tol, int32_t max_restart, void* scratch,
                  int32_t zero_y, htn_exchange2_fn exchange, void* user,
                  double* eig_host, int32_t* n_matvec_host, double* residual_host,
                  double* matvec_ms_host ,
                  void* stream);
int htn_lanczos_orth_z(const htn_gemm_launch* stages_host, int32_t n_stages, int32_t x_slot, int32_t y_slot,
                       void* V, int64_t n, int32_t krylovdim, double tol, int32_t max_restart, void* scratch,
                       int32_t zero_y, htn_exchange2_fn exchange, void* user,
                       double* eig_host, int32_t* n_matvec_host, double* residual_host, double* matvec_ms_host,
                       const void* Q, int32_t n_frozen, void* stream);

#define HTN_SVD_ACCUMULATE 1
#define HTN_SVD_QRCP 2
typedef struct {
    int64_t g_off, v_off, s_off;
    int32_t m, n;
    int32_t flags, pad;
} htn_svd_block;
typedef struct {
    int32_t split_elems;
    int32_t sweeps_hint;
    double rank_cut;
    int32_t* sweeps_used;
} htn_svd_opts;
int htn_jacobi_svd_z(void* G, void* Vj, double* S, const htn_svd_block* desc, const htn_svd_block* desc_host,
                     int32_t n_blocks, int32_t max_m_host, int32_t max_sweeps, double tol, int32_t* info_dev,
                     const htn_svd_opts* opts, void* stream);

typedef struct {
    int64_t dst_off, src_off, idx_off, scl_off;
    int32_t rows, cols;
    int32_t ldd, lds;
    int32_t op;
    int32_t gather_dim;
    int32_t scale_dim;
    int32_t inv_norm;
} htn_copy_item;
int htn_batched_copy_z(void* dst, const void* src, const int32_t* idx, const double* scl,
                       const htn_copy_item* items, int32_t n_items, double global_scale,
                       void* stream);


typedef struct htn_ctx htn_ctx;
typedef struct htn_mpo htn_mpo;
typedef struct htn_mps htn_mps;

#define HTN_SYM_SU2_U1 0
#define HTN_SYM_U1_U1 1
#define HTN_SYM_SU2 2
#define HTN_MAX_SITE 4
typedef struct {
    int32_t kind;
    int32_t n_site;
    int32_t site_N[HTN_MAX_SITE];
    int32_t site_j[HTN_MAX_SITE];
} htn_symmetry;

typedef struct {
    int32_t k, dN;
    double red[HTN_MAX_SITE * HTN_MAX_SITE];
} htn_site_op;

typedef struct {
    int32_t wl, wr;
    int32_t op;
    int32_t pad;
    double coef_re, coef_im;
} htn_mpo_entry;

typedef struct {
    int32_t lN, lj, s, rN, rj;
    int32_t ld;
    int64_t off;
} htn_subblock;

typedef struct {
    int32_t N, j, count;
} htn_sector;

typedef struct {
    int32_t chi_full;
    int32_t weighting;
    double cutoff;
    int32_t krylovdim;
    int32_t maxrestart;
    double lanczos_tol;
    double jacobi_tol;
    int32_t jacobi_max_sweeps;
    int32_t svd_split_elems;
    double rank_cut;
    int32_t profile;
    int32_t pad;
} htn_sweep_opts;

typedef struct {
    int32_t bond, direction;
    int32_t n_matvec, jacobi_sweeps;
    int32_t chi_full, multiplets;
    int32_t n_tiles, n_segs;
    int64_t theta_size;
    int64_t apply_flops, apply_bytes, svd_flops;
    double energy, residual, trunc_weight;
    double t_plan, t_lanczos, t_svd, t_env, t_total;
    double matvec_ms;
} htn_bond_stats;

#define HTN_BACKEND_CPU 0
#define HTN_BACKEND_HIP 1
int htn_ctx_create(int32_t backend, int32_t device, void* stream, htn_ctx** out);
void htn_ctx_destroy(htn_ctx* ctx);
// ... 87 lines not shown
```

Baseline: 423.7 ms.

## Mirror SVD singular values to pinned host memory and fuse Ritz combine

```diff
diff --git a/hubbardtn_amd/abi.py b/hubbardtn_amd/abi.py
--- a/hubbardtn_amd/abi.py
+++ b/hubbardtn_amd/abi.py
@@ -84,7 +84,7 @@
 
 EXPORTS = ["htn_last_error", "htn_abi_version", "htn_device_init", "htn_grouped_gemm_z",
            "htn_dots_scratch_elems", "htn_dots_z", "htn_axpys_z", "htn_scale_inv_sqrt_z",
-           "htn_jacobi_svd_z", "htn_batched_copy_z", "htn_lanczos_scratch_elems", "htn_lanczos_z", "htn_lanczos_orth_z"]
+           "htn_jacobi_svd_z", "htn_jacobi_svd_host_values", "htn_batched_copy_z", "htn_lanczos_scratch_elems", "htn_lanczos_z", "htn_lanczos_orth_z"]
 ENGINE_EXPORTS = ["htn_ctx_create", "htn_ctx_destroy", "htn_ctx_backend", "htn_ctx_set_timing", "htn_comm_unique_id",
                   "htn_ctx_set_comm", "htn_ctx_set_exchange", "htn_mpo_create", "htn_mpo_destroy", "htn_mps_create",
                   "htn_mps_destroy", "htn_bond_update", "htn_dmrg2_sweep", "htn_mps_theta_size", "htn_heff2_apply",
@@ -130,6 +130,8 @@
     lib.htn_axpys_z.argtypes = [vp, vp, i64, i32, vp, f64, i64, vp]
     lib.htn_scale_inv_sqrt_z.argtypes = [vp, vp, vp, i64, vp]
     lib.htn_jacobi_svd_z.argtypes = [vp, vp, vp, vp, vp, i32, i32, i32, f64, vp, C.POINTER(SvdOpts), vp]
+    lib.htn_jacobi_svd_host_values.argtypes = [vp, C.POINTER(C.POINTER(f64)), C.POINTER(C.POINTER(i32)), C.POINTER(i64),
+                                               C.POINTER(i32)]
     lib.htn_batched_copy_z.argtypes = [vp, vp, vp, vp, vp, i32, f64, vp]
     lib.htn_lanczos_scratch_elems.argtypes = [i32]
     lib.htn_lanczos_scratch_elems.restype = i64
diff --git a/hubbardtn_amd/csrc/htn_backend_hip.hip b/hubbardtn_amd/csrc/htn_backend_hip.hip
--- a/hubbardtn_amd/csrc/htn_backend_hip.hip
+++ b/hubbardtn_amd/csrc/htn_backend_hip.hip
@@ -267,6 +267,13 @@
         fork_open = false;
         return rc;
     }
+    int svd_host_values(const double** S_host, const int32_t** info_host) override {
+        HtnSvdHostValues v;
+        if (htn_svd_host_values(st, &v)) return 1;
+        *S_host = v.S, *info_host = v.info;
+        if (v.S) stage_pos = 0;
+        return 0;
+    }
     int batched_copy(void* dst, const void* src, const int32_t* idx, const double* scl, const htn_copy_item* items, int n_items,
                      double gscale) override {
         return htn_batched_copy_z(dst, src, idx, scl, items, n_items, gscale, st);
diff --git a/hubbardtn_amd/csrc/htn_common.h b/hubbardtn_amd/csrc/htn_common.h
--- a/hubbardtn_amd/csrc/htn_common.h
+++ b/hubbardtn_amd/csrc/htn_common.h
@@ -149,6 +149,13 @@
 };
 void htn_krylov_release_stream(hipStream_t st);
 void htn_svd_release_stream(hipStream_t st);
+struct HtnSvdHostValues {
+    const double* S;
+    const int32_t* info;
+    int64_t s_elems;
+    int32_t n_blocks;
+};
+int htn_svd_host_values(hipStream_t st, HtnSvdHostValues* out);
 
 template <int CTRL>
 __device__ __forceinline__ double dpp_f64(double v) {
diff --git a/hubbardtn_amd/csrc/htn_core.h b/hubbardtn_amd/csrc/htn_core.h
--- a/hubbardtn_amd/csrc/htn_core.h
+++ b/hubbardtn_amd/csrc/htn_core.h
@@ -290,6 +290,10 @@
     virtual int jacobi_svd(void* G, void* Vj, double* S, const htn_svd_block* desc_dev, const htn_svd_block* desc_host,
                            int n_blocks, int max_m, int max_sweeps, double tol, int32_t* info_dev,
                            const htn_svd_opts* opts) = 0;
+    virtual int svd_host_values(const double** S_host, const int32_t** info_host) {
+        *S_host = nullptr, *info_host = nullptr;
+        return 0;
+    }
     virtual int batched_copy(void* dst, const void* src, const int32_t* idx, const double* scl,
                              const htn_copy_item* items_dev, int n_items, double gscale) = 0;
     virtual int scale(void* x, int64_t n, double f) = 0;
diff --git a/hubbardtn_amd/csrc/htn_engine.cpp b/hubbardtn_amd/csrc/htn_engine.cpp
--- a/hubbardtn_amd/csrc/htn_engine.cpp
+++ b/hubbardtn_amd/csrc/htn_engine.cpp
@@ -297,6 +297,9 @@
     std::map<int, std::pair<std::pair<int, double>, double>> cut_hint;
     std::map<int, int> sweeps_hint;
     std::vector<int32_t> idx_host;
+    std::vector<double> s_download;
+    std::vector<int> sv_order;
+    std::vector<std::pair<double, int>> sv_sort;
     std::vector<OrthState> orth;
     int orth_dropped = 0;
 
@@ -738,23 +741,31 @@
     if (jac_used > 0) sweeps_hint[i + 1] = jac_used;
     static const bool dbg_timers = getenv("HTN_DEBUG_HOST_TIMERS") != nullptr;
     const double tA = now();
-    std::vector<double> s_host(s_elems + (i_elems + 1) / 2);
-    if (be->download(s_host.data(), S->p, sizeof(double) * s_elems + sizeof(int32_t) * i_elems)) return 1;
+    const double* s_h = nullptr;
+    const int32_t* info_h = nullptr;
+    if (!svd_shard && be->svd_host_values(&s_h, &info_h)) return 1;
+    if (!s_h) {
+        s_download.resize(s_elems + (i_elems + 1) / 2);
+        if (be->download(s_download.data(), S->p, sizeof(double) * s_elems + sizeof(int32_t) * i_elems)) return 1;
+        s_h = s_download.data();
+        info_h = (const int32_t*)(s_download.data() + s_elems);
+    }
     const double tB = now();
-    const int32_t* info_h = (const int32_t*)(s_host.data() + s_elems);
     int jac_sweeps = 0;
     for (int b = 0; b < (svd_shard ? sc->n_own : nb); ++b) {
         if (info_h[b] < 0) return set_error("Jacobi SVD did not converge (bond %d, block %d, %d sweeps)", i + 1, b, -info_h[b]);
         jac_sweeps = std::max(jac_sweeps, (int)info_h[b]);
     }
     std::vector<int> lens(nb), qd(nb);
-    std::vector<std::vector<int>> order(nb);
+    std::vector<int>& order = sv_order;
+    order.clear();
     std::vector<double> vals;
     vals.reserve((size_t)sp.s_size);
-    std::vector<std::pair<double, int>> tmp;
+    order.reserve((size_t)sp.s_size);
+    std::vector<std::pair<double, int>>& tmp = sv_sort;
     for (int b = 0; b < nb; ++b) {
         const int len = sp.desc[b].n;
-        const double* sv = s_host.data() + sp.desc[b].s_off;
+        const double* sv = s_h + sp.desc[b].s_off;
         lens[b] = len;
         qd[b] = sym.qdim(sp.mids[b]);
         tmp.resize(len);
@@ -762,9 +773,8 @@
         std::sort(tmp.begin(), tmp.end(), [](const std::pair<double, int>& a, const std::pair<double, int>& c) {
             return a.first != c.first ? a.first > c.first : a.second < c.second;
         });
-        order[b].resize(len);
         for (int k = 0; k < len; ++k) {
-            order[b][k] = tmp[k].second;
+            order.push_back(tmp[k].second);
             vals.push_back(tmp[k].first);
         }
     }
@@ -818,8 +828,8 @@
     if (!fc) return 1;
     const double tD = now();
     idx_host.clear();
-    for (int b = 0; b < nb; ++b)
-        for (int k = 0; k < counts[b]; ++k) idx_host.push_back(order[b][k]);
+    for (int b = 0, p = 0; b < nb; p += lens[b], ++b)
+        for (int k = 0; k < counts[b]; ++k) idx_host.push_back(order[p + k]);
     DBufP idx_d = dalloc(sizeof(int32_t) * std::max<size_t>(idx_host.size(), 1));
     const int64_t sizeA = fc->layA->size, sizeB = fc->layB->size;
     DView out = zalloc(sizeA + sizeB, true);
diff --git a/hubbardtn_amd/csrc/htn_krylov.hip b/hubbardtn_amd/csrc/htn_krylov.hip
--- a/hubbardtn_amd/csrc/htn_krylov.hip
+++ b/hubbardtn_amd/csrc/htn_krylov.hip
@@ -399,6 +399,26 @@
     }
 }
 
+struct RitzCoef {
+    double2 c[DOT_CHUNK];
+};
+__global__ __launch_bounds__(256) void k_ritz_combine(double2* __restrict__ x, const double2* __restrict__ V, int64_t ldv,
+                                                      int nvec, RitzCoef coef, int64_t n) {
+    for (int64_t j = (int64_t)blockIdx.x * blockDim.x + threadIdx.x; j < n; j += (int64_t)gridDim.x * blockDim.x) {
+        double sr = 0.0, si = 0.0;
+        for (int i = 0; i < nvec; ++i) {
+            const double2 c = coef.c[i];
+            const double2 v = V[(int64_t)i * ldv + j];
+            sr += c.x * v.x - c.y * v.y;
+            si += c.x * v.y + c.y * v.x;
+        }
+        double2 r = make_double2(0.0, 0.0);
+        r.x += 1.0 * sr;
+        r.y += 1.0 * si;
+        x[j] = r;
+    }
+}
+
 __global__ __launch_bounds__(256) void k_scale_inv_sqrt(double2* __restrict__ dst, const double2* __restrict__ src,
                                                         const double2* __restrict__ nrm2, int64_t n) {
     const double s = 1.0 / sqrt(nrm2[0].x);
@@ -512,7 +532,6 @@
     int device = -1;
     LanRecord* h_rec = nullptr;
     LanRecord* d_rec = nullptr;
-    double2* h_y = nullptr;
     hipEvent_t ev_done[LAN_SLOTS], ev_mv0[LAN_SLOTS], ev_mv1[LAN_SLOTS];
     bool have_events = false;
     unsigned long long serial = 0;
@@ -520,7 +539,6 @@
     ~LanRes() {
         if (device >= 0) (void)hipSetDevice(device);
         if (h_rec) (void)hipHostFree(h_rec);
-        if (h_y) (void)hipHostFree(h_y);
         if (have_events)
             for (int i = 0; i < LAN_SLOTS; ++i) {
                 (void)hipEventDestroy(ev_done[i]);
@@ -536,7 +554,6 @@
         HIP_TRY(hipHostMalloc((void**)&r.h_rec, sizeof(LanRecord) * LAN_SLOTS, hipHostMallocMapped | hipHostMallocCoherent));
         memset(r.h_rec, 0, sizeof(LanRecord) * LAN_SLOTS);
         HIP_TRY(hipHostGetDevicePointer((void**)&r.d_rec, r.h_rec, 0));
-        HIP_TRY(hipHostMalloc((void**)&r.h_y, sizeof(double2) * LAN_SLOTS, hipHostMallocDefault));
         for (int i = 0; i < LAN_SLOTS; ++i) {
             HIP_TRY(hipEventCreateWithFlags(&r.ev_done[i], hipEventDisableTiming));
             HIP_TRY(hipEventCreate(&r.ev_mv0[i]));
@@ -563,8 +580,7 @@
     double2* partial2 = partial + (int64_t)(kt + 1) * DOT_BLOCKS;
     double2* c1 = partial2 + (int64_t)(kt + 1) * DOT_BLOCKS;
     double2* c2 = c1 + (kt + 1);
-    double2* ycoef = c2 + (kt + 1);
-    double* norm_partial = (double*)(ycoef + (kt + 1));
+    double* norm_partial = (double*)(c2 + 2 * (kt + 1));
 
     LanRes* R = nullptr;
     if (lan_res_get(st, &R)) return 1;
@@ -705,17 +721,15 @@
         }
         HIP_TRY(htn_stream_spin(st));
         const int k = (int)y.size();
-        for (int i = 0; i < k; ++i) R->h_y[i] = make_double2(y[i], 0.0);
-        HIP_TRY(hipMemcpyAsync(ycoef, R->h_y, sizeof(double2) * k, hipMemcpyHostToDevice, st));
+        RitzCoef yc;
+        for (int i = 0; i < DOT_CHUNK; ++i) yc.c[i] = make_double2(i < k ? y[i] : 0.0, 0.0);
         double2* xrow = V + (int64_t)(kd + 1) * n;
-        HIP_TRY(hipMemsetAsync(xrow, 0, sizeof(double2) * n, st));
-        hipLaunchKernelGGL(k_axpys, dim3(grid_for(n)), dim3(256), 0, st, xrow, V, n, k, ycoef, 1.0, n);
+        hipLaunchKernelGGL(k_ritz_combine, dim3(grid_for(n)), dim3(256), 0, st, xrow, (const double2*)V, n, k, yc, n);
         if (nf > 0) project_out(xrow);
         else
         hipLaunchKernelGGL(k_norm_partial, dim3(DOT_BLOCKS), dim3(DOT_THREADS), 0, st, xrow, n, norm_partial);
         hipLaunchKernelGGL(k_scale_by_norm, dim3(grid_for(n)), dim3(DOT_THREADS), 0, st, V, xrow, norm_partial, n,
                            (LanRecord*)nullptr, (const double2*)nullptr, (const double2*)nullptr, 0ull);
-        HIP_TRY(htn_stream_spin(st));
         if (res < tol || beta < 1e-14 * std::max(amax, 1e-300)) break;
     }
     HIP_TRY(hipGetLastError());
diff --git a/hubbardtn_amd/csrc/htn_svd.hip b/hubbardtn_amd/csrc/htn_svd.hip
--- a/hubbardtn_amd/csrc/htn_svd.hip
+++ b/hubbardtn_amd/csrc/htn_svd.hip
@@ -997,7 +997,8 @@
                                                             const htn_svd_block* __restrict__ desc,
                                                             int max_sweeps, double tol, int* __restrict__ info,
                                                             int lds_elems, const int* __restrict__ large_slot,
-                                                            double cut2) {
+                                                            double cut2, double* __restrict__ S_host,
+                                                            int* __restrict__ info_host) {
     extern __shared__ double2 g_lds[];
     __shared__ double s_ratio;
     __shared__ double s_piv[2];
@@ -1065,9 +1066,17 @@
                 gglob[(int64_t)j * m + s_col[i]] = x;
             }
             sn = wave_sum(sn);
-            if (lane == 0) S[D.s_off + j] = sqrt(sn);
-        }
-        if (tid == 0) info[blockIdx.x] = swq;
+            if (lane == 0) {
+                const double sv = sqrt(sn);
+                S[D.s_off + j] = sv;
+                if (S_host) S_host[D.s_off + j] = sv;
+            }
+        }
+        if (tid == 0) {
+            info[blockIdx.x] = swq;
+            if (info_host) info_host[blockIdx.x] = swq;
+        }
+        if (S_host && lane == 0) __threadfence_system();
         return;
     } else {
         if (accumulate)
@@ -1111,9 +1120,17 @@
             if (in_lds) gglob[(int64_t)j * m + i] = x;
         }
         s = wave_sum(s);
-        if (lane == 0) S[D.s_off + j] = sqrt(s);
-    }
-    if (tid == 0) info[blockIdx.x] = sw;
+        if (lane == 0) {
+            const double sv = sqrt(s);
+            S[D.s_off + j] = sv;
+            if (S_host) S_host[D.s_off + j] = sv;
+        }
+    }
+    if (tid == 0) {
+        info[blockIdx.x] = sw;
+        if (info_host) info_host[blockIdx.x] = sw;
+    }
+    if (S_host && lane == 0) __threadfence_system();
 }
 
 #define JAC_PANEL 8
@@ -1383,7 +1400,8 @@
                                                                const int* __restrict__ large_ids,
                                                                const int* __restrict__ perm,
                                                                const int* __restrict__ sweeps,
-                                                               const int* __restrict__ done, int* __restrict__ info) {
+                                                               const int* __restrict__ done, int* __restrict__ info,
+                                                               double* __restrict__ S_host, int* __restrict__ info_host) {
     const int b = large_ids[blockIdx.x];
     const htn_svd_block D = desc[b];
     const int m = D.m, n = D.n, tid = threadIdx.x, lane = tid & 63, wave = tid >> 6;
@@ -1400,9 +1418,18 @@
             g[(int64_t)j * m + pc[i]] = x;
         }
         sn = wave_sum(sn);
-        if (lane == 0) S[D.s_off + j] = sqrt(sn);
-    }
-    if (tid == 0) info[b] = done[blockIdx.x] ? sweeps[blockIdx.x] : -sweeps[blockIdx.x];
+        if (lane == 0) {
+            const double sv = sqrt(sn);
+            S[D.s_off + j] = sv;
+            if (S_host) S_host[D.s_off + j] = sv;
+        }
+    }
+    if (tid == 0) {
+        const int r = done[blockIdx.x] ? sweeps[blockIdx.x] : -sweeps[blockIdx.x];
+        info[b] = r;
+        if (info_host) info_host[b] = r;
+    }
+    if (S_host && lane == 0) __threadfence_system();
 }
 
 #define TALL_THREADS 512
@@ -1627,7 +1654,8 @@
                                                             const htn_svd_block* __restrict__ desc,
                                                             const int* __restrict__ tall_ids,
                                                             const int* __restrict__ sweeps, const int* __restrict__ done,
-                                                            int* __restrict__ info) {
+                                                            int* __restrict__ info, double* __restrict__ S_host,
+                                                            int* __restrict__ info_host) {
     const int b = tall_ids[blockIdx.y];
     const htn_svd_block D = desc[b];
     const int m = D.m, tid = threadIdx.x, lane = tid & 63, wave = tid >> 6;
@@ -1637,9 +1665,18 @@
         double sn = 0.0;
         for (int i = lane; i < m; i += 64) sn += x[i].x * x[i].x + x[i].y * x[i].y;
         sn = wave_sum(sn);
-        if (lane == 0) S[D.s_off + j] = sqrt(sn);
-    }
-    if (blockIdx.x == 0 && tid == 0) info[b] = done[blockIdx.y] ? sweeps[blockIdx.y] : -sweeps[blockIdx.y];
+        if (lane == 0) {
+            const double sv = sqrt(sn);
+            S[D.s_off + j] = sv;
+            if (S_host) S_host[D.s_off + j] = sv;
+        }
+    }
+    if (blockIdx.x == 0 && tid == 0) {
+        const int r = done[blockIdx.y] ? sweeps[blockIdx.y] : -sweeps[blockIdx.y];
+        info[b] = r;
+        if (info_host) info_host[b] = r;
+    }
+    if (S_host && lane == 0) __threadfence_system();
 }
 
 #define RING_THREADS 512
@@ -2028,6 +2065,8 @@
     double tol;
     int* info;
     int* sweeps_out;
+    double* S_host;
+    int* info_host;
 };
 
 template <int GS, int E>
@@ -2223,15 +2262,25 @@
                 g[(int64_t)col * m + pc[i]] = x;
             }
             sn = wave_sum(sn);
-            if (lane == 0) A.S[D.s_off + col] = sqrt(sn);
+            if (lane == 0) {
+                const double sv = sqrt(sn);
+                A.S[D.s_off + col] = sv;
+                if (A.S_host) A.S_host[D.s_off + col] = sv;
+            }
         }
     }
     for (int col = n + k * (RING_THREADS / 64) + wave; col < D.n; col += P * (RING_THREADS / 64)) {
         for (int i = lane; i < m; i += 64) g[(int64_t)col * m + i] = make_double2(0.0, 0.0);
-        if (lane == 0) A.S[D.s_off + col] = 0.0;
-    }
+        if (lane == 0) {
+            A.S[D.s_off + col] = 0.0;
+            if (A.S_host) A.S_host[D.s_off + col] = 0.0;
+        }
+    }
+    if (A.S_host && lane == 0) __threadfence_system();
     if (k == 0 && tid == 0) {
-        A.info[A.large_ids[it.li]] = (done && ok) ? sweeps : -(sweeps > 0 ? sweeps : 1);
+        const int r = (done && ok) ? sweeps : -(sweeps > 0 ? sweeps : 1);
+        A.info[A.large_ids[it.li]] = r;
+        if (A.info_host) A.info_host[A.large_ids[it.li]] = r;
         A.sweeps_out[it.li] = ok ? sweeps + ((local || P == 1) ? 1000 : 0) : 0;
         __threadfence_system();
     }
@@ -2281,6 +2330,10 @@
     HtnBuf tall_dev{HTN_BUF_DEVICE};
     HtnBuf tall_pin{HTN_BUF_PINNED};
     HtnBuf tall_flags{HTN_BUF_MAPPED};
+    HtnBuf mirror{HTN_BUF_MAPPED};
+    int64_t mirror_s_elems = 0;
+    int mirror_blocks = 0;
+    bool mirror_complete = false;
     hipStream_t aux = nullptr;
     hipEvent_t ev_fork = nullptr, ev_join = nullptr, ev_sweep[2] = {nullptr, nullptr};
     ~JacScratch() {
@@ -2389,6 +2442,8 @@
     int split;
     int32_t* info_dev;
     hipStream_t st;
+    double* S_host;
+    int* info_host;
     std::vector<int> large;
     std::vector<int> n_eff;
     int nl() const { return (int)large.size(); }
@@ -2588,6 +2643,7 @@
     ra.xcc_off = xcc_off;
     ra.two_partner = two_partner ? 1 : 0;
     ra.info = c.info_dev, ra.sweeps_out = B.d_ring_sw;
+    ra.S_host = c.S_host, ra.info_host = c.info_host;
     for (auto& bt : plan.batches) {
         ra.items = (const RingItem*)js.ring_items.p + bt.first;
         hipLaunchKernelGGL(k_jacobi_ring, dim3((unsigned)bt.second), dim3(RING_THREADS), 2 * RING_PANEL_ELEMS * sizeof(double2),
@@ -2596,6 +2652,7 @@
     HIP_TRY(hipGetLastError());
     HIP_TRY(hipStreamWaitEvent(c.st, js.ev_join, 0));
     HIP_TRY(htn_stream_spin(c.st));
+    js.mirror_complete = true;
     int used = 0;
     for (int li = 0; li < nl; ++li) {
         if (B.h_rank[li] < 0) return fail_msg("htn_jacobi_svd_z: a hand-off of the multi-workgroup QR timed out");
@@ -2629,27 +2686,29 @@
     if (sweeps_used) *sweeps_used = used;
     HIP_TRY(hipStreamWaitEvent(c.st, js.ev_join, 0));
     hipLaunchKernelGGL(k_jacobi_finish, dim3(nl), dim3(JAC_THREADS), 0, c.st, c.G, (const double2*)c.Vj, c.S, c.desc, B.d_ids,
-                       B.d_perm, B.d_sw, B.d_done, c.info_dev);
+                       B.d_perm, B.d_sw, B.d_done, c.info_dev, c.S_host, c.info_host);
     HIP_TRY(hipGetLastError());
     HIP_TRY(htn_stream_spin(c.st));
+    js.mirror_complete = true;
     return 0;
 }
 
 static int jacobi_svd_core(void* G, void* Vj, double* S, const htn_svd_block* desc, const htn_svd_block* desc_host,
                            int32_t n_blocks, int32_t max_m_host, int32_t max_sweeps, double tol, int32_t* info_dev,
-                           const htn_svd_opts* opts, void* stream, const int* skip_dev, const unsigned char* skip_host) {
+                           const htn_svd_opts* opts, void* stream, const int* skip_dev, const unsigned char* skip_host,
+                           double* S_host, int* info_host) {
     if (n_blocks <= 0) return 0;
     if (max_m_host > 64 * JAC_MAXEL) return fail_msg("htn_jacobi_svd_z: block taller than 512 rows");
     const double rank_cut = opts && opts->rank_cut > 0.0 ? opts->rank_cut : 0.0;
     JacCall c = {(double2*)G, (double2*)Vj, S, desc, desc_host, n_blocks, max_sweeps, tol, rank_cut * rank_cut,
-                 opts && opts->split_elems > 0 ? opts->split_elems : 0, info_dev, (hipStream_t)stream, {}, {}};
+                 opts && opts->split_elems > 0 ? opts->split_elems : 0, info_dev, (hipStream_t)stream, S_host, info_host, {}, {}};
     int32_t* sweeps_used = opts ? opts->sweeps_used : nullptr;
     if (jac_set_kernel_attributes()) return 1;
     c.large = classify_large(desc_host, n_blocks, c.split);
     if (sweeps_used) *sweeps_used = 0;
     if (c.large.empty()) {
         hipLaunchKernelGGL(k_jacobi_svd, dim3(n_blocks), dim3(JAC_THREADS), JAC_LDS_ELEMS * sizeof(double2), c.st, c.G, c.Vj, S,
-                           desc, max_sweeps, tol, info_dev, JAC_LDS_ELEMS, skip_dev, c.cut2);
+                           desc, max_sweeps, tol, info_dev, JAC_LDS_ELEMS, skip_dev, c.cut2, S_host, info_host);
         HIP_TRY(hipGetLastError());
         return 0;
     }
@@ -2685,7 +2744,7 @@
     HIP_TRY(hipEventRecord(js.ev_fork, c.st));
     HIP_TRY(hipStreamWaitEvent(js.aux, js.ev_fork, 0));
     hipLaunchKernelGGL(k_jacobi_svd, dim3(n_blocks), dim3(JAC_THREADS), JAC_LDS_ELEMS * sizeof(double2), js.aux, c.G, c.Vj, S,
-                       desc, max_sweeps, tol, info_dev, JAC_LDS_ELEMS, (const int*)B.d_slot, c.cut2);
+                       desc, max_sweeps, tol, info_dev, JAC_LDS_ELEMS, (const int*)B.d_slot, c.cut2, S_host, info_host);
     HIP_TRY(hipEventRecord(js.ev_join, js.aux));
     if (launch_qr_large(c, js, B, n_xcd)) return 1;
     if (c.cut2 > 0.0) {
@@ -2704,7 +2763,8 @@
 
 static int jacobi_svd_tall(void* G, void* Vj, double* S, const htn_svd_block* desc, const htn_svd_block* desc_host,
                            int32_t n_blocks, int32_t max_m_rest, int32_t max_sweeps, double tol, int32_t* info_dev,
-                           const htn_svd_opts* opts, void* stream, const std::vector<int>& tall) {
+                           const htn_svd_opts* opts, void* stream, const std::vector<int>& tall, double* S_host,
+                           int* info_host) {
     const int nt = (int)tall.size();
     hipStream_t st = (hipStream_t)stream;
     JacScratch* jsp = nullptr;
@@ -2747,7 +2807,7 @@
     int core_used = 0;
     if (nt < n_blocks) {
         if (jacobi_svd_core(G, Vj, S, desc, desc_host, n_blocks, max_m_rest, max_sweeps, tol, info_dev, opts, stream, d_skip,
-                            skip.data()))
+                            skip.data(), S_host, info_host))
             return 1;
         if (opts && opts->sweeps_used) core_used = *opts->sweeps_used;
     }
@@ -2767,10 +2827,54 @@
     });
     if (used < 0) return 1;
     hipLaunchKernelGGL(k_jacobi_tall_finish, dim3((unsigned)((max_n + 3) / 4), (unsigned)nt), dim3(256), 0, st,
-                       (const double2*)G, S, desc, d_ids, d_sw, d_done, info_dev);
+                       (const double2*)G, S, desc, d_ids, d_sw, d_done, info_dev, S_host, info_host);
     HIP_TRY(hipGetLastError());
     HIP_TRY(htn_stream_spin(st));
+    js.mirror_complete = true;
     if (opts && opts->sweeps_used) *opts->sweeps_used = std::max(core_used, used);
+    return 0;
+}
+
+static int svd_host_mirror(hipStream_t st, const htn_svd_block* desc_host, int n_blocks, double** S_host, int** info_host) {
+    JacScratch* js = nullptr;
+    if (js_get(st, &js)) return 1;
+    js->mirror_s_elems = 0, js->mirror_blocks = 0, js->mirror_complete = false;
+    static const bool off = htn_env_flag("HTN_SVD_NO_HOST_VIEW");
+    if (!desc_host || off) return 0;
+    int64_t s_elems = 0;
+    for (int b = 0; b < n_blocks; ++b) {
+        if (desc_host[b].s_off < 0) return 0;
+        s_elems = std::max<int64_t>(s_elems, desc_host[b].s_off + desc_host[b].n);
+    }
+    s_elems = (s_elems + 1) & ~(int64_t)1;
+    if (js->mirror.reserve(sizeof(double) * (size_t)s_elems + sizeof(int) * (size_t)n_blocks)) return 1;
+    js->mirror_s_elems = s_elems, js->mirror_blocks = n_blocks;
+    *S_host = (double*)js->mirror.dev;
+    *info_host = (int*)(*S_host + s_elems);
+    return 0;
+}
+int htn_svd_host_values(hipStream_t st, HtnSvdHostValues* out) {
+    JacScratch* js = nullptr;
+    if (js_get(st, &js)) return 1;
+    *out = HtnSvdHostValues{nullptr, nullptr, 0, 0};
+    if (js->mirror_blocks <= 0) return 0;
+    if (!js->mirror_complete) {
+        HIP_TRY(htn_stream_spin(st));
+        js->mirror_complete = true;
+    }
+    out->S = (const double*)js->mirror.p;
+    out->info = (const int32_t*)(out->S + js->mirror_s_elems);
+    out->s_elems = js->mirror_s_elems, out->n_blocks = js->mirror_blocks;
+    return 0;
+}
+extern "C" int htn_jacobi_svd_host_values(void* stream, const double** S_host, const int32_t** info_host, int64_t* s_elems,
+                                          int32_t* n_blocks) {
+    HtnSvdHostValues v;
+    if (htn_svd_host_values((hipStream_t)stream, &v)) return 1;
+    if (!v.S) return fail_msg("htn_jacobi_svd_host_values: the last htn_jacobi_svd_z call on this stream had no desc_host (no host copy of S)");
+    *S_host = v.S, *info_host = v.info;
+    if (s_elems) *s_elems = v.s_elems;
+    if (n_blocks) *n_blocks = v.n_blocks;
     return 0;
 }
 
@@ -2781,6 +2885,9 @@
     if (n_blocks <= 0) return 0;
     std::vector<int> tall;
     int max_m_rest = 0;
+    double* S_host = nullptr;
+    int* info_host = nullptr;
+    if (svd_host_mirror((hipStream_t)stream, desc_host, n_blocks, &S_host, &info_host)) return 1;
     if (desc_host) {
         for (int b = 0; b < n_blocks; ++b) {
             const htn_svd_block& D = desc_host[b];
@@ -2792,9 +2899,9 @@
     }
     if (tall.empty())
         return jacobi_svd_core(G, Vj, S, desc, desc_host, n_blocks, max_m_host, max_sweeps, tol, info_dev, opts, stream,
-                               nullptr, nullptr);
+                               nullptr, nullptr, S_host, info_host);
     if (max_m_rest > 64 * JAC_MAXEL) return fail_msg("htn_jacobi_svd_z: block taller than 512 rows");
-    return jacobi_svd_tall(G, Vj, S, desc, desc_host, n_blocks, max_m_rest, max_sweeps, tol, info_dev, opts, stream, tall);
+    return jacobi_svd_tall(G, Vj, S, desc, desc_host, n_blocks, max_m_rest, max_sweeps, tol, info_dev, opts, stream, tall, S_host, info_host);
 }
 
 __global__ __launch_bounds__(256) void k_batched_copy(double2* __restrict__ dst, const double2* __restrict__ src,
diff --git a/include/hubbardtn_hip.h b/include/hubbardtn_hip.h
--- a/include/hubbardtn_hip.h
+++ b/include/hubbardtn_hip.h
@@ -95,6 +95,8 @@
 int htn_jacobi_svd_z(void* G, void* Vj, double* S, const htn_svd_block* desc, const htn_svd_block* desc_host,
                      int32_t n_blocks, int32_t max_m_host, int32_t max_sweeps, double tol, int32_t* info_dev,
                      const htn_svd_opts* opts, void* stream);
+int htn_jacobi_svd_host_values(void* stream, const double** S_host, const int32_t** info_host, int64_t* s_elems,
+                               int32_t* n_blocks);
 
 typedef struct {
     int64_t dst_off, src_off, idx_off, scl_off;
```

New measurement: 426.3 ms. About the same (+0.6%).
